# caomuqing/neptune

Hardware: AMD Instinct MI355X
Metric: backend_replans_per_sec (higher is better)
Workload: dtype f64; 1 GPU; 64 agents + 20 static obstacles, K=8, 128 seeded scenes in flight per GPU per step (seeds 0..127 over 1 GPU); the handle's default solve path: verified line presolve 4 m, polish on; agents=64, obstacles=20, scenes_per_gpu=128, scenes_in_flight=128, scene_groups=1

## Files before the change

include/neptune_backend_debug.h:

```cpp
#ifndef NEPTUNE_BACKEND_DEBUG_H
#define NEPTUNE_BACKEND_DEBUG_H

#include "neptune_backend.h"

#ifdef __cplusplus
extern "C" {
#endif

int nep_backend_debug_time_sequence(nep_backend_t* h, const nep_pwp* init, int32_t n_obst, const int32_t* hull_off,
                                    const double* hull_xy, const int32_t* h0_off, const double* h0_xy, const nep_ent_view* ent,
                                    double t_start, double dc, int32_t n_iter, double* us_out, double* us_optimize_out);

int nep_backend_debug_set_lines(nep_backend_t* h, int32_t n_lines, const int32_t* seg,
                                const double* nd);
int nep_backend_debug_get_lines(nep_backend_t* h, int32_t cap, int32_t* seg, double* nd,
                                int32_t* n_out);

int nep_debug_regroup_records(const nep_traj_rec* d_src, nep_traj_rec* d_dst, int32_t world, int32_t n_scenes,
                              int32_t n_local, void* stream);

int nep_batch_debug_redo_count(nep_batch_t* h, int32_t* by_reason);
int nep_batch_debug_redo_list(nep_batch_t* h, int32_t* slots_out, int32_t cap);

int64_t nep_batch_line_bucket_bytes(nep_batch_t* h);
int64_t nep_batch_row_scratch_bytes(nep_batch_t* h);

int nep_batch_active_rows(nep_batch_t* h, const nep_solution* d_solution, double tol, int32_t* d_out, void* stream);

int nep_batch_debug_set_separator_pack(nep_batch_t* h, int32_t pack);

int nep_batch_qp_placement(nep_batch_t* h);

int nep_batch_set_launch_order(nep_batch_t* h, int32_t enable);
int nep_batch_debug_launch_order(nep_batch_t* h, int32_t* order, int32_t cap, int32_t* n_out);

int nep_batch_debug_set_option(nep_batch_t* h, const char* name, int32_t value);
int nep_backend_debug_set_option(nep_backend_t* h, const char* name, int32_t value);
int nep_debug_set_global_option(const char* name, int32_t value);

int nep_batch_set_hull_kernel(nep_batch_t* h, int32_t mode);

int nep_batch_debug_conflicts(nep_batch_t* h, int32_t scene, uint8_t* conflict_out);
int nep_batch_debug_conflicts_prev(nep_batch_t* h, int32_t scene, uint8_t* conflict_out);

int nep_batch_kernel_time(nep_batch_t* h, int32_t which, double* avg_ms, int32_t* n_launch);
int nep_batch_enable_timing(nep_batch_t* h, int32_t on);
int nep_batch_reset_timing(nep_batch_t* h);

enum {
  NEP_PATH_BOX_KERNEL = 1,
  NEP_PATH_HULLS_GROUPED = 2,
  NEP_PATH_FUSED_BOXES = 4,
  NEP_PATH_FUSED_ORDER = 8,
  NEP_PATH_ORDERED_QP = 16,
  NEP_PATH_PRESOLVE_KERNEL = 32,
  NEP_PATH_REDO_PASS = 64
};
int nep_batch_debug_launch_path(nep_batch_t* h, int32_t* bits);
int nep_batch_debug_boxes(nep_batch_t* h, int32_t scene, double* out, int32_t cap);
int nep_batch_debug_order_keys(nep_batch_t* h, int32_t* keys, int32_t cap);

int nep_batch_debug_hulls(nep_batch_t* h, int32_t scene, double* hull_xy, int32_t* hull_nv);
int nep_batch_debug_lines(nep_batch_t* h, int32_t slot, int32_t cap, int32_t* seg, double* nd,
                          int32_t* n_out);

int nep_batch_debug_phase_cycles(nep_batch_t* h, int32_t slot, int64_t* out16);

int nep_batch_fe_search_us(nep_batch_t* h, float* us, int32_t cap);

int nep_batch_set_fe_ent_fast_caps(nep_batch_t* h, int32_t list_cap, int32_t add_cap, int32_t bend_cap);

int nep_batch_debug_polish_count(nep_batch_t* h, int32_t* listed, int32_t* certified);
int nep_batch_debug_polish_flags(nep_batch_t* h, int32_t* flags, int32_t cap);

int nep_debug_live_bytes(int64_t* device_bytes, int64_t* pinned_bytes);

#ifdef __cplusplus
}
#endif
#endif
```

neptune_amd/_lib.py:

```python
import ctypes as C
import os

from . import abi

_HERE = os.path.dirname(os.path.abspath(__file__))
LIB_PATH = os.environ.get("NEP_BACKEND_LIB") or os.path.join(_HERE, "libneptune_backend.so")
_lib = None

EXPORTS = [
    "nep_backend_create", "nep_backend_destroy", "nep_backend_set_max_values", "nep_backend_set_max_runtime",
    "nep_backend_set_tether_length", "nep_backend_set_static_obst_vert", "nep_backend_set_init_trajectory",
    "nep_backend_set_hulls", "nep_backend_set_hulls_no_inflation", "nep_backend_set_ent_state_vector",
    "nep_backend_optimize", "nep_backend_generate_pwp_out", "nep_backend_get_stats", "nep_inflate_static",
    "nep_separator_batch", "nep_separator_batch_rule", "nep_gjk_batch", "nep_hulls_batch", "nep_batch_create",
    "nep_batch_destroy", "nep_batch_set_scene_statics", "nep_batch_replan", "nep_batch_replan_lines", "nep_batch_replan_solve", "nep_batch_hull_block_bytes",
    "nep_batch_set_ent_samples", "nep_batch_hulls", "nep_batch_replan_hulls", "nep_comm_unique_id",
    "nep_comm_create", "nep_comm_destroy", "nep_comm_nranks", "nep_batch_exchange_hulls",
    "nep_batch_exchange_records", "nep_batch_exchange_slots", "nep_comm_reserve", "nep_batch_ent_bytes",
    "nep_batch_safety_commit", "nep_batch_set_line_cull", "nep_backend_set_line_cull", "nep_batch_get_line_cull", "nep_batch_reserve_row_scratch",
    "nep_batch_set_line_capacity", "nep_batch_set_separator_rule", "nep_backend_set_separator_rule",
    "nep_batch_set_tolerances", "nep_backend_set_tolerances", "nep_batch_set_polish", "nep_backend_set_polish", "nep_batch_set_max_runtime",
    "nep_batch_set_safety_check_prev", "nep_batch_set_active", "nep_batch_wait", "nep_batch_check", "nep_abi_sizeof", "nep_last_error",
    "nep_version",
]
DEBUG_EXPORTS = [
    "nep_batch_debug_polish_count", "nep_batch_debug_polish_flags",
    "nep_backend_debug_time_sequence", "nep_backend_debug_set_lines", "nep_backend_debug_get_lines",
    "nep_debug_regroup_records", "nep_batch_debug_redo_count", "nep_batch_debug_redo_list",
    "nep_batch_line_bucket_bytes", "nep_batch_row_scratch_bytes", "nep_batch_active_rows",
    "nep_batch_debug_set_separator_pack", "nep_batch_qp_placement", "nep_batch_set_launch_order",
    "nep_batch_debug_launch_order", "nep_batch_set_hull_kernel", "nep_batch_debug_conflicts", "nep_batch_debug_conflicts_prev",
    "nep_batch_kernel_time", "nep_batch_enable_timing", "nep_batch_reset_timing", "nep_batch_debug_hulls",
    "nep_batch_debug_lines", "nep_batch_debug_phase_cycles", "nep_batch_fe_search_us",
    "nep_batch_set_fe_ent_fast_caps", "nep_batch_debug_set_option", "nep_backend_debug_set_option", "nep_debug_set_global_option",
    "nep_batch_debug_launch_path", "nep_batch_debug_boxes", "nep_batch_debug_order_keys", "nep_debug_live_bytes",
]
PLAN_EXPORTS = [
    "nep_pwp_compose", "nep_pwp_compose_exact", "nep_dyntraj_wire_size", "nep_dyntraj_encode", "nep_dyntraj_decode", "nep_plan_create",
    "nep_plan_destroy", "nep_plan_reset", "nep_plan_size", "nep_plan_get", "nep_plan_next_goal",
    "nep_plan_select_a", "nep_plan_splice", "nep_plan_update_delta", "nep_plan_delta",
]
FE_EXPORTS = ["nep_batch_frontend", "nep_batch_frontend_hulls", "nep_batch_set_static_reps", "nep_batch_set_fe_ent_big_records", "nep_batch_frontend_ent", "nep_batch_frontend_ent_hulls", "nep_batch_safety_commit_ent", "nep_batch_track_ent", "nep_batch_track_ent_lists", "nep_batch_ent_lists_at_a", "nep_batch_next_starts", "nep_batch_audit", "nep_audit_records", "nep_audit_init"]
FLEET_EXPORTS = ["nep_batch_fleet_init", "nep_batch_fleet_select", "nep_batch_fleet_commit", "nep_batch_fleet_tick", "nep_batch_fleet_ring_cap",
                 "nep_batch_fleet_plans", "nep_batch_fleet_state", "nep_batch_fleet_counters", "nep_batch_fleet_init_ent", "nep_batch_fleet_predict_ent",
                 "nep_batch_fleet_track_ent", "nep_batch_fleet_ent_state", "nep_batch_fleet_init_ent_lists", "nep_batch_fleet_ent_lists", "nep_batch_fleet_mission_keepout", "nep_batch_fleet_mission_init",
                 "nep_batch_fleet_mission", "nep_batch_fleet_mission_state", "nep_batch_fleet_mission_log", "nep_mission_step"]
ENT_EXPORTS = ["nep_ent_sample_points", "nep_ent_propagate_segment", "nep_ent_propagate_guess", "nep_ent_case_ids", "nep_ent_track_step", "nep_ent_predict_a"]


class BackendError(RuntimeError):
    pass


def lib():
    global _lib
    if _lib is not None:
        return _lib
    if not os.path.exists(LIB_PATH):
        raise BackendError("%s is missing: build it with `python -c 'import __graft_entry__ as g; g.build()'` "
                           "(or make -C neptune_amd/csrc); there is no CPU fallback" % LIB_PATH)
    try:
        import torch
    except ImportError:
        pass
    L = C.CDLL(LIB_PATH)
    d, i, vp = C.c_double, C.c_int32, C.c_void_p
    pd, pi = C.POINTER(C.c_double), C.POINTER(C.c_int32)
    L.nep_last_error.restype = C.c_char_p
    L.nep_version.restype = C.c_char_p
    L.nep_abi_sizeof.argtypes = [i]; L.nep_abi_sizeof.restype = C.c_int
    L.nep_backend_create.argtypes = [C.POINTER(abi.nep_backend_cfg)]; L.nep_backend_create.restype = vp
    L.nep_backend_destroy.argtypes = [vp]; L.nep_backend_destroy.restype = None
    L.nep_backend_set_max_values.argtypes = [vp] + [d] * 9
    L.nep_backend_set_max_runtime.argtypes = [vp, d]
    L.nep_backend_set_tether_length.argtypes = [vp, d]
    L.nep_backend_set_static_obst_vert.argtypes = [vp, i, pi, pd]
    L.nep_backend_set_init_trajectory.argtypes = [vp, C.POINTER(abi.nep_pwp)]
    L.nep_backend_set_hulls.argtypes = [vp, i, pi, pd]
    L.nep_backend_set_hulls_no_inflation.argtypes = [vp, i, pi, pd]
    L.nep_backend_set_ent_state_vector.argtypes = [vp, C.POINTER(abi.nep_ent_view)]
    L.nep_backend_optimize.argtypes = [vp, pd]
    L.nep_backend_generate_pwp_out.argtypes = [vp, d, d, C.POINTER(abi.nep_pwp), pd, i, pi]
    L.nep_backend_get_stats.argtypes = [vp, C.POINTER(abi.nep_stats)]
    L.nep_backend_debug_set_lines.argtypes = [vp, i, pi, pd]
    L.nep_backend_debug_get_lines.argtypes = [vp, i, pi, pd, pi]
    L.nep_separator_batch.argtypes = [i, pi, pd, pi, pd, pd, pi]
    L.nep_inflate_static.argtypes = [i, pi, pd, d, pi, pd, i]
    L.nep_separator_batch_rule.argtypes = [i, i, pi, pd, pi, pd, pd, pi]
    L.nep_batch_set_separator_rule.argtypes = [vp, i]
    L.nep_backend_set_separator_rule.argtypes = [vp, i]
    L.nep_batch_set_tolerances.argtypes = [vp, C.c_double, C.c_double]
    L.nep_backend_set_tolerances.argtypes = [vp, C.c_double, C.c_double]
    L.nep_gjk_batch.argtypes = [i, pi, pd, pd, pi]
    L.nep_hulls_batch.argtypes = [i, vp, d, i, d, d, pd, pi, pd, pi]
    L.nep_batch_create.argtypes = [C.POINTER(abi.nep_batch_cfg)]; L.nep_batch_create.restype = vp
    L.nep_batch_destroy.argtypes = [vp]; L.nep_batch_destroy.restype = None
    L.nep_batch_replan.argtypes = [vp, vp, vp, vp, vp, vp, vp, vp]
    L.nep_batch_replan_lines.argtypes = [vp, vp, vp, vp, vp]
    L.nep_batch_replan_solve.argtypes = [vp, vp, vp, vp, vp, vp, vp, vp]
    L.nep_batch_ent_bytes.argtypes = [vp]; L.nep_batch_ent_bytes.restype = C.c_int64
    L.nep_batch_wait.argtypes = [vp, vp]
    L.nep_batch_kernel_time.argtypes = [vp, i, pd, pi]
    L.nep_batch_enable_timing.argtypes = [vp, i]
    L.nep_batch_reset_timing.argtypes = [vp]
    L.nep_batch_debug_hulls.argtypes = [vp, i, pd, pi]
    L.nep_batch_debug_lines.argtypes = [vp, i, i, pi, pd, pi]
    L.nep_batch_debug_phase_cycles.argtypes = [vp, i, C.POINTER(C.c_int64)]
    L.nep_batch_safety_commit.argtypes = [vp, vp, vp, vp, vp, vp, vp]
    L.nep_batch_debug_conflicts.argtypes = [vp, i, C.POINTER(C.c_uint8)]
    L.nep_batch_debug_conflicts_prev.argtypes = [vp, i, C.POINTER(C.c_uint8)]
    L.nep_batch_set_safety_check_prev.argtypes = [vp, i]
    L.nep_batch_set_active.argtypes = [vp, vp]
    L.nep_batch_set_line_cull.argtypes = [vp, d]; L.nep_backend_set_line_cull.argtypes = [vp, d]
    L.nep_batch_debug_set_option.argtypes = [vp, C.c_char_p, i]; L.nep_backend_debug_set_option.argtypes = [vp, C.c_char_p, i]; L.nep_debug_set_global_option.argtypes = [C.c_char_p, i]
    L.nep_batch_get_line_cull.argtypes = [vp]; L.nep_batch_get_line_cull.restype = d
    L.nep_batch_debug_redo_count.argtypes = [vp, pi]
    L.nep_batch_debug_redo_list.argtypes = [vp, pi, i]
    L.nep_batch_debug_set_separator_pack.argtypes = [vp, i]
    L.nep_batch_active_rows.argtypes = [vp, vp, d, vp, vp]
    L.nep_batch_reserve_row_scratch.argtypes = [vp]
    L.nep_batch_set_line_capacity.argtypes = [vp, i]
    L.nep_batch_set_fe_ent_big_records.argtypes = [vp, C.c_int64]
    L.nep_batch_set_fe_ent_fast_caps.argtypes = [vp, i, i, i]
    L.nep_batch_fe_search_us.argtypes = [vp, C.POINTER(C.c_float), i]
    L.nep_batch_line_bucket_bytes.argtypes = [vp]; L.nep_batch_line_bucket_bytes.restype = C.c_int64
    L.nep_batch_row_scratch_bytes.argtypes = [vp]; L.nep_batch_row_scratch_bytes.restype = C.c_int64
    L.nep_backend_debug_time_sequence.argtypes = [vp, vp, i, pi, pd, pi, pd, vp, d, d, i, pd, pd]
    L.nep_batch_set_max_runtime.argtypes = [vp, d]
    L.nep_batch_qp_placement.argtypes = [vp]
    L.nep_batch_set_launch_order.argtypes = [vp, i]
    L.nep_batch_set_hull_kernel.argtypes = [vp, i]
    L.nep_batch_debug_launch_order.argtypes = [vp, pi, i, pi]
    L.nep_batch_debug_launch_path.argtypes = [vp, pi]
    L.nep_batch_debug_boxes.argtypes = [vp, i, pd, i]
    L.nep_batch_debug_order_keys.argtypes = [vp, pi, i]
    L.nep_debug_live_bytes.argtypes = [C.POINTER(C.c_int64), C.POINTER(C.c_int64)]
    L.nep_batch_set_scene_statics.argtypes = [vp, i, i, pi, pd]
    L.nep_batch_check.argtypes = [vp, vp]
    L.nep_comm_unique_id.argtypes = [C.POINTER(C.c_uint8)]
    L.nep_comm_create.argtypes = [C.POINTER(C.c_uint8), i, i]; L.nep_comm_create.restype = vp
    L.nep_comm_destroy.argtypes = [vp]; L.nep_comm_destroy.restype = None
    L.nep_comm_nranks.argtypes = [vp]
    L.nep_comm_reserve.argtypes = [vp, C.c_int64, C.c_int64]
    L.nep_batch_exchange_hulls.argtypes = [vp, vp, vp, vp, vp]
    L.nep_batch_exchange_records.argtypes = [vp, vp, vp, vp, vp]
    L.nep_debug_regroup_records.argtypes = [vp, vp, i, i, i, vp]
    L.nep_batch_hull_block_bytes.argtypes = [vp]; L.nep_batch_hull_block_bytes.restype = C.c_int64
    L.nep_batch_hulls.argtypes = [vp, vp, vp, vp, vp]
    L.nep_batch_replan_hulls.argtypes = [vp, vp, i, vp, vp, vp, vp, vp, vp]
    ppwp, prec, phdr = C.POINTER(abi.nep_pwp), C.POINTER(abi.nep_traj_rec), C.POINTER(abi.nep_wire_header)
    pu8 = C.POINTER(C.c_uint8)
    L.nep_pwp_compose.argtypes = [d, d, ppwp, ppwp, ppwp]
    L.nep_pwp_compose_exact.argtypes = [d, ppwp, ppwp, ppwp]
    L.nep_dyntraj_wire_size.argtypes = [prec, phdr]; L.nep_dyntraj_wire_size.restype = C.c_int64
    L.nep_dyntraj_encode.argtypes = [prec, phdr, pu8, C.c_size_t]; L.nep_dyntraj_encode.restype = C.c_int64
    L.nep_dyntraj_decode.argtypes = [pu8, C.c_size_t, prec, phdr]; L.nep_dyntraj_decode.restype = C.c_int64
    L.nep_plan_create.argtypes = [C.POINTER(abi.nep_plan_cfg)]; L.nep_plan_create.restype = vp
    L.nep_plan_destroy.argtypes = [vp]; L.nep_plan_destroy.restype = None
    L.nep_plan_reset.argtypes = [vp, pd]
    L.nep_plan_size.argtypes = [vp]
    L.nep_plan_get.argtypes = [vp, i, pd]
    L.nep_plan_next_goal.argtypes = [vp, pd, pi]
    L.nep_plan_select_a.argtypes = [vp, pd, d, C.POINTER(abi.nep_point_a)]
    L.nep_plan_splice.argtypes = [vp, i, pd, i]
    L.nep_plan_update_delta.argtypes = [vp, d]
    L.nep_plan_delta.argtypes = [vp]
    pcfg, pin, pst = C.POINTER(abi.nep_ent_cfg), C.POINTER(abi.nep_ent_inputs), C.POINTER(abi.nep_ent_state)
    L.nep_ent_sample_points.argtypes = [ppwp, d, d, i, i, pd]
    L.nep_ent_propagate_segment.argtypes = [pcfg, pin, pst, pd, pd, pd, i, pd]
    L.nep_ent_propagate_guess.argtypes = [pcfg, pin, pst, vp, i, pi, pi, pi, pi, pst]
    L.nep_ent_case_ids.argtypes = [i, i, pi, pi, pi, i, pi]
    L.nep_ent_track_step.argtypes = [pcfg, C.POINTER(abi.nep_ent_track_inputs), pst, pd, pd]
    L.nep_ent_predict_a.argtypes = [pcfg, pd, pd, pi, pi, pd, pst, pd, pd, pst]
    L.nep_batch_frontend.argtypes = [vp, C.POINTER(abi.nep_fe_cfg), vp, vp, vp, vp, vp]
    L.nep_batch_frontend_hulls.argtypes = [vp, C.POINTER(abi.nep_fe_cfg), vp, i, vp, vp, vp, vp]
    L.nep_batch_set_static_reps.argtypes = [vp, i, pd, pd]
    L.nep_batch_frontend_ent.argtypes = [vp, C.POINTER(abi.nep_fe_cfg), vp, vp, vp, vp, vp, vp, vp]
    L.nep_batch_safety_commit_ent.argtypes = [vp, vp, vp, vp, vp, i, d, vp, vp, vp]
    L.nep_batch_next_starts.argtypes = [vp, vp, d, vp, vp, d, vp]
    L.nep_batch_track_ent.argtypes = [vp, vp, vp, vp, i, i, d, vp, vp, vp]
    L.nep_batch_track_ent_lists.argtypes = [vp, vp, vp, vp, i, i, d, C.POINTER(abi.nep_ent_lists), vp, vp]
    L.nep_batch_ent_lists_at_a.argtypes = [vp, C.POINTER(abi.nep_ent_lists), vp, vp, vp, vp, vp, vp]
    L.nep_batch_audit.argtypes = [vp, vp, vp, d, i, vp, vp]
    L.nep_audit_records.argtypes = [vp, i, pi, pd, i, d, d, d, i, vp]
    L.nep_audit_init.argtypes = [vp, C.c_int64]
    L.nep_batch_fleet_init.argtypes = [vp, C.POINTER(abi.nep_fleet_cfg), vp, vp, vp, vp, vp]
    L.nep_batch_fleet_select.argtypes = [vp, vp, vp, vp, vp, vp]
    L.nep_batch_fleet_commit.argtypes = [vp, vp, vp, vp, vp, vp, vp]
    L.nep_batch_fleet_tick.argtypes = [vp, vp]
    L.nep_batch_fleet_ring_cap.argtypes = [vp]
    L.nep_batch_fleet_plans.argtypes = [vp, i, i, pd, pi]
    L.nep_batch_fleet_state.argtypes = [vp, pd, vp, pi, pi, pi, pi, pi]
    L.nep_batch_fleet_counters.argtypes = [vp, pi, pd, pi]
    L.nep_batch_fleet_init_ent.argtypes = [vp, d, vp, vp]
    L.nep_batch_fleet_predict_ent.argtypes = [vp, vp, vp, vp, vp, vp]
    L.nep_batch_fleet_track_ent.argtypes = [vp, vp, vp, vp]
    L.nep_batch_fleet_ent_state.argtypes = [vp, vp, pi, pi, pi]
    L.nep_batch_fleet_init_ent_lists.argtypes = [vp, d, C.POINTER(abi.nep_ent_lists), vp]
    L.nep_batch_fleet_ent_lists.argtypes = [vp, C.POINTER(abi.nep_ent_lists), pi]
    L.nep_batch_fleet_mission_keepout.argtypes = [vp, i, i, pi, pd]
    L.nep_batch_fleet_mission_init.argtypes = [vp, C.POINTER(abi.nep_mission_cfg), vp]
    L.nep_batch_fleet_mission.argtypes = [vp, vp]
    L.nep_batch_fleet_mission_state.argtypes = [vp, pd, pd, pd, pi, pi, pd, pi, pd]
    L.nep_batch_fleet_mission_log.argtypes = [vp, vp, pi]
    L.nep_mission_step.argtypes = [C.POINTER(abi.nep_mission_cfg), C.POINTER(abi.nep_mission_scene)]
    L.nep_batch_frontend_ent_hulls.argtypes = [vp, C.POINTER(abi.nep_fe_cfg), vp, i, vp, vp, vp, vp, vp, vp]
    L.nep_batch_exchange_slots.argtypes = [vp, vp, vp, vp, C.c_int64, vp]
    L.nep_batch_set_ent_samples.argtypes = [vp, i]
    L.nep_batch_set_polish.argtypes = [vp, i]; L.nep_backend_set_polish.argtypes = [vp, i]; L.nep_batch_debug_polish_count.argtypes = [vp, pi, pi]; L.nep_batch_debug_polish_flags.argtypes = [vp, pi, i]
    L.nep_abi_sizeof.argtypes = [i]; L.nep_abi_sizeof.restype = i
    for which, struct in ((1, abi.nep_traj_rec), (5, abi.nep_guess), (6, abi.nep_solution), (11, abi.nep_fe_cfg), (12, abi.nep_fe_start),
                          (13, abi.nep_fe_result), (14, abi.nep_fe_ent_state), (17, abi.nep_audit), (18, abi.nep_fleet_cfg),
                          (20, abi.nep_mission_cfg), (21, abi.nep_mission_leg), (23, abi.nep_ent_lists)):
        if L.nep_abi_sizeof(which) != C.sizeof(struct):
            raise BackendError("%s: sizeof(%s) is %d in the library, %d in neptune_amd/abi.py — rebuild the library from this tree's headers"
                               % (LIB_PATH, struct.__name__, L.nep_abi_sizeof(which), C.sizeof(struct)))
    _lib = L
    return L
# ... 7 lines not shown
```

neptune_amd/backend.py:

```python
import ctypes as C

import numpy as np

from . import abi
from ._lib import BackendError, check, lib


def _csr(polys):
    off = np.zeros(len(polys) + 1, dtype=np.int32)
    for k, p in enumerate(polys):
        off[k + 1] = off[k] + len(p)
    xy = (np.concatenate([np.asarray(p, dtype=np.float64).reshape(-1, 2) for p in polys])
          if len(polys) and off[-1] > 0 else np.zeros((0, 2)))
    return off, np.ascontiguousarray(xy, dtype=np.float64)


def make_pwp(times, coeff):
    p = abi.nep_pwp()
    K = coeff.shape[1]
    p.n_seg = K
    for i in range(K + 1):
        p.times[i] = float(times[i])
    arr = np.ctypeslib.as_array(p.coeff)
    arr[:, :K, :] = coeff
# ... 383 lines not shown
        check(lib().nep_batch_fleet_ent_state(self._h, out["state"].ctypes.data if states else None, abi.iptr(out["flags"]), abi.iptr(out["ever"]),
                                              abi.iptr(out["walked"])))
        return out

    def fleet_mission_keepout(self, scene, polys):
        off, xy = _csr(polys)
        check(lib().nep_batch_fleet_mission_keepout(self._h, scene, len(polys), abi.iptr(off), abi.dptr(xy)))

    def fleet_mission_init(self, cfg, stream=None):
        st = stream if stream is not None else self.torch.cuda.current_stream(self.device)
        check(lib().nep_batch_fleet_mission_init(self._h, C.byref(cfg), st.cuda_stream))
        self.mission_cfg = cfg

    def fleet_mission(self, stream=None):
        st = stream if stream is not None else self.torch.cuda.current_stream(self.device)
        check(lib().nep_batch_fleet_mission(self._h, st.cuda_stream))

    def fleet_mission_state(self):
        n, S = self.slots, self.n_scenes
        out = dict(goal=np.zeros((n, 3)), t_issue=np.zeros(n), length=np.zeros(n), completed=np.zeros(n, dtype=np.int32),
                   counts=np.zeros((n, 4), dtype=np.int32), sums=np.zeros((n, 2)), scene=np.zeros((S, 4), dtype=np.int32), t_run=np.zeros(S))
        check(lib().nep_batch_fleet_mission_state(self._h, abi.dptr(out["goal"]), abi.dptr(out["t_issue"]), abi.dptr(out["length"]),
                                                  abi.iptr(out["completed"]), abi.iptr(out["counts"]), abi.dptr(out["sums"]),
                                                  abi.iptr(out["scene"]), abi.dptr(out["t_run"])))
        return out

    def fleet_mission_finished(self):
        sc = np.zeros((self.n_scenes, 4), dtype=np.int32)
        check(lib().nep_batch_fleet_mission_state(self._h, None, None, None, None, None, None, abi.iptr(sc), None))
        return sc[:, 3] != 0

    def fleet_mission_log(self, ordered=True):
        cfg = self.mission_cfg
        owners = self.slots if cfg.mode == abi.NEP_MISSION_PER_AGENT else self.n_scenes
        cap = int(cfg.log_cap)
        log = np.zeros((owners, max(cap, 1)), dtype=abi.MISSION_LEG_DTYPE); n = np.zeros(owners, dtype=np.int32)
        check(lib().nep_batch_fleet_mission_log(self._h, log.ctypes.data, abi.iptr(n)))
        log = log[:, :cap]
        if not ordered:
            return log, n
        return [log[o, [i % cap for i in range(max(0, int(n[o]) - cap), int(n[o]))]] if cap else log[o, :0] for o in range(owners)], n

    def next_starts(self, d_records, dt, d_start, d_alt_goal=None, switch_radius=0.0, stream=None):
        st = stream if stream is not None else self.torch.cuda.current_stream(self.device)
        check(lib().nep_batch_next_starts(self._h, d_records.data_ptr(), float(dt), d_start.data_ptr(),
                                          d_alt_goal.data_ptr() if d_alt_goal is not None else None, float(switch_radius), st.cuda_stream))

    def safety_commit(self, d_prev, d_new, d_guess, d_final, d_accept=None, stream=None):
        st = stream if stream is not None else self.torch.cuda.current_stream(self.device)
        check(lib().nep_batch_safety_commit(self._h, d_prev.data_ptr(), d_new.data_ptr(), d_guess.data_ptr(), d_final.data_ptr(),
                                            d_accept.data_ptr() if d_accept is not None else None, st.cuda_stream))

    def set_active(self, mask):
        torch = self.torch
        if mask is not None:
            if mask.dtype != torch.int32 or mask.device != self.device or tuple(mask.shape) != (self.n_scenes, self.N) or not mask.is_contiguous():
                raise ValueError("the active mask is a contiguous int32 tensor [n_scenes, N] on the handle's device")
        check(lib().nep_batch_set_active(self._h, mask.data_ptr() if mask is not None else None))
        self._active = mask

    def set_scene_statics(self, scene, statics):
        soff, sxy = _csr(statics)
        check(lib().nep_batch_set_scene_statics(self._h, scene, len(statics), abi.iptr(soff), abi.dptr(sxy)))

    def check(self, stream=None):
        st = stream if stream is not None else self.torch.cuda.current_stream(self.device)
        check(lib().nep_batch_check(self._h, st.cuda_stream))

    def qp_kernel_name(self):
        return "qp_reg_kernel" if lib().nep_batch_qp_placement(self._h) == 1 else "qp_kernel"

    def set_hull_kernel(self, mode=0):
        check(lib().nep_batch_set_hull_kernel(self._h, int(mode)))

    def set_launch_order(self, enable=True):
        check(lib().nep_batch_set_launch_order(self._h, 1 if enable else 0))

    def launch_order(self):
        out = np.zeros(self.n_scenes * self.n_local, dtype=np.int32); n = C.c_int32(0)
        check(lib().nep_batch_debug_launch_order(self._h, abi.iptr(out), len(out), C.byref(n)))
        return out[:n.value].copy() if n.value else None

    LAUNCH_PATH = (("box_kernel", 1), ("grouped_hulls", 2), ("fused_boxes", 4), ("fused_order", 8), ("ordered_qp", 16),
                   ("presolve_kernel", 32), ("redo_pass", 64))

    def debug_launch_path(self):
        b = C.c_int32(0)
        check(lib().nep_batch_debug_launch_path(self._h, C.byref(b)))
        return {name: bool(b.value & bit) for name, bit in self.LAUNCH_PATH}

    def debug_boxes(self, scene=0):
        out = np.zeros((self.N + self.n_static, self.par.num_pol, 4))
        check(lib().nep_batch_debug_boxes(self._h, int(scene), abi.dptr(out), out.size))
        return out

    def debug_order_keys(self):
        out = np.zeros(self.slots, dtype=np.int32)
        check(lib().nep_batch_debug_order_keys(self._h, abi.iptr(out), len(out)))
        return out

    def set_max_runtime(self, seconds):
        check(lib().nep_batch_set_max_runtime(self._h, float(seconds)))

    def set_line_cull(self, radius):
        check(lib().nep_batch_set_line_cull(self._h, float(radius)))

    def line_cull(self):
        return float(lib().nep_batch_get_line_cull(self._h))

    def redo_count(self):
        r = np.zeros(2, dtype=np.int32)
        n = int(check(lib().nep_batch_debug_redo_count(self._h, abi.iptr(r))))
        self.redo_reasons = {"parked_line_violated": int(r[0]), "moved_beyond_radius": int(r[1])}
        return n

    def reserve_row_scratch(self):
        check(lib().nep_batch_reserve_row_scratch(self._h))

    def fe_search_us(self):
        out = np.zeros(self.slots, dtype=np.float32)
        check(lib().nep_batch_fe_search_us(self._h, out.ctypes.data_as(C.POINTER(C.c_float)), int(self.slots)))
        return out

    def set_fe_ent_big_records(self, records):
        check(lib().nep_batch_set_fe_ent_big_records(self._h, int(records)))

    def set_fe_ent_fast_caps(self, list_cap=40, add_cap=32, bend_cap=8):
        check(lib().nep_batch_set_fe_ent_fast_caps(self._h, int(list_cap), int(add_cap), int(bend_cap)))

    def set_line_capacity(self, lines_per_segment):
        check(lib().nep_batch_set_line_capacity(self._h, int(lines_per_segment)))

    def line_bucket_bytes(self):
        return int(lib().nep_batch_line_bucket_bytes(self._h))

    def row_scratch_bytes(self):
        return int(lib().nep_batch_row_scratch_bytes(self._h))

    def set_separator_pack(self, pack):
        check(lib().nep_batch_debug_set_separator_pack(self._h, int(pack)))

    def redo_list(self, cap=4096):
        out = np.zeros(cap, dtype=np.int32)
        n = int(check(lib().nep_batch_debug_redo_list(self._h, abi.iptr(out), cap)))
        return out[:n].copy()

    def set_separator_rule(self, rule):
        check(lib().nep_batch_set_separator_rule(self._h, int(rule)))

    def set_tolerances(self, residual_tol=1e-10, gap_tol=1e-11):
        check(lib().nep_batch_set_tolerances(self._h, float(residual_tol), float(gap_tol)))

    def set_polish(self, on=True):
        check(lib().nep_batch_set_polish(self._h, int(on) if (on is not True and on is not False) else (1 if on else 0)))

    def debug_option(self, name, value):
        check(lib().nep_batch_debug_set_option(self._h, name.encode(), int(value)))

    def polish_count(self):
        a = C.c_int32(0); b = C.c_int32(0)
        check(lib().nep_batch_debug_polish_count(self._h, C.byref(a), C.byref(b)))
        return a.value, b.value

    def polish_flags(self):
        out = np.zeros(self.n_scenes * self.n_local, dtype=np.int32)
        check(lib().nep_batch_debug_polish_flags(self._h, abi.iptr(out), len(out)))
        return out

    def set_safety_check_prev(self, on=True):
        check(lib().nep_batch_set_safety_check_prev(self._h, 1 if on else 0))

    def debug_conflicts(self, scene=0):
        out = np.zeros((self.N, self.N), dtype=np.uint8)
        check(lib().nep_batch_debug_conflicts(self._h, scene, out.ctypes.data_as(C.POINTER(C.c_uint8))))
        return out

    def debug_conflicts_prev(self, scene=0):
        out = np.zeros((self.N, self.N), dtype=np.uint8)
        check(lib().nep_batch_debug_conflicts_prev(self._h, scene, out.ctypes.data_as(C.POINTER(C.c_uint8))))
        return out

# ... 71 lines not shown
```

neptune_amd/csrc/backend.hip:

```cpp
#include <hip/hip_runtime.h>

#include <atomic>
#include <chrono>
#include <cmath>
#include <cstdio>
#include <cstdlib>
#include <cstring>
#include <memory>
#include <string>
#include <vector>

#include "nep_device.h"
#include "qp_outputs.h"
#include "audit_common.h"
#include "mission_common.h"
#include "../../include/neptune_plan.h"
#include "../../include/neptune_entangle.h"

using namespace nep;

namespace nep { DebugGlobals g_debug; }

namespace {

// ... 14 lines not shown
  ~DevBuf() { release(); }
  int ensure(size_t count) {
    if (count <= n && p) return 0;
    release();
    if (count == 0) count = 1;
    hipError_t e = hipMalloc((void**)&p, count * sizeof(T));
    if (e != hipSuccess) { p = nullptr; g_err = std::string("hipMalloc: ") + hipGetErrorString(e); return NEP_E_HIP; }
    n = count; g_live_device += (long long)(n * sizeof(T));
    return 0;
  }
  void release() { if (p) { hipFree(p); g_live_device -= (long long)(n * sizeof(T)); } p = nullptr; n = 0; }
};

struct ListBuf {
  DevBuf<int> n_alpha, n_bend; DevBuf<int16_t> id, bend; DevBuf<int8_t> cs; DevBuf<double> beta; int cap = 0;
  int ensure(size_t slots, int cap_) {
    if (int e = n_alpha.ensure(slots)) return e;
    if (int e = n_bend.ensure(slots)) return e;
    if (int e = id.ensure(slots * cap_)) return e;
    if (int e = cs.ensure(slots * cap_)) return e;
    if (int e = beta.ensure(slots * cap_)) return e;
    if (int e = bend.ensure(slots * NEP_MAX_BEND)) return e;
    cap = cap_;
    return 0;
  }
  nep_ent_lists view() const { nep_ent_lists v{}; v.cap = cap; v.n_alpha = n_alpha.p; v.n_bend = n_bend.p; v.id = id.p; v.cs = cs.p; v.beta = beta.p; v.bend = bend.p; return v; }
};

struct PinnedArena {
  char* p = nullptr; size_t n = 0;
  PinnedArena() = default;
  PinnedArena(const PinnedArena&) = delete;
  PinnedArena& operator=(const PinnedArena&) = delete;
  PinnedArena(PinnedArena&& o) noexcept : p(o.p), n(o.n) { o.p = nullptr; o.n = 0; }
  PinnedArena& operator=(PinnedArena&& o) noexcept { if (this != &o) { release(); p = o.p; n = o.n; o.p = nullptr; o.n = 0; } return *this; }
  ~PinnedArena() { release(); }
  int ensure(size_t bytes) {
    if (bytes <= n && p) return 0;
    char* q = nullptr;
    hipError_t e = hipHostMalloc((void**)&q, bytes ? bytes : 1, hipHostMallocDefault);
    if (e != hipSuccess) { g_err = std::string("hipHostMalloc: ") + hipGetErrorString(e); return NEP_E_HIP; }
    if (p) std::memcpy(q, p, n);
    if (bytes > n) std::memset(q + n, 0, bytes - n);
    release();
    p = q; n = bytes; g_live_pinned += (long long)(bytes ? bytes : 1);
    return 0;
  }
  void release() { if (p) { hipHostFree(p); g_live_pinned -= (long long)(n ? n : 1); } p = nullptr; n = 0; }
};

constexpr size_t kLdsBudget = 150 * 1024;

bool normalize_ccw(double* xy, int n) {
  if (n < 3) return true;
  double area2 = 0, scale = 0;
  for (int v = 0; v < n; v++) {
    const double* a = xy + 2 * v; const double* b = xy + 2 * ((v + 1) % n);
    area2 += a[0] * b[1] - a[1] * b[0];
    scale = std::fmax(scale, std::fmax(std::fabs(a[0]), std::fabs(a[1])));
  }
  if (area2 < 0) for (int lo = 1, hi = n - 1; lo < hi; lo++, hi--) { std::swap(xy[2 * lo], xy[2 * hi]); std::swap(xy[2 * lo + 1], xy[2 * hi + 1]); }
  const double tol = 1e-9 * (1.0 + scale) * (1.0 + scale);
  for (int v = 0; v < n; v++) {
    const double* o = xy + 2 * v; const double* a = xy + 2 * ((v + 1) % n); const double* b = xy + 2 * ((v + 2) % n);
    if ((a[0] - o[0]) * (b[1] - o[1]) - (a[1] - o[1]) * (b[0] - o[0]) < -tol) return false;
  }
  return true;
}

double wall_clock_hz() {
  int dev = 0, khz = 0;
  if (hipGetDevice(&dev) == hipSuccess && hipDeviceGetAttribute(&khz, hipDeviceAttributeWallClockRate, dev) == hipSuccess && khz > 0) return (double)khz * 1e3;
  return 1e8;
}

struct Engine {
  SceneParams sp{};
  int n_scenes = 1;
  DevBuf<QpTable> d_tables;
  DevBuf<int> d_sched_n, d_sched_seg; DevBuf<double> d_sched_dt;
  DevBuf<double> d_pb, d_static_xy, d_static_el; DevBuf<int> d_static_nv;
  DevBuf<double> d_hull_xy, d_hull0_xy, d_bend_xy, d_line_nd, d_row_scratch;
  DevBuf<int> d_hull_nv, d_hull0_nv, d_bend_n, d_line_cnt, d_line_far, d_lp_stats;
  DevBuf<int> d_presolved; bool presolve_kernel = true;
  DevBuf<int> d_line_skip, d_redo_list, d_redo_count;
  DevBuf<double> d_polish_z; DevBuf<int> d_polish_flag, d_polish_list, d_polish_count; bool polish = true, polish_presolve = true, last_polish_armed = false;
  DevBuf<long long> d_dbg; bool profile_phases = false;
  DevBuf<int> d_flags;
  DevBuf<double> d_sampled, d_srep, d_slong; DevBuf<int> d_present, d_entangles;
  DevBuf<nep_fe_ent_state> d_fe_nodes, d_fe_work, d_fe_saved; DevBuf<double> d_fe_arc, d_fe_packed; bool have_reps = false;
  DevBuf<double> d_fe_big_beta, d_fe_stf; DevBuf<long long> d_fe_stvox; DevBuf<unsigned> d_fe_xpool;
  DevBuf<unsigned char> d_fe_big, d_fe_big_check; DevBuf<int> d_fe_big_count, d_fe_big_check_count; long fe_big_records = 0;
  int fe_fast_cap = NEP_FE_ENT_CAP, fe_fast_add = 32, fe_fast_bend = NEP_MAX_BEND;
  DevBuf<unsigned char> d_conflict, d_conflict_prev;
  bool safety_check_prev = false;
  int lds_lines = 0, lds_rows = 0, rows_cap = 0; size_t lds_bytes = 0;
  DevBuf<double> d_fe_box;
  DevBuf<int> d_fe_order, d_fe_order_key; DevBuf<float> d_fe_us; bool fe_history = false, fe_lpt = true;
  DevBuf<int> d_order, d_order_key; bool have_history = false, lpt = true, last_ordered = false;
  const int* active = nullptr;
  DevBuf<int> d_act, d_fe_act;
  ListBuf d_track_lsave;
  DevBuf<nep_fe_ent_state> d_track_save; DevBuf<int> d_track_flags; DevBuf<double> d_track_pos;
  DevBuf<AuditPart> d_audit_part;
  int static_nv_max = 0;
  DevBuf<nep_traj_rec> d_safety_recs;
  bool use_reg = false;
  double clock_hz = 1e8;
  void set_clock() { clock_hz = wall_clock_hz(); sp.us_per_tick = 1e6 / clock_hz; sp.corr_from_it = opt_corr_from; sp.corr_max_count = opt_corr_max; if (!(sp.tol_res > 0.0)) { sp.tol_res = 1e-10; sp.tol_gap = 1e-11; sp.tol_res_inv = 1e10; sp.tol_gap_inv = 1e11; sp.tol_gap_floor = 0.1 * 1e-11; } }
  double sched_dc = -1, tab_T = -1, tab_w = -1; int sched_cap = 0;
  std::vector<int> h_sched_n, h_sched_seg; std::vector<double> h_sched_dt;
  bool timing = false; std::vector<hipEvent_t> ev; size_t ev_used = 0;

  int build_tables() {
    if (tab_T == sp.T_span && tab_w == sp.weight && d_tables.p) return 0;
    std::vector<QpTable> t(2 * (kMaxK + 1));
    std::memset(t.data(), 0, t.size() * sizeof(QpTable));
    for (int mode = 0; mode < 2; mode++) for (int K = 1; K <= kMaxK; K++) build_qp_table(K, sp.T_span, sp.weight, mode, &t[mode * (kMaxK + 1) + K]);
    if (int e = d_tables.ensure(t.size())) return e;
    HIPCHK(hipMemcpy(d_tables.p, t.data(), t.size() * sizeof(QpTable), hipMemcpyHostToDevice));
    tab_T = sp.T_span; tab_w = sp.weight;
    return 0;
  }
  int build_schedule(double dc, int cap) {
    if (dc == sched_dc && cap == sched_cap && d_sched_n.p) return 0;
    h_sched_n.assign(kMaxK + 1, 0); h_sched_seg.assign((size_t)(kMaxK + 1) * cap, 0); h_sched_dt.assign((size_t)(kMaxK + 1) * cap, 0.0);
    for (int K = 1; K <= kMaxK; K++) h_sched_n[K] = build_sample_schedule(K, sp.T_span, dc, cap, &h_sched_seg[(size_t)K * cap], &h_sched_dt[(size_t)K * cap]);
    if (int e = d_sched_n.ensure(h_sched_n.size())) return e;
    if (int e = d_sched_seg.ensure(h_sched_seg.size())) return e;
    if (int e = d_sched_dt.ensure(h_sched_dt.size())) return e;
    HIPCHK(hipMemcpy(d_sched_n.p, h_sched_n.data(), h_sched_n.size() * sizeof(int), hipMemcpyHostToDevice));
    HIPCHK(hipMemcpy(d_sched_seg.p, h_sched_seg.data(), h_sched_seg.size() * sizeof(int), hipMemcpyHostToDevice));
    HIPCHK(hipMemcpy(d_sched_dt.p, h_sched_dt.data(), h_sched_dt.size() * sizeof(double), hipMemcpyHostToDevice));
    sched_dc = dc; sched_cap = cap; sp.max_states = cap; sp.dc = dc;
    return 0;
  }
  static constexpr double kAutoCullRadius = 4.0;
  bool fits_reg = true, cull_user_set = false, skip_lps = true, no_redo = false; int lds_lines_lds = 0, sep_pack = 0, force_kernel = 0, opt_qp_key_decay = 2, opt_fe_key_decay = 1, opt_corr_from = kCorrFromItDefault, opt_corr_max = kCorrMaxCountDefault, opt_fleet_ent_proof = 1;
  static constexpr int kScratchPool = 1024;
  bool scratch_full = false; int scratch_chunks = 0;
  std::vector<double> h_static_box;
  const double* box_buf = nullptr; int box_N = -1, box_S = -1, box_np = -1;
  bool static_boxes_ok = false;
  bool static_boxes_placed() const { return static_boxes_ok && box_buf == d_fe_box.p && box_N == sp.num_agents && box_S == sp.n_static && box_np == sp.num_pol; }
  static void static_boxes_of(int n, const std::vector<double>& sx, const std::vector<int>& nv, double* out) {
    for (int j = 0; j < n; j++) {
      const double* q = &sx[(size_t)j * kHullV * 2];
      double x0 = HUGE_VAL, x1 = -HUGE_VAL, y0 = HUGE_VAL, y1 = -HUGE_VAL;
      if (nv[j] > 0) { x0 = x1 = q[0]; y0 = y1 = q[1]; }
      for (int v = 1; v < nv[j]; v++) { x0 = std::fmin(x0, q[2 * v]); x1 = std::fmax(x1, q[2 * v]); y0 = std::fmin(y0, q[2 * v + 1]); y1 = std::fmax(y1, q[2 * v + 1]); }
      out[4 * j] = x0; out[4 * j + 1] = x1; out[4 * j + 2] = y0; out[4 * j + 3] = y1;
    }
  }
  int push_static_boxes(int scene = -1) {
    const bool placed = static_boxes_placed();
    static_boxes_ok = false;
    const int N = sp.num_agents, S = sp.n_static, np = sp.num_pol;
    const size_t row = (size_t)(N + S) * np * 4, blk = (size_t)S * np * 4;
    if (!d_fe_box.p || d_fe_box.n < (size_t)n_scenes * row || h_static_box.size() < (size_t)n_scenes * S * 4) return 0;
    if (S > 0) {
      const int s0 = (scene >= 0 && placed) ? scene : 0, s1 = (scene >= 0 && placed) ? scene + 1 : n_scenes;
      std::vector<double> b((size_t)(s1 - s0) * blk);
      for (int s = s0; s < s1; s++)
        for (int j = 0; j < S; j++)
          for (int i = 0; i < np; i++) std::memcpy(&b[(((size_t)(s - s0) * S + j) * np + i) * 4], &h_static_box[((size_t)s * S + j) * 4], 4 * sizeof(double));
      HIPCHK(hipMemcpy2D(d_fe_box.p + (size_t)s0 * row + (size_t)N * np * 4, row * sizeof(double), b.data(), blk * sizeof(double), blk * sizeof(double), (size_t)(s1 - s0), hipMemcpyHostToDevice));
    }
// ... 1 lines not shown
    return 0;
  }
  int last_path = 0;
  int lines_cap_user = 0;
  bool can_skip_lps() const { return sp.cull_radius > 0.0 && use_reg && sp.sep_rule == 0 && sp.skip_own == 1 && sp.n_hull == sp.num_agents && skip_lps && statics_boxy; }
  bool skip_mode() const { return can_skip_lps() && !no_redo; }
  int size_row_scratch() {
    const long slots = (long)n_scenes * sp.n_local;
    const bool pooled = skip_mode() && !scratch_full && slots > kScratchPool;
    scratch_chunks = pooled ? kScratchPool : 0;
    return d_row_scratch.ensure((size_t)(pooled ? kScratchPool : slots) * (11L * (rows_cap / 4 + 2)));
  }
  void choose_placement() {
    use_reg = fits_reg || sp.cull_radius > 0.0;
    if (force_kernel == 1) use_reg = true; else if (force_kernel == 2) use_reg = false;
    if (use_reg) { lds_lines = NEP_MAX_POL * 8 * qp_reg_slots(); lds_rows = 4 * lds_lines; lds_bytes = qp_reg_lds_bytes(); }
    else { lds_lines = lds_lines_lds; lds_rows = 4 * lds_lines; lds_bytes = qp_lds_fixed_bytes() + (size_t)(lds_lines + 2) * 11 * 8; }
  }
  int size_scratch() {
    const int N = sp.num_agents, np = sp.num_pol;
    const long slots = (long)n_scenes * sp.n_local;
    const int worst_lines = sp.n_hull + N + sp.n_static + (sp.ent_enabled ? N * kBend : 0);
    if ((long)NEP_MAX_POL * worst_lines > 65535) return fail(NEP_E_CAP, "more than 65535 separator candidates per agent");
    sp.lines_cap = lines_cap_user < 0 ? worst_lines : (lines_cap_user > 0 ? lines_cap_user : sp.n_hull + N + sp.n_static + (sp.ent_enabled ? std::min(N * kBend, std::max(2 * N, 64)) : 0));
    if (sp.lines_cap > worst_lines) sp.lines_cap = worst_lines;
    if (sp.lines_cap < 8) sp.lines_cap = 8;
    const long lines_total = (long)NEP_MAX_POL * sp.lines_cap;
    const size_t fixed = qp_lds_fixed_bytes();
    const long per_line = 11 * 8;
    const long l_half = ((long)(160 * 1024 / 2) - (long)fixed) / per_line - 2;
    const long l_full = ((long)kLdsBudget - (long)fixed) / per_line - 2;
    const long expect = (long)NEP_MAX_POL * (sp.n_hull + 4 + sp.n_static / 8 + (sp.ent_enabled ? sp.num_agents / 8 : 0));
    long ll = expect <= l_half ? l_half : l_full;
    if (ll > lines_total) ll = lines_total;
    lds_lines_lds = (int)((ll + 1) & ~1L);
    fits_reg = expect / NEP_MAX_POL <= 8L * qp_reg_slots() + 8;
    if (!cull_user_set) sp.cull_radius = kAutoCullRadius;
    sp.fe_key_decay = opt_fe_key_decay; sp.qp_key_decay = opt_qp_key_decay;
    if (lpt) { if (int e = d_order.ensure((size_t)slots)) return e; const int* was = d_order_key.p; if (int e = d_order_key.ensure((size_t)slots)) return e; if (d_order_key.p != was) hipMemset(d_order_key.p, 0, d_order_key.n * sizeof(int)); }
    if (lpt) { if (int e = d_fe_order.ensure((size_t)slots)) return e; const int* was = d_fe_order_key.p; if (int e = d_fe_order_key.ensure((size_t)slots)) return e; if (d_fe_order_key.p != was) hipMemset(d_fe_order_key.p, 0, d_fe_order_key.n * sizeof(int)); }
    if (int e = d_fe_us.ensure((size_t)slots)) return e;
    choose_placement();
    rows_cap = 4 * (int)lines_total; rows_cap = (rows_cap + 3) & ~3;
    if (int e = d_hull_xy.ensure((size_t)n_scenes * sp.n_hull * np * kHullV * 2)) return e;
    if (int e = d_fe_box.ensure((size_t)n_scenes * (N + (sp.n_static > 0 ? sp.n_static : 0)) * np * 4)) return e;
    if (!static_boxes_placed()) { if (int e = push_static_boxes()) return e; }
    if (int e = d_hull_nv.ensure((size_t)n_scenes * sp.n_hull * np)) return e;
    if (int e = d_hull0_xy.ensure((size_t)n_scenes * N * np * 2)) return e;
    if (int e = d_hull0_nv.ensure((size_t)n_scenes * N * np)) return e;
    if (int e = d_bend_xy.ensure((size_t)n_scenes * N * kBend * 2)) return e;
    if (int e = d_bend_n.ensure((size_t)n_scenes * N)) return e;
    if (int e = d_line_nd.ensure((size_t)slots * lines_total * 3)) return e;
    if (int e = d_line_cnt.ensure((size_t)slots * NEP_MAX_POL)) return e;
    if (int e = d_line_far.ensure((size_t)slots * NEP_MAX_POL)) return e;
    if (int e = d_lp_stats.ensure((size_t)slots * NEP_MAX_POL * 2)) return e;
    if (int e = d_line_skip.ensure((size_t)slots * NEP_MAX_POL)) return e;
    if (int e = d_redo_list.ensure((size_t)slots)) return e;
    if (int e = d_presolved.ensure((size_t)slots)) return e;
    if (!d_redo_count.p) { if (int e = d_redo_count.ensure(4)) return e; HIPCHK(hipMemset(d_redo_count.p, 0, 4 * sizeof(int))); }
    if (!d_flags.p) { if (int e = d_flags.ensure(1)) return e; HIPCHK(hipMemset(d_flags.p, 0, sizeof(int))); }
    if (int e = d_polish_z.ensure((size_t)slots * 2 * 24)) return e;
    if (int e = d_polish_flag.ensure((size_t)slots)) return e;
    if (int e = d_polish_list.ensure((size_t)slots)) return e;
    if (!d_polish_count.p) { if (int e = d_polish_count.ensure(8)) return e; HIPCHK(hipMemset(d_polish_count.p, 0, 8 * sizeof(int))); }
    if (!profile_phases) profile_phases = getenv("NEP_QP_PROFILE") != nullptr;
    if (profile_phases) { if (int e = d_dbg.ensure((size_t)slots * 32)) return e; }
    if (int e = size_row_scratch()) return e;
    return 0;
  }
  void fill(ProblemSet& ps) {
    ps.pb = d_pb.p; ps.static_xy = d_static_xy.p; ps.static_nv = d_static_nv.p; ps.static_el = d_static_el.p;
    ps.hull_xy = d_hull_xy.p; ps.hull_nv = d_hull_nv.p; ps.hull0_xy = d_hull0_xy.p; ps.hull0_nv = d_hull0_nv.p;
    ps.bend_xy = d_bend_xy.p; ps.bend_n = d_bend_n.p;
    ps.fe_order = nullptr; ps.fe_order_key = (lpt && fe_lpt && d_fe_order_key.n >= (size_t)n_scenes * (size_t)sp.n_local) ? d_fe_order_key.p : nullptr; ps.fe_us = d_fe_us.p;
    ps.line_nd = d_line_nd.p; ps.line_cnt = d_line_cnt.p; ps.lp_stats = d_lp_stats.p;
    ps.line_far = sp.cull_radius > 0.0 ? d_line_far.p : nullptr;
    const bool skip = can_skip_lps();
    ps.scratch_chunks = skip_mode() ? scratch_chunks : 0; ps.scratch_by_block = 0;
    ps.skip_box = skip ? d_fe_box.p : nullptr; ps.line_skip = skip ? d_line_skip.p : nullptr;
    ps.redo_list = skip ? d_redo_list.p : nullptr; ps.redo_count = skip ? d_redo_count.p : nullptr; ps.order_count = nullptr;
    ps.sep_pack = sep_pack;
    ps.row_scratch = d_row_scratch.p; ps.rows_cap = rows_cap; ps.lds_rows = lds_rows; ps.lds_lines = lds_lines;
    ps.dbg = profile_phases ? d_dbg.p : nullptr;
    ps.presolved = nullptr;
    ps.flags = d_flags.p;
    ps.fe_box = d_fe_box.p;
    ps.active = active; ps.fe_count = nullptr;
    const bool pol = polish && use_reg && (polish_presolve || !(sp.cull_radius > 0.0)) && d_polish_z.p != nullptr;
    ps.polish_z = pol ? d_polish_z.p : nullptr; ps.polish_flag = pol ? d_polish_flag.p : nullptr;
    ps.polish_list = pol ? d_polish_list.p : nullptr; ps.polish_count = pol ? d_polish_count.p : nullptr;
    last_polish_armed = pol;
  }
  bool statics_boxy = true;
  int pack_statics(int n, const int32_t* off, const double* xy, std::vector<double>& sx, std::vector<int>& nv, std::vector<double>& el) {
    sx.assign((size_t)(n > 0 ? n : 1) * kHullV * 2, 0.0); nv.assign(n > 0 ? n : 1, 0);
    for (int j = 0; j < n; j++) {
      int c = off[j + 1] - off[j];
      if (c > kHullV) return fail(NEP_E_CAP, "static obstacle with more than NEP_HULL_MAX_V vertices");
      if (c < 0) return fail(NEP_E_ARG, "static obstacle offsets must not decrease");
      nv[j] = c;
      if (c > static_nv_max) static_nv_max = c;
      for (int v = 0; v < c; v++) { sx[((size_t)j * kHullV + v) * 2] = xy[2 * (off[j] + v)]; sx[((size_t)j * kHullV + v) * 2 + 1] = xy[2 * (off[j] + v) + 1]; }
      if (!normalize_ccw(&sx[(size_t)j * kHullV * 2], c)) return fail(NEP_E_ARG, "static obstacle polygon is not convex");
      if (c > 0) {
        const double* q = &sx[(size_t)j * kHullV * 2];
        double lo[2] = {q[0], q[1]}, hi[2] = {q[0], q[1]};
        for (int v = 1; v < c; v++) for (int a = 0; a < 2; a++) { lo[a] = std::min(lo[a], q[2 * v + a]); hi[a] = std::max(hi[a], q[2 * v + a]); }
        const double tol = 1e-9 * (1.0 + (hi[0] - lo[0]) + (hi[1] - lo[1]));
        for (int a = 0; a < 2; a++) {
          int n_lo = 0, n_hi = 0;
          for (int v = 0; v < c; v++) { n_lo += q[2 * v + a] - lo[a] <= tol; n_hi += hi[a] - q[2 * v + a] <= tol; }
          if (n_lo < 2 || n_hi < 2) statics_boxy = false;
        }
      }
    }
    el.assign(sx.size() / 2, 0.0);
    for (int j = 0; j < n; j++)
      for (int v = 0; v + 1 < nv[j]; v++) {
        const double* q = &sx[((size_t)j * kHullV + v) * 2];
        volatile double ex = q[2] - q[0], ey = q[3] - q[1];
        volatile double a = ex * ex, b = ey * ey;
        volatile double c = a + b;
        el[(size_t)j * kHullV + v] = std::sqrt(c);
      }
    return 0;
  }
  int upload_statics(int n, const int32_t* off, const double* xy) {
    static_boxes_ok = false;
    std::vector<double> sx, el; std::vector<int> nv;
    statics_boxy = true;
    if (int e = pack_statics(n, off, xy, sx, nv, el)) return e;
    if (int e = d_static_xy.ensure(sx.size())) return e;
    if (int e = d_static_el.ensure(el.size())) return e;
    if (int e = d_static_nv.ensure(nv.size())) return e;
    HIPCHK(hipMemcpy(d_static_el.p, el.data(), el.size() * sizeof(double), hipMemcpyHostToDevice));
    HIPCHK(hipMemcpy(d_static_xy.p, sx.data(), sx.size() * sizeof(double), hipMemcpyHostToDevice));
    HIPCHK(hipMemcpy(d_static_nv.p, nv.data(), nv.size() * sizeof(int), hipMemcpyHostToDevice));
    sp.n_static = n; sp.static_stride = 0;
    h_static_box.resize((size_t)n_scenes * n * 4);
    for (int s = 0; s < n_scenes; s++) static_boxes_of(n, sx, nv, &h_static_box[(size_t)s * n * 4]);
    if (n_scenes > 0 && sp.num_agents > 0 && sp.num_pol > 0)
      if (int e = d_fe_box.ensure((size_t)n_scenes * (sp.num_agents + n) * sp.num_pol * 4)) return e;
    return push_static_boxes();
  }
  int upload_scene_statics(int scene, int n, const int32_t* off, const double* xy) {
    const int S = sp.n_static;
    if (n != S) return fail(NEP_E_ARG, "every scene must have the handle's n_static polygons");
    if (S == 0) return 0;
    std::vector<double> sx, el; std::vector<int> nv;
    if (int e = pack_statics(n, off, xy, sx, nv, el)) return e;
    if (sp.static_stride == 0) {
      DevBuf<double> nxy, nel; DevBuf<int> nnv;
      if (int e = nxy.ensure((size_t)n_scenes * S * kHullV * 2)) return e;
      if (int e = nel.ensure((size_t)n_scenes * S * kHullV)) return e;
      if (int e = nnv.ensure((size_t)n_scenes * S)) return e;
      for (int s = 0; s < n_scenes; s++) {
        HIPCHK(hipMemcpy(nxy.p + (size_t)s * S * kHullV * 2, d_static_xy.p, (size_t)S * kHullV * 2 * sizeof(double), hipMemcpyDeviceToDevice));
        HIPCHK(hipMemcpy(nel.p + (size_t)s * S * kHullV, d_static_el.p, (size_t)S * kHullV * sizeof(double), hipMemcpyDeviceToDevice));
        HIPCHK(hipMemcpy(nnv.p + (size_t)s * S, d_static_nv.p, (size_t)S * sizeof(int), hipMemcpyDeviceToDevice));
      }
      d_static_xy = std::move(nxy); d_static_el = std::move(nel); d_static_nv = std::move(nnv);
      sp.static_stride = S;
      if (have_reps && d_srep.p && d_srep.n >= (size_t)S * 4 && d_slong.n >= (size_t)S * 2) {
        DevBuf<double> nr, nl;
        if (int e = nr.ensure((size_t)n_scenes * S * 4)) return e;
        if (int e = nl.ensure((size_t)n_scenes * S * 2)) return e;
        for (int s = 0; s < n_scenes; s++) {
          HIPCHK(hipMemcpy(nr.p + (size_t)s * S * 4, d_srep.p, (size_t)S * 4 * sizeof(double), hipMemcpyDeviceToDevice));
          HIPCHK(hipMemcpy(nl.p + (size_t)s * S * 2, d_slong.p, (size_t)S * 2 * sizeof(double), hipMemcpyDeviceToDevice));
        }
        d_srep = std::move(nr); d_slong = std::move(nl);
      } else have_reps = false;
    }
    HIPCHK(hipMemcpy(d_static_xy.p + (size_t)scene * S * kHullV * 2, sx.data(), (size_t)S * kHullV * 2 * sizeof(double), hipMemcpyHostToDevice));
    HIPCHK(hipMemcpy(d_static_el.p + (size_t)scene * S * kHullV, el.data(), (size_t)S * kHullV * sizeof(double), hipMemcpyHostToDevice));
    HIPCHK(hipMemcpy(d_static_nv.p + (size_t)scene * S, nv.data(), (size_t)S * sizeof(int), hipMemcpyHostToDevice));
    static_boxes_of(S, sx, nv, &h_static_box[(size_t)scene * S * 4]);
    return push_static_boxes(scene);
  }
  hipEvent_t next_event() {
    if (ev_used == ev.size()) { hipEvent_t e; hipEventCreate(&e); ev.push_back(e); }
    return ev[ev_used++];
  }
  int run(const nep_traj_rec* d_recs, int n_rec, ProblemSet& ps, hipStream_t st, int phases = 3) {
    const int slots = n_scenes * sp.n_local;
    SampleSched sc{d_sched_n.p, d_sched_seg.p, d_sched_dt.p};
    const bool geo = (phases & 1) != 0, qp = (phases & 2) != 0;
    if (timing) hipEventRecord(next_event(), st);
    const bool fused_boxes = d_recs && geo && ps.skip_box != nullptr && !ps.lines_override && static_boxes_ok && ps.hull_pb <= 0
                             && n_rec == sp.num_agents && sp.n_hull == sp.num_agents && hulls_grouped(sp, n_scenes, n_rec);
    const bool want_order = qp && lpt && have_history && slots > 1024 && d_order_key.n >= (size_t)slots && d_order.n >= (size_t)slots;
    const bool fused_order = fused_boxes && want_order;
    if (fused_order) { ps.order = d_order.p; ps.order_key = d_order_key.p; }
    if (geo) last_path = 0; else last_path &= NEP_PATH_BOX_KERNEL | NEP_PATH_HULLS_GROUPED | NEP_PATH_FUSED_BOXES | NEP_PATH_FUSED_ORDER;
    if (d_recs && geo) launch_hulls(d_recs, n_scenes, n_rec, ps.guess, sp, ps, st, fused_boxes);
    if (d_recs && geo && hulls_grouped(sp, n_scenes, n_rec)) last_path |= NEP_PATH_HULLS_GROUPED;
    if (fused_boxes) last_path |= NEP_PATH_FUSED_BOXES;
    if (fused_order) last_path |= NEP_PATH_FUSED_ORDER;
    if (timing) hipEventRecord(next_event(), st);
    if (ps.lines_override) { ps.skip_box = nullptr; ps.line_skip = nullptr; ps.redo_list = nullptr; ps.redo_count = nullptr; }
    if (scratch_chunks > 0 && ps.scratch_chunks == 0) {
      scratch_full = true;
      HIPCHK(hipStreamSynchronize(st));
      if (int e = size_row_scratch()) return e;
      ps.row_scratch = d_row_scratch.p;
    }
    const bool skip = ps.skip_box != nullptr;
    if (!ps.lines_override && geo) {
      if (skip && !fused_boxes) { launch_boxes(n_scenes, sp, ps, st); last_path |= NEP_PATH_BOX_KERNEL; }
      launch_separator(slots, sp, ps, st);
    }
    if (timing) hipEventRecord(next_event(), st);
    if (!qp) { if (timing) hipEventRecord(next_event(), st); HIPCHK(hipGetLastError()); return 0; }
    ps.order = nullptr; last_ordered = false;
    ps.order_key = (lpt && d_order_key.n >= (size_t)slots) ? d_order_key.p : nullptr;
    if (ps.order_key && have_history && slots > 1024 && d_order.n >= (size_t)slots) {
      if (!fused_order) launch_qp_order(slots, d_order_key.p, d_order.p, st, ps.polish_count);
      ps.order = d_order.p; last_ordered = true; last_path |= NEP_PATH_ORDERED_QP;
    } else if (ps.polish_count && !(use_reg && slots == 1)) launch_qp_polish_zero(ps.polish_count, st);
    if (ps.active) {
      if (int e = d_act.ensure((size_t)slots + 1)) return e;
      launch_active_list(slots, sp, ps.active, ps.order, d_act.p, ps.polish_count, st);
      ps.order = d_act.p; ps.order_count = d_act.p + slots;
      launch_skipped_replan(slots, sp, ps, st);
    }
    if (use_reg && presolve_kernel && ps.line_far != nullptr && !ps.lines_override && d_presolved.n >= (size_t)slots) {
      ps.presolved = d_presolved.p;
      launch_qp_presolve(slots, sp, ps, d_tables.p, sc, d_presolved.p, st);
      last_path |= NEP_PATH_PRESOLVE_KERNEL;
    }
    if (use_reg) launch_qp_reg(slots, sp, ps, d_tables.p, sc, lds_bytes, st);
    else launch_qp(slots, sp, ps, d_tables.p, sc, lds_bytes, st);
    if (skip && !no_redo) {
      launch_separator_redo(slots, sp, ps, st);
      last_path |= NEP_PATH_REDO_PASS;
      ProblemSet pr = ps;
      pr.line_far = nullptr; pr.line_skip = nullptr; pr.order = d_redo_list.p; pr.order_count = d_redo_count.p;
      pr.presolved = nullptr;
      pr.scratch_by_block = ps.scratch_chunks > 0 ? 1 : 0;
      launch_qp_reg(slots, sp, pr, d_tables.p, sc, lds_bytes, st);
    }
    if (ps.polish_list) launch_qp_polish(slots, sp, ps, d_tables.p, sc, st);
    have_history = ps.order_key != nullptr;
    if (timing) hipEventRecord(next_event(), st);
    HIPCHK(hipGetLastError());
    return 0;
  }
  ~Engine() { for (auto e : ev) hipEventDestroy(e); }
};

bool have_device() { int n = 0; return hipGetDeviceCount(&n) == hipSuccess && n > 0; }


__global__ void sample_kernel(const nep_solution* __restrict__ sol, int K, const int* __restrict__ seg, const double* __restrict__ dt, int ns, double* __restrict__ out) {
  const int s = blockIdx.x * blockDim.x + threadIdx.x;
  if (s >= ns) return;
  sample_state(&sol->coeff[0][0][0], seg[s], dt[s], out + (long)s * NEP_STATE_DOUBLES);
}

int read_lines(Engine& E, size_t slot, int n_seg, int32_t cap, int32_t* seg, double* nd, int32_t* n_out) {
  std::vector<int> cnt(NEP_MAX_POL), far(NEP_MAX_POL, 0); std::vector<double> buf((size_t)NEP_MAX_POL * E.sp.lines_cap * 3);
  HIPCHK(hipMemcpy(cnt.data(), E.d_line_cnt.p + slot * NEP_MAX_POL, cnt.size() * sizeof(int), hipMemcpyDeviceToHost));
  if (E.sp.cull_radius > 0.0) HIPCHK(hipMemcpy(far.data(), E.d_line_far.p + slot * NEP_MAX_POL, far.size() * sizeof(int), hipMemcpyDeviceToHost));
  HIPCHK(hipMemcpy(buf.data(), E.d_line_nd.p + slot * NEP_MAX_POL * E.sp.lines_cap * 3, buf.size() * sizeof(double), hipMemcpyDeviceToHost));
  for (int& c : cnt) c = line_count(c);
  int n = 0;
  for (int s = 0; s < n_seg && s < NEP_MAX_POL; s++)
    for (int c = 0; c < cnt[s] + far[s]; c++) {
      const size_t q = c < cnt[s] ? (size_t)c : (size_t)E.sp.lines_cap - 1 - (size_t)(c - cnt[s]);
      const double* e = &buf[((size_t)s * E.sp.lines_cap + q) * 3];
      if (e[0] == 0.0 && e[1] == 0.0 && e[2] == 0.0) continue;
      if (n < cap) { seg[n] = s; for (int k = 0; k < 3; k++) nd[3 * n + k] = e[k]; }
      n++;
    }
  *n_out = n;
  return 0;
}

}

struct InLayout { size_t guess, nv, cas, h0xy, h0nv, bend, bendn, xy, cap_end; };
static InLayout in_layout(int N, int np, int cap) {
  auto up = [](size_t v) { return (v + 255) & ~(size_t)255; };
  InLayout L{};
  size_t o = 0;
  L.guess = o; o = up(o + sizeof(nep_guess));
  L.nv = o; o = up(o + (size_t)cap * np * sizeof(int));
  L.cas = o; o = up(o + (size_t)NEP_MAX_POL * N * sizeof(int));
  L.h0xy = o; o = up(o + (size_t)N * np * 2 * sizeof(double));
  L.h0nv = o; o = up(o + (size_t)N * np * sizeof(int));
  L.bend = o; o = up(o + (size_t)N * kBend * 2 * sizeof(double));
  L.bendn = o; o = up(o + (size_t)N * sizeof(int));
  L.xy = o; o = up(o + (size_t)cap * np * kHullV * 2 * sizeof(double));
  L.cap_end = o;
  return L;
}
struct nep_backend {
  Engine eng;
  nep_backend_cfg cfg{};
  std::vector<double> pb;
  double max_runtime = 0.05, tether = 0, j_max = 0;
  bool have_bounds = false, have_init = false, have_hulls = false, solved = false;
  nep_guess guess{}; std::vector<double> guess_times;
  int n_obst = 0;
  PinnedArena hin, hout; DevBuf<char> d_in, d_out;
  int in_cap = 0; InLayout L{};
  bool have_h0 = false, have_ent = false, states_fresh = false;
  int override_n = -1; std::vector<int> ov_seg; std::vector<double> ov_nd;
  nep_solution h_sol{}; nep_stats stats{};
// ... 1275 lines not shown
  launch_next_starts(d_records, h->cfg.n_scenes, h->cfg.num_agents, h->cfg.first_local, h->cfg.n_local, dt, d_start, d_alt_goal, switch_radius, (hipStream_t)stream);
  HIPCHK(hipGetLastError());
  return 0;
}

int nep_batch_set_scene_statics(nep_batch_t* h, int32_t scene, int32_t n_static, const int32_t* static_off, const double* static_xy) {
  if (!h || scene < 0 || scene >= h->cfg.n_scenes || n_static < 0 || (n_static > 0 && (!static_off || !static_xy))) return fail(NEP_E_ARG, "bad arguments");
  HIPCHK(hipDeviceSynchronize());
  return h->eng.upload_scene_statics(scene, n_static, static_off, static_xy);
}

int nep_batch_debug_redo_count(nep_batch_t* h, int32_t* by_reason) {
  if (!h) return fail(NEP_E_ARG, "null handle");
  int n[3] = {0, 0, 0};
  HIPCHK(hipDeviceSynchronize());
  if (h->eng.d_redo_count.p) HIPCHK(hipMemcpy(n, h->eng.d_redo_count.p, 3 * sizeof(int), hipMemcpyDeviceToHost));
  if (by_reason) { by_reason[0] = n[1]; by_reason[1] = n[2]; }
  return n[0];
}

int nep_batch_debug_redo_list(nep_batch_t* h, int32_t* slots_out, int32_t cap) {
  if (!h || !slots_out || cap < 0) return fail(NEP_E_ARG, "bad arguments");
  int n = 0;
  HIPCHK(hipDeviceSynchronize());
  if (!h->eng.d_redo_count.p) return 0;
  HIPCHK(hipMemcpy(&n, h->eng.d_redo_count.p, sizeof(int), hipMemcpyDeviceToHost));
  if (n > cap) n = cap;
  if (n > 0) HIPCHK(hipMemcpy(slots_out, h->eng.d_redo_list.p, (size_t)n * sizeof(int), hipMemcpyDeviceToHost));
  return n;
}

int nep_batch_debug_set_separator_pack(nep_batch_t* h, int32_t pack) {
  if (!h || pack < -1 || pack > NEP_MAX_POL) return fail(NEP_E_ARG, "pack must be -1, 0 or 1..NEP_MAX_POL");
  h->eng.sep_pack = pack;
  return 0;
}

int nep_batch_qp_placement(nep_batch_t* h) { return h ? (h->eng.use_reg ? 1 : 0) : NEP_E_ARG; }

int nep_batch_set_launch_order(nep_batch_t* h, int32_t enable) {
  if (!h) return fail(NEP_E_ARG, "null handle");
  if (enable) { if (int e = h->eng.d_order.ensure((size_t)h->slots)) return e; if (int e = h->eng.d_order_key.ensure((size_t)h->slots)) return e; }
  if (enable) { if (int e = h->eng.d_fe_order.ensure((size_t)h->slots)) return e; if (int e = h->eng.d_fe_order_key.ensure((size_t)h->slots)) return e; }
  if (!enable) { h->eng.have_history = false; h->eng.fe_history = false; }
  if (enable && !h->eng.lpt) {
    HIPCHK(hipDeviceSynchronize());
    HIPCHK(hipMemset(h->eng.d_order_key.p, 0, h->eng.d_order_key.n * sizeof(int))); HIPCHK(hipMemset(h->eng.d_fe_order_key.p, 0, h->eng.d_fe_order_key.n * sizeof(int)));
    h->eng.have_history = false; h->eng.fe_history = false;
  }
  h->eng.lpt = enable != 0;
  return 0;
}
int nep_batch_fe_search_us(nep_batch_t* h, float* us, int32_t cap) {
  if (!h || !us || cap < h->slots) return fail(NEP_E_ARG, "bad arguments");
  HIPCHK(hipDeviceSynchronize());
  HIPCHK(hipMemcpy(us, h->eng.d_fe_us.p, (size_t)h->slots * sizeof(float), hipMemcpyDeviceToHost));
  return 0;
}
int nep_batch_debug_launch_order(nep_batch_t* h, int32_t* order, int32_t cap, int32_t* n_out) {
  if (!h || !order || !n_out || cap < 0) return fail(NEP_E_ARG, "bad arguments");
  *n_out = 0;
  if (!h->eng.last_ordered) return 0;
  if (cap < h->slots) return fail(NEP_E_CAP, "order buffer smaller than the slot count");
  HIPCHK(hipDeviceSynchronize());
  HIPCHK(hipMemcpy(order, h->eng.d_order.p, (size_t)h->slots * sizeof(int), hipMemcpyDeviceToHost));
  *n_out = h->slots;
  return 0;
}
int nep_batch_debug_launch_path(nep_batch_t* h, int32_t* bits) {
  if (!h || !bits) return fail(NEP_E_ARG, "bad arguments");
  *bits = h->eng.last_path;
  return 0;
}
int nep_batch_debug_boxes(nep_batch_t* h, int32_t scene, double* out, int32_t cap) {
  if (!h || !out || scene < 0 || scene >= h->cfg.n_scenes || cap < 0) return fail(NEP_E_ARG, "bad arguments");
  const Engine& E = h->eng;
  const size_t n = (size_t)(E.sp.num_agents + E.sp.n_static) * E.sp.num_pol * 4;
  if ((size_t)cap < n) return fail(NEP_E_CAP, "box buffer smaller than (num_agents + n_static) x num_pol x 4 doubles");
  if (!E.d_fe_box.p || E.d_fe_box.n < (size_t)h->cfg.n_scenes * n) return fail(NEP_E_STATE, "the handle has no obstacle boxes");
  HIPCHK(hipDeviceSynchronize());
  HIPCHK(hipMemcpy(out, E.d_fe_box.p + (size_t)scene * n, n * sizeof(double), hipMemcpyDeviceToHost));
  return 0;
}
int nep_batch_debug_order_keys(nep_batch_t* h, int32_t* keys, int32_t cap) {
  if (!h || !keys || cap < 0) return fail(NEP_E_ARG, "bad arguments");
  if (cap < h->slots) return fail(NEP_E_CAP, "key buffer smaller than the slot count");
  if (!h->eng.d_order_key.p || h->eng.d_order_key.n < (size_t)h->slots) return fail(NEP_E_STATE, "the handle has no ordering keys (nep_batch_set_launch_order)");
  HIPCHK(hipDeviceSynchronize());
  HIPCHK(hipMemcpy(keys, h->eng.d_order_key.p, (size_t)h->slots * sizeof(int), hipMemcpyDeviceToHost));
  return 0;
}

static int engine_option(Engine& E, const char* name, int32_t v) {
  if (!name) return fail(NEP_E_ARG, "null option name");
  const std::string n(name);
  if (n == "qp_kernel") { if (v < 0 || v > 2) return fail(NEP_E_ARG, "qp_kernel: 0 automatic, 1 register placement, 2 LDS placement"); E.force_kernel = v; E.choose_placement(); }
  else if (n == "sep_skip") E.skip_lps = v != 0;
  else if (n == "sep_no_redo") E.no_redo = v != 0;
  else if (n == "qp_lpt") E.lpt = v != 0;
  else if (n == "fe_lpt") E.fe_lpt = v != 0;
  else if (n == "qp_key_decay") E.opt_qp_key_decay = v;
  else if (n == "fe_key_decay") E.opt_fe_key_decay = v;
  else if (n == "sep_pack") { if (v < -1 || v > NEP_MAX_POL) return fail(NEP_E_ARG, "sep_pack: -1 unpacked, 0 automatic, 1..NEP_MAX_POL"); E.sep_pack = v; }
  else if (n == "corr_from") { if (v < 1) return fail(NEP_E_ARG, "corr_from >= 1"); E.opt_corr_from = v; E.sp.corr_from_it = v; }
  else if (n == "corr_max") { if (v < 1) return fail(NEP_E_ARG, "corr_max >= 1"); E.opt_corr_max = v; E.sp.corr_max_count = v; }
  else if (n == "fleet_ent_proof") E.opt_fleet_ent_proof = v != 0;
  else if (n == "qp_profile") E.profile_phases = v != 0;
  else if (n == "presolve_kernel") E.presolve_kernel = v != 0;
  else return fail(NEP_E_ARG, "unknown debug option: " + n);
  return 0;
}
int nep_batch_debug_set_option(nep_batch_t* h, const char* name, int32_t value) { if (!h) return fail(NEP_E_ARG, "null handle"); return engine_option(h->eng, name, value); }
int nep_backend_debug_set_option(nep_backend_t* h, const char* name, int32_t value) { if (!h) return fail(NEP_E_ARG, "null handle"); return engine_option(h->eng, name, value); }
int nep_debug_set_global_option(const char* name, int32_t value) {
  if (!name) return fail(NEP_E_ARG, "null option name");
  const std::string n(name);
  if (n == "fe_three") g_debug.fe_three = value != 0;
  else if (n == "fe_xcd") g_debug.fe_xcd = value;
  else if (n == "polish_grid") { if (value < 1) return fail(NEP_E_ARG, "polish_grid >= 1"); g_debug.polish_grid = value; }
  else return fail(NEP_E_ARG, "unknown global debug option: " + n);
  return 0;
}

int nep_batch_set_hull_kernel(nep_batch_t* h, int32_t mode) {
  if (!h || mode < 0 || mode > 2) return fail(NEP_E_ARG, "mode: 0 automatic, 1 one hull per wave, 2 eight hulls per wave");
  h->eng.sp.hull_mode = mode;
  return 0;
}

int nep_batch_set_max_runtime(nep_batch_t* h, double seconds) {
  if (!h || !(seconds >= 0.0)) return fail(NEP_E_ARG, "bad arguments");
  h->eng.sp.time_limit_ticks = seconds > 0 ? (long long)(seconds * h->eng.clock_hz) : 0;
  return 0;
}

namespace {
int set_line_cull(Engine* E, double radius) {
  if (!E || !(radius >= 0.0)) return fail(NEP_E_ARG, "bad arguments");
  E->sp.cull_radius = radius; E->cull_user_set = true;
  return 0;
}
int set_separator_rule(Engine* E, int32_t rule) {
  if (!E || (rule != 0 && rule != 1)) return fail(NEP_E_ARG, "separator rule: 0 largest gap, 1 GLPK-class simplex");
  E->sp.sep_rule = rule;
  return 0;
}
int resize_row_scratch(Engine& E) { HIPCHK(hipDeviceSynchronize()); return E.size_row_scratch(); }
}
int nep_batch_set_line_cull(nep_batch_t* h, double radius) {
  if (int e = set_line_cull(h ? &h->eng : nullptr, radius)) return e;
  h->eng.choose_placement();
  return resize_row_scratch(h->eng);
}
double nep_batch_get_line_cull(nep_batch_t* h) { return h ? h->eng.sp.cull_radius : -1.0; }
int nep_backend_set_line_cull(nep_backend_t* h, double radius) { return set_line_cull(h ? &h->eng : nullptr, radius); }

int nep_batch_set_separator_rule(nep_batch_t* h, int32_t rule) {
  if (int e = set_separator_rule(h ? &h->eng : nullptr, rule)) return e;
  return resize_row_scratch(h->eng);
}
int nep_batch_reserve_row_scratch(nep_batch_t* h) {
  if (!h) return fail(NEP_E_ARG, "null handle");
  h->eng.scratch_full = true;
  return resize_row_scratch(h->eng);
}
int nep_batch_set_line_capacity(nep_batch_t* h, int32_t lines_per_segment) {
  if (!h || lines_per_segment < -1) return fail(NEP_E_ARG, "bad arguments");
  HIPCHK(hipDeviceSynchronize());
  h->eng.lines_cap_user = lines_per_segment;
  return h->eng.size_scratch();
}
int64_t nep_batch_line_bucket_bytes(nep_batch_t* h) { return h ? (int64_t)h->slots * NEP_MAX_POL * h->eng.sp.lines_cap * 3 * (int64_t)sizeof(double) : 0; }
int64_t nep_batch_row_scratch_bytes(nep_batch_t* h) { return h ? (int64_t)(h->eng.d_row_scratch.n * sizeof(double)) : 0; }
int nep_backend_set_separator_rule(nep_backend_t* h, int32_t rule) { return set_separator_rule(h ? &h->eng : nullptr, rule); }

namespace { int set_tol(Engine& E, double res, double gap) {
  if (!(res >= 1e-12 && res <= 1e-6) || !(gap >= 1e-13 && gap <= 1e-7)) return fail(NEP_E_ARG, "tolerances: residuals in [1e-12, 1e-6], relative gap in [1e-13, 1e-7]");
  E.sp.tol_res = res; E.sp.tol_gap = gap;
  E.sp.tol_res_inv = res == 1e-10 ? 1e10 : (res == 1e-9 ? 1e9 : 1.0 / res); E.sp.tol_gap_inv = gap == 1e-11 ? 1e11 : (gap == 1e-10 ? 1e10 : 1.0 / gap); E.sp.tol_gap_floor = 0.1 * gap;
  return 0;
} }
int nep_batch_set_tolerances(nep_batch_t* h, double residual_tol, double gap_tol) { if (!h) return fail(NEP_E_ARG, "null handle"); return set_tol(h->eng, residual_tol, gap_tol); }
int nep_backend_set_tolerances(nep_backend_t* h, double residual_tol, double gap_tol) { if (!h) return fail(NEP_E_ARG, "null handle"); return set_tol(h->eng, residual_tol, gap_tol); }

namespace { int set_polish(Engine& E, int32_t on) { E.polish = on != 0; E.polish_presolve = on == 1 || on == 2; return 0; } }
int nep_batch_set_polish(nep_batch_t* h, int32_t on) { if (!h) return fail(NEP_E_ARG, "null handle"); return set_polish(h->eng, on); }
int nep_backend_set_polish(nep_backend_t* h, int32_t on) { if (!h) return fail(NEP_E_ARG, "null handle"); return set_polish(h->eng, on); }
int nep_batch_debug_polish_count(nep_batch_t* h, int32_t* listed, int32_t* certified) {
  if (!h) return fail(NEP_E_ARG, "null handle");
  int c[8] = {0, 0, 0, 0, 0, 0, 0, 0};
// ... 157 lines not shown
```

neptune_amd/csrc/geom_kernels.hip:

```cpp
#include <hip/hip_runtime.h>

#include <cstdlib>
#include <cstring>

#include "nep_device.h"
#include "../../include/neptune_frontend.h"
#include "ent_device.h"

namespace nep {

__constant__ double cAPosInv[4][4] = {
    {-0.03203276669713047, -0.09273093424558249, 0.3420572455666699, 1.1023313949144335},
    {-0.05111494245568798, -0.046272612998418894, 0.5458234872124772, 1.0979806946005568},
    {-0.07454781852812224, 0.203951949894552, 0.796048050105448, 1.0745478185281223},
    {1.0, 1.0, 0.9999999999999996, 0.9999999999999993}};

#define SEP_MIN_GAP 1e-7
#define NEP_INF (__builtin_huge_val())

__device__ __forceinline__ double cross3(double ox, double oy, double ax, double ay, double bx, double by) {
  return (ax - ox) * (by - oy) - (ay - oy) * (bx - ox);
}
__device__ __forceinline__ bool lex_less(double ax, double ay, double bx, double by) {
  return ax < bx || (ax == bx && ay < by);
}

__device__ int wave_hull(int n, double px, double py, double* sxy, double* hxy) {
  const int lane = threadIdx.x & 63;
  sxy[2 * lane] = px; sxy[2 * lane + 1] = py;
  __syncthreads();
  int rank = 0;
  if (lane < n) {
    for (int j = 0; j < n; j++) {
      const double qx = sxy[2 * j], qy = sxy[2 * j + 1];
      if (lex_less(qx, qy, px, py) || (qx == px && qy == py && j < lane)) rank++;
    }
  }
  __syncthreads();
  if (lane < n) { sxy[2 * rank] = px; sxy[2 * rank + 1] = py; }
  __syncthreads();
  double ux = 0, uy = 0; bool keep = false;
  if (lane < n) { ux = sxy[2 * lane]; uy = sxy[2 * lane + 1]; keep = lane == 0 || ux != sxy[2 * lane - 2] || uy != sxy[2 * lane - 1]; }
  const unsigned long long km = __ballot(keep);
  const int m = __popcll(km);
  __syncthreads();
  if (keep) { const int pos = __popcll(km & ((1ull << lane) - 1ull)); sxy[2 * pos] = ux; sxy[2 * pos + 1] = uy; }
  __syncthreads();
  if (m == 0) return 0;
  if (m == 1) { if (lane == 0) { hxy[0] = sxy[0]; hxy[1] = sxy[1]; } __syncthreads(); return 1; }
  double* hu = hxy + 132;
  int kc = 0;
  if (lane < 2) {
    double* st = lane == 0 ? hxy : hu;
    double ax = 0, ay = 0, bx = 0, by = 0;
    for (int i = 0; i < m; i++) {
      const int idx = lane == 0 ? i : m - 1 - i;
      const double x = sxy[2 * idx], y = sxy[2 * idx + 1];
      while (kc >= 2 && cross3(ax, ay, bx, by, x, y) <= 0.0) { kc--; bx = ax; by = ay; if (kc >= 2) { ax = st[2 * (kc - 2)]; ay = st[2 * (kc - 2) + 1]; } }
      st[2 * kc] = x; st[2 * kc + 1] = y; kc++;
      ax = bx; ay = by; bx = x; by = y;
    }
  }
  const int kl = __shfl(kc, 0), ku = __shfl(kc, 1);
  __syncthreads();
  if (lane >= 1 && lane < ku - 1) { hxy[2 * (kl + lane - 1)] = hu[2 * lane]; hxy[2 * (kl + lane - 1) + 1] = hu[2 * lane + 1]; }
  __syncthreads();
  return kl + ku - 2;
}

__device__ void hull_body(const nep_traj_rec* __restrict__ r, double ts, int i, double T_span, double drone_radius,
                          long out, bool full0, double* __restrict__ hull_xy, int* __restrict__ hull_nv,
                          double* __restrict__ hull0_xy, int* __restrict__ hull0_nv, int* __restrict__ flags) {
  __shared__ __attribute__((aligned(16))) double sxy[128], hxy[264];
  __shared__ double cpx[kHullCP], cpy[kHullCP], stimes[NEP_TRAJ_MAX_SEG + 2];
  const int lane = threadIdx.x;
  if (!(r->valid && r->is_agent) || r->pwp.n_seg <= 0) {
    if (lane == 0) { hull_nv[out] = 0; if (hull0_nv) hull0_nv[out] = 0; }
    return;
  }
  const double t0 = ts + i * T_span, t1 = ts + (i + 1) * T_span;
  const int n = r->pwp.n_seg;
  const bool inr = lane <= n;
  const double tk = inr ? r->pwp.times[lane] : 0.0;
  if (inr) stimes[lane] = tk;
  int first = __popcll(__ballot(inr && tk < t0)) - 1;
  int last = __popcll(__ballot(inr && tk <= t1)) - 1;
  if (first < 0) first = 0; if (first > n - 1) first = n - 1;
  if (last < 0) last = 0; if (last > n - 1) last = n - 1;
  int nseg = last - first + 1; if (nseg < 0) nseg = 0;
  if (nseg > kHullCP / 4) { nseg = kHullCP / 4; if (lane == 0 && flags) atomicOr(flags, NEP_FLAG_HULL_OVERFLOW); }
  const int np0 = 4 * nseg;
  __syncthreads();
  if (lane < 2 * np0) {
    const int sl = lane >> 3, k = (lane >> 1) & 3, ax = lane & 1;
    const int s = first + sl;
    double _t;
    if (s != last) _t = stimes[s + 1] - stimes[s];
    else if (t1 > stimes[s + 1]) _t = stimes[s + 1] - stimes[s];
// ... 777 lines not shown
      if (!ok) { n_fail++; nd[0] = nd[1] = nd[2] = 0.0; }
      if (cull) {
        double worst = -NEP_INF;
#pragma unroll
        for (int k = 0; k < 4; k++) { const double v = (nd[0] * B4.x[k] + nd[1] * B4.y[k]) + (nd[2] - 1.0); if (v > worst) worst = v; }
        const double len = sqrt(nd[0] * nd[0] + nd[1] * nd[1]);
        far = !ok || -worst > sp.cull_radius * len;
      }
    }
    if (!cull) {
      if (active && a < sp.lines_cap) { bucket[3 * a] = nd[0]; bucket[3 * a + 1] = nd[1]; bucket[3 * a + 2] = nd[2]; }
    } else {
      const unsigned long long mn = __ballot(active && !far), mf = __ballot(active && far);
      const unsigned long long below = (1ull << lane) - 1ull;
      if (active) {
        const long pos = far ? (long)sp.lines_cap - 1 - (n_far + __popcll(mf & below)) : (long)n_near + __popcll(mn & below);
        if (pos >= 0 && pos < sp.lines_cap) { bucket[3 * pos] = nd[0]; bucket[3 * pos + 1] = nd[1]; bucket[3 * pos + 2] = nd[2]; }
      }
      n_near += __popcll(mn); n_far += __popcll(mf);
    }
  }
  for (int o = 32; o > 0; o >>= 1) n_fail += __shfl_xor(n_fail, o);
  if (lane == 0) {
    const bool spill = cull ? n_near + n_far > sp.lines_cap : n_att > sp.lines_cap;
    if (spill) { if (ps.flags) atomicOr(ps.flags, NEP_FLAG_LINES); if (n_near > sp.lines_cap) n_near = sp.lines_cap; if (n_far > sp.lines_cap - n_near) n_far = sp.lines_cap - n_near; }
    const int n_out = cull ? n_near : (n_att < sp.lines_cap ? n_att : sp.lines_cap);
    *cnt_out = spill ? -1 - n_out : n_out;
    if (ps.line_far) ps.line_far[(long)slot * NEP_MAX_POL + seg] = cull ? n_far : 0;
    if (ps.line_skip) ps.line_skip[(long)slot * NEP_MAX_POL + seg] = n_skip;
    lp_out[0] = n_att + n_skip; lp_out[1] = n_fail;
  }
}
template <int RULE>
__global__ __launch_bounds__(64, NEP_SEP_WAVES) void separator_kernel(SceneParams sp, ProblemSet ps, int pool_pairs) {
  if (!slot_active(sp, ps.active, blockIdx.x / NEP_MAX_POL)) return;
  separator_body<RULE>(sp, ps, pool_pairs, blockIdx.x / NEP_MAX_POL, blockIdx.x % NEP_MAX_POL, true);
}
__device__ __forceinline__ int wave_incl_scan(int v) {
  v += __builtin_amdgcn_update_dpp(0, v, 0x111, 0xf, 0xf, false);
  v += __builtin_amdgcn_update_dpp(0, v, 0x112, 0xf, 0xf, false);
  v += __builtin_amdgcn_update_dpp(0, v, 0x114, 0xf, 0xf, false);
  v += __builtin_amdgcn_update_dpp(0, v, 0x118, 0xf, 0xf, false);
  v += __builtin_amdgcn_update_dpp(0, v, 0x142, 0xa, 0xf, false);
  v += __builtin_amdgcn_update_dpp(0, v, 0x143, 0xc, 0xf, false);
  return v;
}
__host__ __device__ inline int sep_packed_cap(int n_plain) { return n_plain + 72 < 320 ? 320 : n_plain + 72; }
#ifdef NEP_SEP_PROF
__device__ unsigned long long g_sep_prof[16384 * 16];
#define SEP_PT(k) do { const long long t_ = clock64(); pa_[k] += t_ - pt_; pt_ = t_; } while (0)
#else
#define SEP_PT(k) do { } while (0)
#endif
__global__ __launch_bounds__(64, NEP_SEP_WAVES) void separator_packed_kernel(SceneParams sp, ProblemSet ps, int pool_pairs, int kSepPack) {
#ifdef NEP_SEP_PROF
  long long pt_ = clock64(); long long pa_[12] = {0, 0, 0, 0, 0, 0, 0, 0, 0, 0, 0, 0};
#endif
  const int kSepGroups = (NEP_MAX_POL + kSepPack - 1) / kSepPack;
  extern __shared__ __attribute__((aligned(16))) double sdyn[];
  const int rh = (sp.n_hull + 63) >> 6, rb = (sp.num_agents + 63) >> 6, rs = (sp.n_static + 63) >> 6, rounds = rh + rb + rs;
  double2* sA = (double2*)sdyn;
  double* sBx = sdyn + 2 * pool_pairs; double* sBy = sBx + 4 * NEP_MAX_POL;
  double* sEl = sBy + 4 * NEP_MAX_POL;
  double* sBb = sEl + 3 * NEP_MAX_POL;
  unsigned long long* sMask = (unsigned long long*)(sBb + 4 * NEP_MAX_POL);
  const bool ent_any = sp.ent_enabled && ps.case_id;
  unsigned long long* sEMask = sMask + 2 * NEP_MAX_POL * rounds;
  int* sCnt = (int*)(sEMask + (ent_any ? NEP_MAX_POL * rb : 0));
  unsigned short* sAtt = (unsigned short*)(sCnt + 6 * NEP_MAX_POL);
  const int lane = threadIdx.x;
  const int slot = blockIdx.x / kSepGroups, grp = blockIdx.x % kSepGroups;
  if (!slot_active(sp, ps.active, slot)) return;
  const int seg_lo = grp * kSepPack, seg_hi = seg_lo + kSepPack < NEP_MAX_POL ? seg_lo + kSepPack : NEP_MAX_POL;
  const nep_guess* g = ps.guess + slot;
  const int K = g->K;
  const double T = sp.T_span;
  SepCtx cx; cx.sp = &sp; cx.ps = &ps; cx.slot = slot; cx.scene = slot / sp.n_local; cx.own = sp.first_local + (slot % sp.n_local);
  cx.N = sp.num_agents; cx.S = sp.n_static; cx.nH = sp.n_hull;
  cx.total = cx.nH + cx.N + cx.S + ((sp.ent_enabled && ps.case_id) ? cx.N * kBend : 0);
  const bool cull = sp.cull_radius > 0.0 && ps.line_far != nullptr;
  cx.skip_box = cull ? ps.skip_box : nullptr; cx.skip_r = sp.cull_radius;
  const int total = cx.total, cap = sep_packed_cap(cx.nH + cx.N + cx.S);
  int seg_end = seg_hi < K ? seg_hi : K; if (seg_end > sp.num_pol) seg_end = sp.num_pol;
  if (lane < 6 * NEP_MAX_POL) sCnt[lane] = 0;
  if (lane < 4 * (seg_hi - seg_lo)) {
    const int seg = seg_lo + (lane >> 2), k = lane & 3;
    const double4 Px = *(const double4*)g->coeff[0][seg], Py = *(const double4*)g->coeff[1][seg];
    const double tp0 = T * T * T, tp1 = T * T, tp2 = T;
    const double m0 = tp0 * cAPosInv[0][k], m1 = tp1 * cAPosInv[1][k], m2 = tp2 * cAPosInv[2][k], m3 = 1.0 * cAPosInv[3][k];
    const double vx_ = ((Px.x * m0 + Px.y * m1) + Px.z * m2) + Px.w * m3, vy_ = ((Py.x * m0 + Py.y * m1) + Py.z * m2) + Py.w * m3;
    if (seg < seg_end) { sBx[seg * 4 + k] = vx_; sBy[seg * 4 + k] = vy_; }
  }
  __syncthreads();
  if (lane < 4 * (seg_hi - seg_lo) && seg_lo + (lane >> 2) < seg_end) {
    const int seg = seg_lo + (lane >> 2), k = lane & 3;
    const double* bx_ = sBx + seg * 4; const double* by_ = sBy + seg * 4;
    if (k < 3) { const double ex = bx_[k + 1] - bx_[k], ey = by_[k + 1] - by_[k]; sEl[seg * 3 + k] = sqrt(ex * ex + ey * ey); }
    const double* q_ = k < 2 ? bx_ : by_;
    sBb[seg * 4 + k] = (k & 1) ? fmax(fmax(q_[0], q_[1]), fmax(q_[2], q_[3])) : fmin(fmin(q_[0], q_[1]), fmin(q_[2], q_[3]));
  }
  __syncthreads();
  SEP_PT(0);
  const int nsv = seg_end - seg_lo;
  const int n_items = nsv > 0 ? nsv * rounds : 0;
  const bool reg_items = cx.total == cx.nH + cx.N + cx.S && n_items <= 64;
  unsigned long long my_a = 0ull, my_k = 0ull;
  auto put_mask = [&](int sg, int round, unsigned long long ma, unsigned long long mk) {
    if (reg_items) { if (lane == (sg - seg_lo) * rounds + round) { my_a = ma; my_k = mk; } }
    else if (lane == 0) { sMask[(sg * rounds + round) * 2] = ma; sMask[(sg * rounds + round) * 2 + 1] = mk; }
  };
  if (nsv > 0) {
    const double rr = cx.skip_r;
    for (int c0 = 0; c0 < cx.nH; c0 += 64) {
      const int j = c0 + lane; const bool in = j < cx.nH;
      const bool valid0 = in && !(sp.skip_own && j == cx.own);
      if (cx.skip_box) {
        const double2* q = (const double2*)(cx.skip_box + ((long)cx.scene * (cx.N + cx.S) + (in ? j : 0)) * sp.num_pol * 4);
        for (int s0 = seg_lo; s0 < seg_end; s0 += 8) {
          double2 qa[8], qb[8];
#pragma unroll
          for (int u = 0; u < 8; u++) { const int sg = s0 + u < seg_end ? s0 + u : seg_end - 1; qa[u] = q[sg * 2]; qb[u] = q[sg * 2 + 1]; }
#pragma unroll
          for (int u = 0; u < 8; u++) {
            const int sg = s0 + u;
            if (sg < seg_end) {
              const double* bb = sBb + sg * 4;
              const bool valid = valid0 && qa[u].x < NEP_INF;
              const bool far = (qa[u].x - bb[1] > rr) | (bb[0] - qa[u].y > rr) | (qb[u].x - bb[3] > rr) | (bb[2] - qb[u].y > rr);
              const unsigned long long ma = __ballot(valid && !far), mk = __ballot(valid && far);
              put_mask(sg, c0 >> 6, ma, mk);
            }
          }
        }
      } else {
        for (int sg = seg_lo; sg < seg_end; sg++) {
          int nA; int ord; const double2* unused = nullptr;
          const bool att = in && cand_eval(cx, sg, j, sBx + sg * 4, sBy + sg * 4, 0.0, 0, nullptr, nA, ord, unused);
          const unsigned long long ma = __ballot(att);
          put_mask(sg, c0 >> 6, ma, 0ull);
        }
      }
    }
    SEP_PT(1);
    for (int j0 = 0; j0 < cx.N; j0 += 64) {
      const int j = j0 + lane; const bool in = j < cx.N;
      constexpr double base_radius = 0.7;
      const double pbx = ps.pb[2 * (in ? j : 0)], pby = ps.pb[2 * (in ? j : 0) + 1];
      for (int sg = seg_lo; sg < seg_end; sg++) {
        const double* bx_ = sBx + sg * 4; const double* by_ = sBy + sg * 4;
        constexpr double kBaseNear2 = 0x1.1a3d70a3d70a2p+2;
        static_assert(base_radius * 3 == 0x1.0ccccccccccccp+1, "kBaseNear2 belongs to 0.7 * 3");
        bool close_to_base = false;
#pragma unroll
        for (int k = 0; k < 4; k++) { const double ddx = bx_[k] - pbx, ddy = by_[k] - pby; close_to_base |= ddx * ddx + ddy * ddy < kBaseNear2; }
        close_to_base &= in;
        const unsigned long long ma = __ballot(close_to_base);
        put_mask(sg, rh + (j0 >> 6), ma, 0ull);
      }
    }
    SEP_PT(2);
    const int spr = (cx.S > 0 && cx.S <= 32) ? 64 / cx.S : 1;
    for (int c0 = 0; c0 < cx.S; c0 += 64) {
      const int qs = spr > 1 ? lane / cx.S : 0;
      const int js = spr > 1 ? lane - qs * cx.S : c0 + lane; const bool in = js < cx.S && qs < spr;
      const long j = (long)cx.scene * sp.static_stride + (in ? js : 0);
      const int nv = in ? ps.static_nv[j] : 0;
      const double* src = ps.static_xy + j * kHullV * 2;
      const double sx0 = src[0], sy0 = src[1];
      const double* elp = ps.static_el + j * kHullV;
      const double e0 = elp[0], e1 = elp[1], e2 = elp[2];
      double perim = 0;
      if (nv > 1) perim += e0; if (nv > 2) perim += e1; if (nv > 3) perim += e2;
      for (int k = 3; k < nv - 1; k++) perim += elp[k];
      double2 qa = make_double2(0, 0), qb = qa;
      if (cx.skip_box) { const double2* q = (const double2*)(cx.skip_box + (((long)cx.scene * (cx.N + cx.S) + cx.N + (in ? js : 0)) * sp.num_pol + seg_lo) * 4); qa = q[0]; qb = q[1]; }
      for (int sg0 = seg_lo; sg0 < seg_end; sg0 += spr) {
        const int sg = sg0 + qs;
        const bool on = nv > 0 && sg < seg_end;
        const int sgc = sg < seg_end ? sg : seg_end - 1;
        const double* bb = sBb + sgc * 4;
        const double el0 = sEl[sgc * 3], el1 = sEl[sgc * 3 + 1], el2 = sEl[sgc * 3 + 2];
        bool close_s = false;
        const double ddx = sBx[sgc * 4] - sx0, ddy = sBy[sgc * 4] - sy0;
        const double d2s = ddx * ddx + ddy * ddy;
        const double thr = ((el0 + el1) + el2 + perim) * 1.000001 + 1e-6;
        if (__ballot(on && d2s <= thr * thr) != 0ull)
        if (on) {
          double dist = sqrt(d2s);
          dist -= el0; close_s |= dist < 0; dist -= el1; close_s |= dist < 0; dist -= el2; close_s |= dist < 0;
          if (nv > 1) { dist -= e0; close_s |= dist < 0; }
          if (nv > 2) { dist -= e1; close_s |= dist < 0; }
          if (nv > 3) { dist -= e2; close_s |= dist < 0; }
          for (int k = 3; k < nv - 1; k++) { dist -= elp[k]; close_s |= dist < 0; }
        }
        const bool far = cx.skip_box != nullptr && ((qa.x - bb[1] > rr) | (bb[0] - qa.y > rr) | (qb.x - bb[3] > rr) | (bb[2] - qb.y > rr));
        const unsigned long long ma = __ballot(close_s && !far), mk = __ballot(close_s && far);
        if (spr > 1) {
          const unsigned long long sm = (1ull << cx.S) - 1ull;
          for (int u = 0; u < spr && sg0 + u < seg_end; u++) put_mask(sg0 + u, rh + rb, (ma >> (u * cx.S)) & sm, (mk >> (u * cx.S)) & sm);
        } else put_mask(sg0, rh + rb + (c0 >> 6), ma, mk);
      }
      if (spr > 1) break;
    }
    if (ent_any) {
      for (int j0 = 0; j0 < cx.N; j0 += 256) {
        for (int s0 = seg_lo; s0 < seg_end; s0 += 8) {
          int cv[4][8];
#pragma unroll
          for (int w = 0; w < 4; w++) {
            const int j = j0 + 64 * w + lane;
            const int* cp = ps.case_id + ((long)cx.slot * NEP_MAX_POL + seg_lo) * cx.N + (j < cx.N ? j : 0);
#pragma unroll
            for (int u = 0; u < 8; u++) { const int sg = s0 + u < seg_end ? s0 + u : seg_end - 1; cv[w][u] = cp[(long)(sg - seg_lo) * cx.N]; }
          }
#pragma unroll
          for (int w = 0; w < 4; w++) {
            const int j = j0 + 64 * w + lane; const bool in = j < cx.N && j != cx.own;
            if (j0 + 64 * w < cx.N) {
#pragma unroll
              for (int u = 0; u < 8; u++) {
                if (s0 + u < seg_end) { const unsigned long long m = __ballot(in && cv[w][u] != 0); if (lane == 0) sEMask[(s0 + u) * rb + ((j0 >> 6) + w)] = m; }
              }
            }
          }
        }
      }
    }
    SEP_PT(3);
  }
  __syncthreads();
  int n_list = 0;
  auto flush = [&]() {
    __syncthreads();
    SEP_PT(4);
    for (int a0 = 0; a0 < n_list; a0 += 64) {
      const int a = a0 + lane;
      const bool active = a < n_list;
      const int e = active ? (int)sAtt[a] : 0;
      const int sl = e >> 13, c = e & 8191;
      Pts4 B4;
#pragma unroll
      for (int k = 0; k < 4; k++) { B4.x[k] = sBx[sl * 4 + k]; B4.y[k] = sBy[sl * 4 + k]; }
      double nd[3] = {0.0, 0.0, 0.0};
      bool far = false, ok = true;
      int nA = 0; int ord = 0;
      if (active) { const double2* u_ = nullptr; cand_eval(cx, sl, c, sBx, sBy, 0.0, 2, nullptr, nA, ord, u_); }
      const int incl = wave_incl_scan(nA);
      if (active) {
        double2 priv[4];
        double2* myA = (incl <= pool_pairs) ? sA + (incl - nA) : nullptr;
        const bool made_here = (c >= cx.nH && c < cx.nH + cx.N) || c >= cx.nH + cx.N + cx.S;
        if (!myA && made_here) myA = priv;
        const double2* Ause = myA;
        cand_eval(cx, sl, c, sBx, sBy, 0.0, 1, myA, nA, ord, Ause);
#ifdef NEP_SEP_PROF
        SEP_PT(5);
#endif
        ok = separator_impl(nA, Ause, ord, B4, nd);
#ifdef NEP_SEP_PROF
        SEP_PT(6);
#endif
        if (!ok) { nd[0] = nd[1] = nd[2] = 0.0; }
        if (cull) {
          double worst = -NEP_INF;
#pragma unroll
          for (int k = 0; k < 4; k++) { const double v = (nd[0] * B4.x[k] + nd[1] * B4.y[k]) + (nd[2] - 1.0); if (v > worst) worst = v; }
          const double len = sqrt(nd[0] * nd[0] + nd[1] * nd[1]);
          far = !ok || -worst > sp.cull_radius * len;
        }
      }
      {
        const unsigned long long below = (1ull << lane) - 1ull;
        const unsigned long long mact = __ballot(active), mn = __ballot(active && !far), mf = __ballot(active && far), mx = __ballot(active && !ok);
        const int sl_prev = __builtin_amdgcn_update_dpp(-1, sl, 0x138, 0xf, 0xf, false);
        const unsigned long long ms = __ballot(active && (lane == 0 || sl != sl_prev));
        const unsigned long long upto = ms & (below | (1ull << lane));
        const int s0_ = upto ? 63 - __clzll((long long)upto) : 0;
        const unsigned long long run_below = below & ~((1ull << s0_) - 1ull), run_incl = run_below | (1ull << lane);
        const bool last = active && (lane == 63 || (((~mact | ms) >> (lane + 1)) & 1ull));
        const int base_n = active ? sCnt[sl * 6] : 0, base_f = active ? sCnt[sl * 6 + 1] : 0;
        if (active) {
          double* bucket = ps.line_nd + ((long)slot * NEP_MAX_POL + sl) * sp.lines_cap * 3;
          const long pos = far ? (long)sp.lines_cap - 1 - (base_f + __popcll(mf & run_below)) : (long)base_n + __popcll(mn & run_below);
          if (pos >= 0 && pos < sp.lines_cap) { bucket[3 * pos] = nd[0]; bucket[3 * pos + 1] = nd[1]; bucket[3 * pos + 2] = nd[2]; }
        }
        __syncthreads();
        if (last) { sCnt[sl * 6] = base_n + __popcll(mn & run_incl); sCnt[sl * 6 + 1] = base_f + __popcll(mf & run_incl); sCnt[sl * 6 + 2] += __popcll(mx & run_incl); }
        __syncthreads();
      }
      SEP_PT(7);
    }
    n_list = 0;
  };
  int seg = seg_lo - 1, ph = 4, c0 = 0, n_att = 0, n_skip = 0, n_act = 0;
  const int n_plain = cx.nH + cx.N + cx.S;
  const double* bx = sBx; const double* by = sBy;
  double hulldist = 0;
  int tag = 0;
  unsigned short* sAct = sAtt + cap;
  bool more = true;
  const bool ent_c = n_plain < total;
  int it_sg = seg_lo, it_r = 0;
  if (!ent_c && !reg_items && lane < nsv) {
    int na_ = 0, nk_ = 0;
    for (int r = 0; r < rounds; r++) { na_ += __popcll(sMask[((seg_lo + lane) * rounds + r) * 2]); nk_ += __popcll(sMask[((seg_lo + lane) * rounds + r) * 2 + 1]); }
    sCnt[(seg_lo + lane) * 6 + 3] = na_; sCnt[(seg_lo + lane) * 6 + 4] = nk_;
  }
  bool placed = false;
  if (reg_items) {
    const int cnt_ = __popcll(my_a), cntk_ = __popcll(my_k);
    const int incl_ = wave_incl_scan(cnt_), inclk_ = wave_incl_scan(cntk_);
    const int tot_ = __builtin_amdgcn_readlane(incl_, 63);
    {
      const int hi_ = lane < nsv ? (lane + 1) * rounds - 1 : 0, lo_ = (lane < nsv && lane > 0) ? lane * rounds - 1 : 0;
      const int a_hi = __shfl(incl_, hi_), k_hi = __shfl(inclk_, hi_), a_lo = __shfl(incl_, lo_), k_lo = __shfl(inclk_, lo_);
      if (lane < nsv) { sCnt[(seg_lo + lane) * 6 + 3] = a_hi - (lane > 0 ? a_lo : 0); sCnt[(seg_lo + lane) * 6 + 4] = k_hi - (lane > 0 ? k_lo : 0); }
    }
    if (tot_ <= cap) {
      const int sgi_ = lane / rounds, r_ = lane - sgi_ * rounds;
      const int cb_ = r_ < rh ? (r_ << 6) : (r_ < rh + rb ? cx.nH + ((r_ - rh) << 6) : cx.nH + cx.N + ((r_ - rh - rb) << 6));
      const int ebase_ = ((seg_lo + sgi_) << 13) | cb_, off_ = incl_ - cnt_;
      { unsigned long long m_ = my_a; int o_ = off_; while (m_) { const int b_ = __builtin_ctzll(m_); m_ &= m_ - 1ull; sAtt[o_++] = (unsigned short)(ebase_ + b_); } }
      n_list = tot_; placed = true;
    } else {
      if (lane < n_items) { sMask[(seg_lo * rounds + lane) * 2] = my_a; sMask[(seg_lo * rounds + lane) * 2 + 1] = my_k; }
      __syncthreads();
    }
  }
  while (more) {
    if (!ent_c) {
      if (placed) it_sg = seg_end;
      for (; it_sg < seg_end; ) {
        if (n_list > 0 && n_list + 64 > cap) break;
        const unsigned long long mv = sMask[(it_sg * rounds + it_r) * 2];
        const unsigned mlo = __builtin_amdgcn_readfirstlane((unsigned)mv), mhi = __builtin_amdgcn_readfirstlane((unsigned)(mv >> 32));
        const int cb_ = it_r < rh ? (it_r << 6) : (it_r < rh + rb ? cx.nH + ((it_r - rh) << 6) : cx.nH + cx.N + ((it_r - rh - rb) << 6));
        const unsigned rank = __builtin_amdgcn_mbcnt_hi(mhi, __builtin_amdgcn_mbcnt_lo(mlo, 0u));
        if ((((lane & 32) ? mhi : mlo) >> (lane & 31)) & 1u) sAtt[n_list + rank] = (unsigned short)((it_sg << 13) | (cb_ + lane));
        n_list += __popc(mlo) + __popc(mhi);
        if (++it_r == rounds) { it_r = 0; it_sg++; }
      }
      if (it_sg >= seg_end) more = false;
    } else
    for (;;) {
      if (ph == 4) {
        if (seg >= seg_lo && seg < seg_end && lane == 0) { sCnt[seg * 6 + 3] = n_att; sCnt[seg * 6 + 4] = n_skip; }
        seg++;
        if (seg >= seg_end) { more = false; break; }
        bx = sBx + seg * 4; by = sBy + seg * 4; tag = seg << 13;
        hulldist = 0;
        for (int k = 0; k < 3; k++) { cx.el[k] = sEl[seg * 3 + k]; hulldist += cx.el[k]; }
// ... 11 lines not shown
        }
        if (n_list > 0 && n_list + tot_seg > cap) break;
        for (int r0 = 0; r0 < rounds; r0 += 64) {
          const int r = r0 + lane;
          unsigned long long m_ = r < rounds ? sMask[(seg * rounds + r) * 2] : 0ull;
          const int cnt_ = __popcll(m_), incl_ = wave_incl_scan(cnt_);
          const int cb_ = r < rh ? (r << 6) : (r < rh + rb ? cx.nH + ((r - rh) << 6) : cx.nH + cx.N + ((r - rh - rb) << 6));
          int o_ = n_list + incl_ - cnt_;
          while (m_) { const int b_ = __builtin_ctzll(m_); m_ &= m_ - 1ull; sAtt[o_++] = (unsigned short)(tag | (cb_ + b_)); }
          n_list += __builtin_amdgcn_readlane(incl_, 63);
        }
        n_att += tot_seg; n_skip += skip_seg;
        ph = n_plain < total ? 2 : 4;
      } else if (ph == 2) {
        SEP_PT(4);
        n_act = 0;
        __syncthreads();
        for (int ch = 0; ch < rb; ch++) {
          const unsigned long long mask = sEMask[seg * rb + ch];
          if ((mask >> lane) & 1ull) sAct[n_act + __popcll(mask & ((1ull << lane) - 1ull))] = (unsigned short)((ch << 6) + lane);
          n_act += __popcll(mask);
        }
        __syncthreads();
        ph = 3; c0 = 0;
        SEP_PT(9);
      } else {
        SEP_PT(4);
        const int n_pairs = n_act * kBend;
        int nr = (n_pairs - c0 + 63) >> 6; if (nr > 4) nr = 4;
        while (nr > 1 && n_list + 64 * nr > cap) nr--;
        int cid[4], nbv[4], h0n[4], jj[4]; double2 X[4], Y[4], Z[4];
#pragma unroll
        for (int u = 0; u < 4; u++) {
          const int pp = c0 + 64 * u + lane; const bool in = u < nr && pp < n_pairs;
          const int j = in ? (int)sAct[pp / kBend] : 0, k = pp % kBend + 1;
          jj[u] = j;
          const HullRef hr = hull_ref(ps, cx.N, cx.scene, j);
          cid[u] = ps.case_id[((long)cx.slot * NEP_MAX_POL + seg) * cx.N + j];
          nbv[u] = blk(ps.bend_n, hr.boff)[hr.e];
          const double2* bp = (const double2*)(blk(ps.bend_xy, hr.boff) + hr.e * kBend * 2);
          const long h0 = hr.e * sp.num_pol + seg;
          h0n[u] = blk(ps.hull0_nv, hr.boff)[h0];
          X[u] = k == 1 ? ((const double2*)blk(ps.hull0_xy, hr.boff))[h0] : bp[k - 2];
          Y[u] = bp[k - 1];
        }
#pragma unroll
        for (int u = 0; u < 4; u++) {
          const int pp = c0 + 64 * u + lane; const int k = pp % kBend + 1;
          const HullRef hr = hull_ref(ps, cx.N, cx.scene, jj[u]);
          const double2* bp = (const double2*)(blk(ps.bend_xy, hr.boff) + hr.e * kBend * 2);
          int nbc = nbv[u]; if (nbc < 1) nbc = 1; if (nbc > kBend) nbc = kBend;
          Z[u] = bp[k == 1 ? nbc - 1 : 0];
        }
#pragma unroll
        for (int u = 0; u < 4; u++) {
          if (u < nr) {
            const int pp = c0 + 64 * u + lane; const int k = pp % kBend + 1;
            bool att = pp < n_pairs && cid[u] != 0 && k != cid[u] && k <= nbv[u];
            double pAx, pAy, pBx, pBy;
            if (k == 1) {
              att = att && h0n[u] > 0;
              pAx = (1 - sp.long_length) * Z[u].x + sp.long_length * X[u].x; pAy = (1 - sp.long_length) * Z[u].y + sp.long_length * X[u].y;
              pBx = X[u].x; pBy = X[u].y;
            } else { pAx = X[u].x; pAy = X[u].y; pBx = Y[u].x; pBy = Y[u].y; }
            const double ax_ = pAx - bx[0], ay_ = pAy - by[0], bx_ = pBx - bx[0], by_ = pBy - by[0];
            const double d2a = ax_ * ax_ + ay_ * ay_, d2b = bx_ * bx_ + by_ * by_;
            const double h2 = hulldist * hulldist, h2hi = h2 * (1.0 + 1e-12), h2lo = h2 * (1.0 - 1e-12);
            bool ga = d2a > h2hi, gb = d2b > h2hi;
            if (__ballot(att && ((!ga && !(d2a < h2lo)) || (!gb && !(d2b < h2lo)))) != 0ull) { ga = sqrt(d2a) - hulldist > 0; gb = sqrt(d2b) - hulldist > 0; }
            if (att && ga && gb) att = false;
            const int c = n_plain + jj[u] * kBend + (k - 1);
            const unsigned long long mask = __ballot(att);
            if (att) sAtt[n_list + __popcll(mask & ((1ull << lane) - 1ull))] = (unsigned short)(tag | c);
            n_list += __popcll(mask); n_att += __popcll(mask);
          }
        }
        c0 += 64 * nr;
        SEP_PT(10);
      }
    }
    flush();
  }
  __syncthreads();
  if (lane < seg_hi - seg_lo) {
    const int seg = seg_lo + lane;
    const long o = (long)slot * NEP_MAX_POL + seg;
    int cn_ = sCnt[seg * 6], cf_ = sCnt[seg * 6 + 1];
    bool spill_ = false;
    if (cn_ + cf_ > sp.lines_cap) { spill_ = true; if (ps.flags) atomicOr(ps.flags, NEP_FLAG_LINES); if (cn_ > sp.lines_cap) cn_ = sp.lines_cap; if (cf_ > sp.lines_cap - cn_) cf_ = sp.lines_cap - cn_; }
    ps.line_cnt[o] = spill_ ? -1 - cn_ : cn_;
    if (ps.line_far) ps.line_far[o] = cf_;
    if (ps.line_skip) ps.line_skip[o] = sCnt[seg * 6 + 4];
    ps.lp_stats[o * 2] = sCnt[seg * 6 + 3] + sCnt[seg * 6 + 4]; ps.lp_stats[o * 2 + 1] = sCnt[seg * 6 + 2];
  }
  SEP_PT(8);
#ifdef NEP_SEP_PROF
  if (lane == 0 && blockIdx.x < 16384) { for (int k = 0; k < 12; k++) g_sep_prof[blockIdx.x * 16 + k] += (unsigned long long)pa_[k]; g_sep_prof[blockIdx.x * 16 + 15] += 1ull; }
#endif
}
#ifdef NEP_SEP_PROF
extern "C" int nep_debug_sep_prof(unsigned long long* out16, int reset) {
  std::vector<unsigned long long> h((size_t)16384 * 16);
  (void)hipMemcpyFromSymbol(h.data(), HIP_SYMBOL(g_sep_prof), h.size() * 8);
  if (out16) { for (int k = 0; k < 16; k++) out16[k] = 0; for (size_t b = 0; b < 16384; b++) for (int k = 0; k < 16; k++) out16[k] += h[b * 16 + k]; }
  if (reset) { std::fill(h.begin(), h.end(), 0ull); (void)hipMemcpyToSymbol(HIP_SYMBOL(g_sep_prof), h.data(), h.size() * 8); }
  return 0;
}
#endif

template <int RULE>
__global__ __launch_bounds__(64, NEP_SEP_WAVES) void separator_redo_kernel(SceneParams sp, ProblemSet ps, int pool_pairs) {
  const int n = *ps.redo_count * NEP_MAX_POL;
  for (int i = blockIdx.x; i < n; i += gridDim.x) {
    separator_body<RULE>(sp, ps, pool_pairs, ps.redo_list[i / NEP_MAX_POL], i % NEP_MAX_POL, false);
    __syncthreads();
  }
}

size_t separator_lds_bytes(const SceneParams& sp) {
  const int total = sp.n_hull + sp.num_agents + sp.n_static + (sp.ent_enabled ? sp.num_agents * kBend : 0);
  const size_t tail = 8 * sizeof(double) + (((size_t)(total + 8 + (sp.ent_enabled ? sp.num_agents : 0)) * sizeof(unsigned short) + 15) & ~(size_t)15);
  size_t pool = tail + 64 * 8 * 16 <= (size_t)kSepLdsTarget ? (size_t)kSepLdsTarget - tail : (size_t)64 * 8 * 16;
  pool &= ~(size_t)15;
  return pool + tail;
}
static int separator_pool_pairs(const SceneParams& sp) {
  const int total = sp.n_hull + sp.num_agents + sp.n_static + (sp.ent_enabled ? sp.num_agents * kBend : 0);
  const size_t tail = 8 * sizeof(double) + (((size_t)(total + 8 + (sp.ent_enabled ? sp.num_agents : 0)) * sizeof(unsigned short) + 15) & ~(size_t)15);
  return (int)((separator_lds_bytes(sp) - tail) / 16);
}

void launch_separator(int n_slots, const SceneParams& sp, const ProblemSet& ps, hipStream_t st) {
  if (n_slots <= 0) return;
  const int total = sp.n_hull + sp.num_agents + sp.n_static + (sp.ent_enabled ? sp.num_agents * kBend : 0);
  if (((ps.skip_box && ps.line_far && sp.cull_radius > 0.0 && ps.sep_pack >= 0) || (sp.cull_radius == 0.0 && ps.sep_pack >= 1)) && sp.sep_rule == 0 && total <= 8191) {
    const size_t rounds_ = (size_t)((sp.n_hull + 63) / 64 + (sp.num_agents + 63) / 64 + (sp.n_static + 63) / 64);
    const size_t extras = 15 * NEP_MAX_POL * sizeof(double) + 2 * NEP_MAX_POL * rounds_ * sizeof(unsigned long long) + 6 * NEP_MAX_POL * sizeof(int)
                          + ((sp.ent_enabled && ps.case_id) ? (size_t)NEP_MAX_POL * ((sp.num_agents + 63) / 64) * sizeof(unsigned long long) : 0)
                          + (size_t)(sep_packed_cap(sp.n_hull + sp.num_agents + sp.n_static) + (sp.ent_enabled ? sp.num_agents : 0)) * sizeof(unsigned short);
    size_t pool_b = extras + 64 * 6 * 16 <= (size_t)kSepLdsTarget ? (size_t)kSepLdsTarget - extras : (size_t)64 * 6 * 16;
    pool_b &= ~(size_t)15;
    const int pairs = (int)(pool_b / 16);
    const size_t lds_p = (pool_b + extras + 15) & ~(size_t)15;
    static DynLdsAttr attr_p;
    (void)attr_p.ensure((const void*)separator_packed_kernel, lds_p);
    int pack = 1; while (pack < NEP_MAX_POL && (long)n_slots * (NEP_MAX_POL / (pack * 2)) >= 4096) pack *= 2;
    if (ps.sep_pack >= 1 && ps.sep_pack <= NEP_MAX_POL) pack = ps.sep_pack;
    const int groups = (NEP_MAX_POL + pack - 1) / pack;
    hipLaunchKernelGGL(separator_packed_kernel, dim3(n_slots * groups), dim3(64), lds_p, st, sp, ps, pairs, pack);
    return;
  }
  const size_t lds = separator_lds_bytes(sp);
  static DynLdsAttr attr[2];
  if (sp.sep_rule == 1) {
    (void)attr[1].ensure((const void*)separator_kernel<1>, lds);
    hipLaunchKernelGGL(separator_kernel<1>, dim3(n_slots * NEP_MAX_POL), dim3(64), lds, st, sp, ps, separator_pool_pairs(sp));
  } else {
    (void)attr[0].ensure((const void*)separator_kernel<0>, lds);
    hipLaunchKernelGGL(separator_kernel<0>, dim3(n_slots * NEP_MAX_POL), dim3(64), lds, st, sp, ps, separator_pool_pairs(sp));
  }
}
void launch_separator_redo(int n_slots, const SceneParams& sp, const ProblemSet& ps, hipStream_t st) {
  if (n_slots <= 0 || !ps.redo_count || !ps.redo_list) return;
  const size_t lds = separator_lds_bytes(sp);
  static DynLdsAttr attr[2];
  const int grid = n_slots * NEP_MAX_POL < 1024 ? n_slots * NEP_MAX_POL : 1024;
  if (sp.sep_rule == 1) {
    (void)attr[1].ensure((const void*)separator_redo_kernel<1>, lds);
    hipLaunchKernelGGL(separator_redo_kernel<1>, dim3(grid), dim3(64), lds, st, sp, ps, separator_pool_pairs(sp));
  } else {
    (void)attr[0].ensure((const void*)separator_redo_kernel<0>, lds);
    hipLaunchKernelGGL(separator_redo_kernel<0>, dim3(grid), dim3(64), lds, st, sp, ps, separator_pool_pairs(sp));
  }
}

__global__ void separator_explicit_kernel(int n_prob, const int* __restrict__ a_off, const double* __restrict__ a_xy,
                                          const int* __restrict__ b_off, const double* __restrict__ b_xy,
                                          double* __restrict__ nd_out, int* __restrict__ solved, int rule) {
  const int p = blockIdx.x * blockDim.x + threadIdx.x;
  if (p >= n_prob) return;
  double2 A[kHullV];
  Pts4 B;
  int nA = a_off[p + 1] - a_off[p];
  if (nA > kHullV) nA = kHullV;
  for (int i = 0; i < nA; i++) A[i] = make_double2(a_xy[2 * (a_off[p] + i)], a_xy[2 * (a_off[p] + i) + 1]);
  for (int i = 0; i < 4; i++) { B.x[i] = b_xy[2 * (b_off[p] + i)]; B.y[i] = b_xy[2 * (b_off[p] + i) + 1]; }
  double nd[3];
  const bool ok = rule == 1 ? separator_glpk_class(nA, A, B, nd) : separator_impl(nA, A, 0, B, nd);
  nd_out[3 * p] = nd[0]; nd_out[3 * p + 1] = nd[1]; nd_out[3 * p + 2] = nd[2];
  solved[p] = ok ? 1 : 0;
}

void launch_separator_explicit(int n_prob, const int* a_off, const double* a_xy, const int* b_off,
                               const double* b_xy, double* nd, int* solved, int rule, hipStream_t st) {
  if (n_prob <= 0) return;
  hipLaunchKernelGGL(separator_explicit_kernel, dim3((n_prob + 63) / 64), dim3(64), 0, st, n_prob, a_off, a_xy, b_off, b_xy, nd, solved, rule);
}

__global__ __launch_bounds__(64) void hull_explicit_kernel(const nep_traj_rec* __restrict__ recs, double t_start, int num_pol,
                                                           double T_span, double drone_radius,
                                                           double* __restrict__ hull_xy, int* __restrict__ hull_nv,
                                                           double* __restrict__ hull0_xy, int* __restrict__ hull0_nv, int* __restrict__ flags) {
  const int i = blockIdx.x % num_pol;
  const int jt = blockIdx.x / num_pol;
  hull_body(recs + jt, t_start, i, T_span, drone_radius, (long)jt * num_pol + i, true, hull_xy, hull_nv, hull0_xy, hull0_nv, flags);
}

void launch_hulls_explicit(const nep_traj_rec* recs, int n_traj, double t_start, int num_pol,
                           double T_span, double drone_radius, double* hull_xy, int* hull_nv,
                           double* hull0_xy, int* hull0_nv, int* flags, hipStream_t st) {
  if (n_traj * num_pol <= 0) return;
  hipLaunchKernelGGL(hull_explicit_kernel, dim3(n_traj * num_pol), dim3(64), 0, st, recs, t_start, num_pol, T_span,
                     drone_radius, hull_xy, hull_nv, hull0_xy, hull0_nv, flags);
}

template <class VP> __device__ __forceinline__ int gjk_furthest(int n, VP V, double dx, double dy) {
  double mx = dx * V[0] + dy * V[1]; int idx = 0;
  for (int i = 1; i < n; i++) { const double p = dx * V[2 * i] + dy * V[2 * i + 1]; if (p > mx) { mx = p; idx = i; } }
  return idx;
}
__device__ __forceinline__ void gjk_furthest4(const Pts4& B, double dx, double dy, double& px, double& py) {
  double mx = dx * B.x[0] + dy * B.y[0]; px = B.x[0]; py = B.y[0];
#pragma unroll
  for (int i = 1; i < 4; i++) { const double p = dx * B.x[i] + dy * B.y[i]; if (p > mx) { mx = p; px = B.x[i]; py = B.y[i]; } }
}
template <class VP> __device__ bool gjk_collision(int n1, VP V1, const Pts4& B) {
  if (n1 <= 0) return false;
  double p1x = 0, p1y = 0, p2x = 0, p2y = 0;
  for (int i = 0; i < n1; i++) { p1x += V1[2 * i]; p1y += V1[2 * i + 1]; }
#pragma unroll
  for (int i = 0; i < 4; i++) { p2x += B.x[i]; p2y += B.y[i]; }
  p1x /= n1; p1y /= n1; p2x /= 4; p2y /= 4;
  double dx = p1x - p2x, dy = p1y - p2y;
  if (dx == 0 && dy == 0) dx = 1.0;
// ... 1299 lines not shown
```

neptune_amd/csrc/nep_device.h:

```cpp
#pragma once
#include <hip/hip_runtime.h>

#include <mutex>

#include "nep_tables.h"
#include "../../include/neptune_frontend.h"
#include "../../include/neptune_fleet.h"
#include "../../include/neptune_backend_debug.h"

namespace nep {

constexpr int kHullV = NEP_HULL_MAX_V;
constexpr int kHullCP = NEP_HULL_MAX_CP;
constexpr int kBend = NEP_MAX_BEND;

struct DebugGlobals { bool fe_three = false; int fe_xcd = 1; int polish_grid = 256; };
extern DebugGlobals g_debug;

constexpr int kCorrFromItDefault = 10, kCorrMaxCountDefault = 8;
struct SceneParams {
  int num_agents;
  int num_pol;
  int n_static;
  int n_hull;
  int ent_enabled;
  int hull_mode;
  int max_states;
  int lines_cap;
  int n_local;
  int first_local;
  int skip_own;
  int static_stride;
  double T_span, weight, dc, drone_radius;
  double mins[3], maxs[3], v_max, a_max;
  double long_length;
  double cull_radius;
  long long time_limit_ticks;
  int corr_from_it, corr_max_count;
  double tol_res, tol_gap, tol_res_inv, tol_gap_inv, tol_gap_floor;
  int sep_rule;
  int qp_key_decay;
  int fe_key_decay;
  double us_per_tick;
};

struct ProblemSet {
  const nep_guess* guess;
  const double* pb;
  const double* static_xy;
  const int* static_nv;
  const double* static_el;
  const int* case_id;
  double* hull_xy;
  int* hull_nv;
  double* hull0_xy;
  int* hull0_nv;
  double* bend_xy;
  int* bend_n;
  int hull_pb;
  unsigned long long hull_pb_magic;
  long hull_bstride;
  double* line_nd;
  int* line_cnt;
  int* line_far;
  int* lp_stats;
  const double* skip_box;
  int* line_skip;
  int* redo_list;
  int* redo_count;
  const int* order_count;
  int lines_override;
  int sep_pack;
  const int* order;
  int* order_key;
  const int* fe_order;
  int* fe_order_key;
  float* fe_us;
  double* row_scratch;
  int scratch_chunks;
  int scratch_by_block;
  int rows_cap;
  int lds_rows;
  int lds_lines;
  nep_solution* solution;
  double* states;
  nep_traj_rec* commit;
  const nep_traj_rec* prev_commit;
  double* polish_z;
  int* polish_flag;
  int* polish_list; int* polish_count;
  int* presolved;
  long long* dbg;
  int* flags;
  double* fe_box;
  const int* active;
  const int* fe_count;
};
__device__ __forceinline__ bool slot_active(const SceneParams& sp, const int* active, int slot) {
  return active == nullptr || active[(long)(slot / sp.n_local) * sp.num_agents + sp.first_local + slot % sp.n_local] != 0;
}
constexpr int NEP_FLAG_MISSION = 128;
constexpr int NEP_FLAG_FLEET = 64;
constexpr int NEP_FLAG_ENT_TRACK = 32;
constexpr int NEP_FLAG_ENT_POOL = 16;
constexpr int NEP_FLAG_LINES = 8;
constexpr int NEP_FLAG_SCRATCH = 4;
constexpr int NEP_FLAG_ENT_BETA = 2;
constexpr int NEP_FLAG_HULL_OVERFLOW = 1;

__host__ __device__ inline int line_count(int stored) { return stored < 0 ? -1 - stored : stored; }
struct HullRef { long e; long boff; };
__host__ __device__ inline HullRef hull_ref(const ProblemSet& ps, int per_scene, int scene, int j) {
  if (ps.hull_pb <= 0) return HullRef{(long)scene * per_scene + j, 0L};
  const int b = ps.hull_pb_magic ? (int)(((unsigned long long)(unsigned)j * ps.hull_pb_magic) >> 32) : j / ps.hull_pb;
  return HullRef{(long)scene * ps.hull_pb + (j - b * ps.hull_pb), (long)b * ps.hull_bstride};
}
template <typename T> __host__ __device__ inline T* blk(T* base, long boff) { return (T*)((char*)base + boff); }

struct DynLdsAttr {
  std::mutex mu; size_t configured[64] = {};
  hipError_t ensure(const void* fn, size_t bytes) {
    int dev = 0;
    if (hipGetDevice(&dev) != hipSuccess || dev < 0 || dev >= 64) return hipFuncSetAttribute(fn, hipFuncAttributeMaxDynamicSharedMemorySize, (int)bytes);
    std::lock_guard<std::mutex> lk(mu);
    if (bytes <= configured[dev]) return hipSuccess;
    const hipError_t e = hipFuncSetAttribute(fn, hipFuncAttributeMaxDynamicSharedMemorySize, (int)bytes);
    if (e == hipSuccess) configured[dev] = bytes;
    return e;
  }
};

struct SampleSched {
  const int* n;
  const int* seg;
  const double* dt;
};

bool hulls_grouped(const SceneParams& sp, int n_scenes, int n_rec);
void launch_hulls(const nep_traj_rec* recs, int n_scenes, int n_rec, const nep_guess* guess,
                  const SceneParams& sp, const ProblemSet& ps, hipStream_t st, bool boxes = false);
void launch_hulls_ts(const nep_traj_rec* recs, int n_scenes, int n_rec, const double* ts0, long ts_slot_stride,
                     const SceneParams& sp, const ProblemSet& ps, hipStream_t st, bool boxes = false);
void launch_hulls_explicit(const nep_traj_rec* recs, int n_traj, double t_start, int num_pol,
                           double T_span, double drone_radius, double* hull_xy, int* hull_nv,
                           double* hull0_xy, int* hull0_nv, int* flags, hipStream_t st);
void launch_separator(int n_slots, const SceneParams& sp, const ProblemSet& ps, hipStream_t st);
void launch_separator_redo(int n_slots, const SceneParams& sp, const ProblemSet& ps, hipStream_t st);
void launch_boxes(int n_scenes, const SceneParams& sp, const ProblemSet& ps, hipStream_t st);
void launch_active_rows(int n_slots, const SceneParams& sp, const ProblemSet& ps, double tol, int* out, hipStream_t st);
void launch_separator_explicit(int n_prob, const int* a_off, const double* a_xy, const int* b_off,
                               const double* b_xy, double* nd, int* solved, int rule, hipStream_t st);
void launch_qp(int n_slots, const SceneParams& sp, const ProblemSet& ps, const QpTable* tables,
               const SampleSched& sched, size_t lds_bytes, hipStream_t st);
size_t qp_lds_fixed_bytes();
void launch_qp_order(int n_slots, const int* key, int* order, hipStream_t st, int* zero_these = nullptr);
void launch_qp_polish_zero(int* counters, hipStream_t st);
void launch_order_xcd(int n_slots, const int* key, int* order, hipStream_t st);
void launch_qp_reg(int n_slots, const SceneParams& sp, const ProblemSet& ps, const QpTable* tables,
                   const SampleSched& sched, size_t lds_bytes, hipStream_t st);
void launch_qp_polish(int n_slots, const SceneParams& sp, const ProblemSet& ps, const QpTable* tables, const SampleSched& sched, hipStream_t st);
void launch_qp_presolve(int n_slots, const SceneParams& sp, const ProblemSet& ps, const QpTable* tables, const SampleSched& sched, int* presolved, hipStream_t st);
int qp_reg_slots();
size_t qp_reg_lds_bytes();
struct EntBigPool { unsigned char* base; int* count; int n_rec; int rec_bytes; int cap; int add_lim; };
__host__ __device__ inline int ent_big_cap(int N, int S, int mult = 1) { int c = (N + S) * mult; if (c < NEP_FE_ENT_CAP) c = NEP_FE_ENT_CAP; return (c + 3) & ~3; }
__host__ __device__ inline int ent_big_add_lim(int N, int S, int mult = 1) { return ((N + S) * mult + 2 + 31) & ~31; }
__host__ __device__ inline int ent_big_rec_bytes(int N, int S, int mult = 1) { const int c = ent_big_cap(N, S, mult), a = ent_big_add_lim(N, S, mult); return (((8 + 13 * c + 3) & ~3) + 4 * a + a / 8 + 7) & ~7; }
struct FeEntArgs {
  const double* sampled;
  const int* present;
  const double* srep;
  const double* slong;
  const nep_fe_ent_state* init;
  nep_fe_ent_state* nodes;
  nep_fe_ent_state* work;
  nep_fe_ent_state* saved;
  double* saved_arc;
  double* st_f; long long* st_vox;
  int* case_out;
  int ns;
  double* packed;
  int pk_stride;
  EntBigPool big;
  EntBigPool big_check;
  int big_lds_off;
  double* big_beta;
  int* redo_list; int* redo_count; int redo_cap;
  unsigned* xpool; int xpool_stride;
  int fast_cap, fast_add, fast_bend;
};
size_t frontend_children_cap(const nep_fe_cfg& fc, int num_pol);
size_t frontend_ent_xpool_words(const SceneParams& sp, const nep_fe_cfg& fc, int ent_ns);
void launch_frontend(int n_slots, const SceneParams& sp, const ProblemSet& ps, const nep_fe_cfg& fc, const nep_fe_start* starts,
                     nep_guess* guess_out, nep_fe_result* res_out, const FeEntArgs* ea, hipStream_t st, int* order_buf = nullptr, bool have_history = false,
                     int* active_buf = nullptr);
void launch_ent_sample(const nep_traj_rec* recs, int n_scenes, int N, const double* ts0, long ts_scene_stride, int num_pol, int ns, double T_span,
                       double* sampled, int* present, hipStream_t st, int* zero_this = nullptr);
struct AuditPart { double c_d2, box, stat; int c_k, c_p, b_k, b_p, s_k, s_i, n_pair, n_stat; };
struct AuditArgs {
  int N, S, n_scenes, static_stride, vstride, n_ticks, chunk_len, n_chunks;
  double tick, drone_radius;
  const nep_traj_rec* recs;
  const nep_fe_start* starts;
  const double* static_xy;
  const int* static_nv;
  AuditPart* part;
  nep_audit* out;
};
size_t audit_lds_bytes(int N, int S, int vstride);
void launch_audit(const AuditArgs& aa, hipStream_t st);
struct FleetArgs {
  int N, n_scenes, cap, max_states;
  nep_fleet_cfg cfg;
  double drone_radius;
  const double* pb;
  double* ring;
  int* head; int* size; int* k_end;
  double* state;
  double* goal;
  nep_pwp* pwp;
  int* flown; int* done; int* outcome; int* sflags;
  const int* period; const int* phase;
  double* t_now; int* round;
  int* counters;
  int* gflags;
  nep_fe_start* start; nep_traj_rec* recs; int* active_out; nep_fe_start* clock;
  const nep_solution* sol; const double* states_in; const nep_fe_result* fres; const int* accept; int* outcome_out;
  const int* active;
};
// ... 68 lines not shown
```

neptune_amd/csrc/nep_tables.h:

```cpp
#pragma once
#include <algorithm>
#include <cmath>
#include <cstring>
#include <vector>

#include "../../include/neptune_backend.h"

namespace nep {

static const double kAPosInv[4][4] = {
    {-0.03203276669713047, -0.09273093424558249, 0.3420572455666699, 1.1023313949144335},
    {-0.05111494245568798, -0.046272612998418894, 0.5458234872124772, 1.0979806946005568},
    {-0.07454781852812224, 0.203951949894552, 0.796048050105448, 1.0745478185281223},
    {1.0, 1.0, 0.9999999999999996, 0.9999999999999993}};
static const double kAVelInv[3][3] = {
    {-0.07735026918962577, 0.16666666666666635, 1.077350269189625},
    {-0.07735026918962577, 0.49999999999999967, 1.077350269189625},
    {1.0000000000000002, 1.0000000000000009, 1.0000000000000016}};

constexpr int kMaxK = NEP_MAX_POL;
constexpr int kMaxR = 8 * kMaxK;
constexpr int kNZ = 8;

struct QpTable {
  int K, nz, R, mode;
  double B[kMaxR][kNZ];
  double U[kMaxR][3];
  double Th[4 * kMaxK][kNZ];
  double ThU[4 * kMaxK][3];
  double Hax[kNZ][kNZ];
  double RowMap[kMaxR][4];
  double ThMap[4 * kMaxK][4];
  double ObjQ[4][4];
  double Gi[kNZ][3];
  double ep[kNZ], ev[kNZ], ea[kNZ];
  double up[3], uv[3], ua[3];
  double Nt[kNZ][kMaxK];
  double Pp[kMaxK][3];
  double res_u[2][3];
  double Zp[kNZ][4 * kMaxK];
  double HaxInv[kNZ][kNZ];
};

struct SampleTable {
  int n;
  int seg[1];
};

inline void build_qp_table(int K, double T, double weight, int mode, QpTable* t) {
  std::memset(t, 0, sizeof(*t));
  double M4[4][4], V3[3][3];
  const double tp[4] = {T * T * T, T * T, T, 1.0};
  const double tv[3] = {T * T, T, 1.0}, m321[3] = {3.0, 2.0, 1.0};
  for (int j = 0; j < 4; j++) for (int k = 0; k < 4; k++) M4[j][k] = tp[j] * kAPosInv[j][k];
  for (int j = 0; j < 3; j++) for (int k = 0; k < 3; k++) V3[j][k] = m321[j] * (tv[j] * kAVelInv[j][k]);
  std::vector<double> Phi(4 * K * K, 0.0), PhiU(4 * K * 3, 0.0);
  double ba[3][kMaxK] = {{0}}, bu[3][3] = {{1, 0, 0}, {0, 1, 0}, {0, 0, 1}};
  for (int i = 0; i < K; i++) {
    Phi[(4 * i + 0) * K + i] = 1.0;
    for (int r = 0; r < 3; r++) {
      for (int c = 0; c < K; c++) Phi[(4 * i + 1 + r) * K + c] = ba[r][c];
      for (int c = 0; c < 3; c++) PhiU[(4 * i + 1 + r) * 3 + c] = bu[r][c];
    }
    double na[3][kMaxK], nu[3][3];
    for (int c = 0; c < K; c++) {
      double e = (c == i) ? 1.0 : 0.0;
      na[0][c] = ba[0][c] + 3 * T * e;
      na[1][c] = ba[1][c] + 2 * T * ba[0][c] + 3 * T * T * e;
      na[2][c] = ba[2][c] + T * ba[1][c] + T * T * ba[0][c] + T * T * T * e;
    }
    for (int c = 0; c < 3; c++) {
      nu[0][c] = bu[0][c];
      nu[1][c] = bu[1][c] + 2 * T * bu[0][c];
      nu[2][c] = bu[2][c] + T * bu[1][c] + T * T * bu[0][c];
    }
    std::memcpy(ba, na, sizeof(ba)); std::memcpy(bu, nu, sizeof(bu));
  }
  int nz;
  std::vector<double> N(K * kNZ, 0.0), Pp(K * 3, 0.0);
  if (mode == 1) {
    nz = K;
    for (int i = 0; i < K; i++) N[i * kNZ + i] = 1.0;
  } else {
    nz = K > 2 ? K - 2 : 0;
    const double* e0 = ba[0]; const double* e1 = ba[1];
    double g00 = 0, g01 = 0, g11 = 0;
    for (int c = 0; c < K; c++) { g00 += e0[c] * e0[c]; g01 += e0[c] * e1[c]; g11 += e1[c] * e1[c]; }
    if (K >= 2) {
      double det = g00 * g11 - g01 * g01;
      double i00 = g11 / det, i01 = -g01 / det, i11 = g00 / det;
      for (int c = 0; c < K; c++) {
        double p0 = e0[c] * i00 + e1[c] * i01, p1 = e0[c] * i01 + e1[c] * i11;
        for (int u = 0; u < 3; u++) Pp[c * 3 + u] = -(p0 * bu[0][u] + p1 * bu[1][u]);
      }
    } else {
      double den = e0[0] * e0[0] + e1[0] * e1[0];
      for (int u = 0; u < 3; u++) Pp[u] = -(e0[0] * bu[0][u] + e1[0] * bu[1][u]) / den;
// ... 122 lines not shown
```

neptune_amd/csrc/qp_outputs.h:

```cpp
#pragma once
#include "nep_device.h"

namespace nep {

__device__ __forceinline__ int sched_states(const SceneParams& sp, const SampleSched& sched, int K) {
  const int ns_all = sched.n[K];
  return ns_all < sp.max_states ? ns_all : sp.max_states;
}

__device__ __forceinline__ void sample_state(const double* theta, int i, double dt, double* st) {
  for (int ax = 0; ax < 3; ax++) {
    const double* c = theta + (ax * NEP_MAX_POL + i) * 4;
    st[ax] = ((c[0] * (dt * dt * dt) + c[1] * (dt * dt)) + c[2] * dt) + c[3];
    st[3 + ax] = (c[0] * (3 * dt * dt) + c[1] * (2 * dt)) + c[2];
    st[6 + ax] = c[0] * (6 * dt) + c[1] * 2;
    st[9 + ax] = c[0] * 6;
  }
}

template <int NT>
__device__ __forceinline__ void write_states(const SceneParams& sp, const ProblemSet& ps, const SampleSched& sched, int slot, const double* theta, int K, int ns, int tid) {
  if (!ps.states) return;
  for (int s = tid; s < ns; s += NT)
    sample_state(theta, sched.seg[K * sp.max_states + s], sched.dt[K * sp.max_states + s], ps.states + ((long)slot * sp.max_states + s) * NEP_STATE_DOUBLES);
}

template <int NT>
__device__ __forceinline__ void write_trajectory(nep_solution* sol, const double* theta, int K, const double* t_start, double T, int tid) {
  for (int t = tid; t < 3 * NEP_MAX_POL * 4; t += NT) (&sol->coeff[0][0][0])[t] = ((t % (NEP_MAX_POL * 4)) / 4 < K) ? theta[t] : 0.0;
  if (tid <= NEP_MAX_POL) sol->times[tid] = (tid <= K) ? *t_start + tid * T : 0.0;
}

template <int NT>
__device__ __forceinline__ void write_commit(const SceneParams& sp, const ProblemSet& ps, int slot, const double* theta, int K, const double* t_start, double T, int tid) {
  nep_traj_rec* cr = ps.commit + slot;
  const int own = sp.first_local + (slot % sp.n_local);
  if (tid == 0) {
    cr->id = own + 1; cr->is_agent = 1; cr->n_bend = 1; cr->valid = 1;
    for (int a = 0; a < 3; a++) { cr->bbox[a] = 2 * sp.drone_radius; cr->pos[a] = theta[(a * NEP_MAX_POL) * 4 + 3]; }
    cr->bend[0][0] = ps.pb[2 * own]; cr->bend[0][1] = ps.pb[2 * own + 1];
    cr->pwp.n_seg = K;
  }
  if (tid <= NEP_TRAJ_MAX_SEG) cr->pwp.times[tid] = (tid <= K) ? *t_start + tid * T : 0.0;
  for (int e = tid; e < 3 * NEP_TRAJ_MAX_SEG * 4; e += NT) {
    const int ax = e / (NEP_TRAJ_MAX_SEG * 4), r = e % (NEP_TRAJ_MAX_SEG * 4), seg = r / 4, j = r % 4;
    (&cr->pwp.coeff[0][0][0])[e] = (seg < K) ? theta[(ax * NEP_MAX_POL + seg) * 4 + j] : 0.0;
  }
}

template <int NT>
__device__ __forceinline__ void carry_commit(const SceneParams& sp, const ProblemSet& ps, int slot, int tid) {
  if (!ps.prev_commit) return;
  const int own = sp.first_local + (slot % sp.n_local);
  const double* src = (const double*)(ps.prev_commit + (long)(slot / sp.n_local) * sp.num_agents + own);
  double* dst = (double*)(ps.commit + slot);
  for (int e = tid; e < (int)(sizeof(nep_traj_rec) / sizeof(double)); e += NT) dst[e] = src[e];
}

__device__ __forceinline__ void lp_totals(const ProblemSet& ps, int slot, int& n_lp, int& n_lpf) {
  n_lp = 0; n_lpf = 0;
  if (ps.lp_stats && !ps.lines_override) {
    int v[2 * NEP_MAX_POL];
#pragma unroll
    for (int i = 0; i < 2 * NEP_MAX_POL; i++) v[i] = ps.lp_stats[(long)slot * NEP_MAX_POL * 2 + i];
#pragma unroll
    for (int i = 0; i < NEP_MAX_POL; i++) { n_lp += v[2 * i]; n_lpf += v[2 * i + 1]; }
  }
}

__device__ __forceinline__ void write_solve_time(const SceneParams& sp, const ProblemSet& ps, nep_solution* sol, int slot, long long t_wg0) {
  const long long dt_ = (long long)wall_clock64() - t_wg0;
  const double us_ = (double)dt_ * sp.us_per_tick;
  sol->stats.solve_us = us_;
  if (ps.order_key) {
    const double k_ = us_ * 0.125;
    const int kn = k_ > 63.0 ? 63 : (int)k_, ko = ps.order_key[slot] - sp.qp_key_decay;
    ps.order_key[slot] = (sp.qp_key_decay > 0 && ko > kn) ? ko : kn;
  }
}

}
```

neptune_amd/csrc/qp_presolve_kernel.hip:

```cpp
#include <hip/hip_runtime.h>

#include "nep_device.h"
#include "nep_tables.h"
#include "qp_outputs.h"

namespace nep {

namespace {
__constant__ double cPreAPosInv[4][4] = {
    {-0.03203276669713047, -0.09273093424558249, 0.3420572455666699, 1.1023313949144335},
    {-0.05111494245568798, -0.046272612998418894, 0.5458234872124772, 1.0979806946005568},
    {-0.07454781852812224, 0.203951949894552, 0.796048050105448, 1.0745478185281223},
    {1.0, 1.0, 0.9999999999999996, 0.9999999999999993}};

__device__ __forceinline__ double pre_wave_max(double v) {
#pragma unroll
  for (int o = 32; o > 0; o >>= 1) v = fmax(v, __shfl_xor(v, o));
  return v;
}
__device__ __forceinline__ double pre_wave_sum(double v) {
#pragma unroll
  for (int o = 32; o > 0; o >>= 1) v += __shfl_xor(v, o);
  return v;
}
}

#ifndef NEP_PRE_WAVES
#define NEP_PRE_WAVES 6
#endif
__global__ __launch_bounds__(64, NEP_PRE_WAVES) void qp_presolve_kernel(SceneParams sp, ProblemSet ps, const QpTable* __restrict__ tables, SampleSched sched, int* __restrict__ presolved) {
  __builtin_amdgcn_s_setprio(3);
  const int lane = threadIdx.x;
  if (ps.order_count && (int)blockIdx.x >= *ps.order_count) return;
  const int slot = ps.order_count ? ps.order[blockIdx.x] : (int)blockIdx.x;
  const long long t0 = (long long)wall_clock64();
  __shared__ double sCoef[96], sTheta[96], sA[2 * 32];
  __shared__ int sCnt[3 * NEP_MAX_POL + 4];
  const nep_guess* __restrict__ g = ps.guess + slot;
  nep_solution* __restrict__ sol = ps.solution + slot;
  const int K = g->K;
  const double T = sp.T_span;
  if (lane == 0) presolved[slot] = 0;
  if (K < 3 || K > NEP_MAX_POL || K > sp.num_pol) return;
  const int R = 8 * K;
  const QpTable* __restrict__ tb = tables + K;

  int cn = 0, cf = 0, cs = 0; bool ovf = false;
  if (lane < NEP_MAX_POL && lane < K) {
    const int raw = ps.line_cnt[(long)slot * NEP_MAX_POL + lane];
    ovf = raw < 0; cn = line_count(raw);
    cf = ps.line_far[(long)slot * NEP_MAX_POL + lane];
    cs = ps.line_skip ? ps.line_skip[(long)slot * NEP_MAX_POL + lane] : 0;
  }
  const double c_lo = (&g->coeff[0][0][0])[lane], c_hi = lane + 64 < 96 ? (&g->coeff[0][0][0])[lane + 64] : 0.0;
  double rm0 = 0, rm1 = 0, rm2 = 0, rm3 = 0, tm0 = 0, tm1 = 0, tm2 = 0, tm3 = 0;
  if (lane < R) { const double* q = tb->RowMap[lane]; rm0 = q[0]; rm1 = q[1]; rm2 = q[2]; rm3 = q[3]; }
  if (lane < 4 * K) { const double* q = tb->ThMap[lane]; tm0 = q[0]; tm1 = q[1]; tm2 = q[2]; tm3 = q[3]; }
  int lpv = 0;
  if (ps.lp_stats && lane < 2 * NEP_MAX_POL) lpv = ps.lp_stats[(long)slot * NEP_MAX_POL * 2 + lane];
  double vv[3][4];
#pragma unroll
  for (int ax = 0; ax < 3; ax++) {
    const double* c0 = g->coeff[ax][0]; const double* cK = g->coeff[ax][K - 1];
    vv[ax][0] = c0[1]; vv[ax][1] = c0[2]; vv[ax][2] = c0[3];
    vv[ax][3] = ((T * T * T) * cK[0] + (T * T) * cK[1] + T * cK[2]) + cK[3];
  }
  if (__ballot(ovf) != 0ull) return;
  sCoef[lane] = c_lo; if (lane + 64 < 96) sCoef[lane + 64] = c_hi;
  if (lane < NEP_MAX_POL) { sCnt[lane] = cn; sCnt[NEP_MAX_POL + lane] = cf; sCnt[2 * NEP_MAX_POL + lane] = cs; }
  const double dix = vv[0][2] - vv[0][3], diy = vv[1][2] - vv[1][3], diz = vv[2][2] - vv[2][3];
  const bool has_qc = sqrt(dix * dix + diy * diy + diz * diz) < 1.0;
  const bool z_override = sqrt(dix * dix + diy * diy) < 1.0;

  double viol = -1.0;
  if (lane < R) {
#pragma unroll
    for (int ax = 0; ax < 3; ax++) {
      const double a = ((rm0 * vv[ax][0] + rm1 * vv[ax][1]) + rm2 * vv[ax][2]) + rm3 * vv[ax][3];
      const double hi = lane < 4 * K ? sp.maxs[ax] : (lane < 7 * K ? sp.v_max : sp.a_max);
      const double lo = lane < 4 * K ? sp.mins[ax] : (lane < 7 * K ? -sp.v_max : -sp.a_max);
      viol = fmax(viol, fmax(a - hi, lo - a));
      if (ax < 2 && lane < 4 * K) sA[ax * 32 + lane] = a;
    }
  }
  sTheta[lane] = 0.0; if (lane + 64 < 96) sTheta[lane + 64] = 0.0;
  __syncthreads();
  if (lane < 4 * K) {
#pragma unroll
    for (int ax = 0; ax < 3; ax++) sTheta[(ax * 8 + lane / 4) * 4 + (lane % 4)] = ((tm0 * vv[ax][0] + tm1 * vv[ax][1]) + tm2 * vv[ax][2]) + tm3 * vv[ax][3];
  }
  __syncthreads();
  int L_near = 0, n_far = 0, n_skip = 0;
#pragma unroll
  for (int i = 0; i < NEP_MAX_POL; i++) { L_near += sCnt[i]; n_far += sCnt[NEP_MAX_POL + i]; n_skip += sCnt[2 * NEP_MAX_POL + i]; }
#pragma unroll 2
  for (int e = lane; e < L_near; e += 64) {
    int i = 0, off = 0, acc = 0;
#pragma unroll
    for (int j = 0; j < NEP_MAX_POL - 1; j++) { acc += sCnt[j]; if (e >= acc) { i = j + 1; off = acc; } }
    const double* nd = ps.line_nd + (((long)slot * NEP_MAX_POL + i) * sp.lines_cap + (e - off)) * 3;
    const double n1 = nd[0], n2 = nd[1], h = 1.0 - nd[2];
#pragma unroll
    for (int k = 0; k < 4; k++) viol = fmax(viol, (n1 * sA[4 * i + k] + n2 * sA[32 + 4 * i + k]) - h);
  }
  if (has_qc) {
    double c = -0.10 * 0.10;
#pragma unroll
    for (int ax = 0; ax < 3; ax++) { const double* q = sTheta + (ax * 8 + (K - 1)) * 4; const double pe = (((T * T * T) * q[0] + (T * T) * q[1] + T * q[2]) + q[3]) - vv[ax][3]; c += pe * pe; }
    viol = fmax(viol, c);
  }
  bool bad = false;
  if (lane < 8 * K) {
    const int rho = lane >> 1, ax = lane & 1, sg = rho >> 2, k = rho & 3;
    const double c0 = (T * T * T) * cPreAPosInv[0][k], c1 = (T * T) * cPreAPosInv[1][k], c2 = T * cPreAPosInv[2][k], c3 = cPreAPosInv[3][k];
    const double* Q = sTheta + (ax * 8 + sg) * 4;
    const double v = ((Q[0] * c0 + Q[1] * c1) + Q[2] * c2) + Q[3] * c3;
    const double* P = sCoef + (ax * 8 + sg) * 4;
    const double gq = ((P[0] * c0 + P[1] * c1) + P[2] * c2) + P[3] * c3;
    double d2 = (v - gq) * (v - gq);
    d2 += __shfl_xor(d2, 1);
    bad = (n_far > 0 || n_skip > 0) && !(d2 <= sp.cull_radius * sp.cull_radius * (1.0 - 1e-9));
  }
  if (!(pre_wave_max(viol) <= 0.0)) return;
  if (__ballot(bad) != 0ull) return;

  int n_lp = (lane & 1) == 0 ? lpv : 0, n_lpf = (lane & 1) == 1 ? lpv : 0;
#pragma unroll
  for (int o_ = 8; o_ > 0; o_ >>= 1) { n_lp += __shfl_xor(n_lp, o_); n_lpf += __shfl_xor(n_lpf, o_); }
  if (z_override) { if (lane < 32) sTheta[64 + lane] = sCoef[64 + lane]; }
  __syncthreads();
  write_trajectory<64>(sol, sTheta, K, &g->t_start, T, lane);
  const int ns = sched_states(sp, sched, K);
  if (lane == 0) {
    double o = 0;
    for (int ax = 0; ax < 3; ax++) for (int a = 0; a < 4; a++) { double r_ = 0; for (int b = 0; b < 4; b++) r_ += tb->ObjQ[a][b] * vv[ax][b]; o += vv[ax][a] * r_; }
    const int L_all = L_near + n_far + n_skip;
    sol->stats.status = NEP_OK; sol->stats.iters = 0; sol->stats.iters_first = 0;
    sol->stats.n_lines = L_all - n_lpf; sol->stats.n_lp = n_lp; sol->stats.n_lp_failed = n_lpf;
    sol->stats.n_rows = 48 * K + 4 * (L_near < L_all ? L_near : L_near - n_lpf); sol->stats.qc_active = has_qc ? 1 : 0;
    sol->stats.objective = o;
    sol->K = K; sol->n_states = ns;
  }
  if (lane == 0) {
    const double us_ = (double)((long long)wall_clock64() - t0) * sp.us_per_tick;
    sol->stats.solve_us = us_;
    if (ps.order_key) { const int ko = ps.order_key[slot] - sp.qp_key_decay; ps.order_key[slot] = (sp.qp_key_decay > 0 && ko > 0) ? ko : 0; }
    presolved[slot] = 1;
  }
}

void launch_qp_presolve(int n_slots, const SceneParams& sp, const ProblemSet& ps, const QpTable* tables, const SampleSched& sched, int* presolved, hipStream_t st) {
  if (n_slots <= 0 || !presolved) return;
  hipLaunchKernelGGL(qp_presolve_kernel, dim3(n_slots), dim3(64), 0, st, sp, ps, tables, sched, presolved);
}

}
```

Before: 20.87 million replans/s.

## Fuse QP presolve certification into the packed separator kernel

Moves the line-presolve certificate check into the packed separator kernel. It evaluates the start state and the near-line violations while the lines are generated, then writes the presolved trajectory directly, so the separate presolve kernel launch is skipped. That launch also reread the line normals from global memory. The presolve code is factored into a shared header, and the standalone kernel's occupancy hint changes from 6 to 4 waves. The cost is extra LDS and registers in the separator kernel, which could lower its occupancy.

Measured after the change: 21.11 million replans/s (median of 6 runs). 1.1% higher.

```diff
diff --git a/include/neptune_backend_debug.h b/include/neptune_backend_debug.h
--- a/include/neptune_backend_debug.h
+++ b/include/neptune_backend_debug.h
@@ -54,11 +54,13 @@
   NEP_PATH_FUSED_ORDER = 8,
   NEP_PATH_ORDERED_QP = 16,
   NEP_PATH_PRESOLVE_KERNEL = 32,
-  NEP_PATH_REDO_PASS = 64
+  NEP_PATH_REDO_PASS = 64,
+  NEP_PATH_FUSED_PRESOLVE = 128
 };
 int nep_batch_debug_launch_path(nep_batch_t* h, int32_t* bits);
 int nep_batch_debug_boxes(nep_batch_t* h, int32_t scene, double* out, int32_t cap);
 int nep_batch_debug_order_keys(nep_batch_t* h, int32_t* keys, int32_t cap);
+int nep_batch_debug_presolved(nep_batch_t* h, int32_t* marks, int32_t cap);
 
 int nep_batch_debug_hulls(nep_batch_t* h, int32_t scene, double* hull_xy, int32_t* hull_nv);
 int nep_batch_debug_lines(nep_batch_t* h, int32_t slot, int32_t cap, int32_t* seg, double* nd,
diff --git a/neptune_amd/_lib.py b/neptune_amd/_lib.py
--- a/neptune_amd/_lib.py
+++ b/neptune_amd/_lib.py
@@ -33,7 +33,7 @@
     "nep_batch_kernel_time", "nep_batch_enable_timing", "nep_batch_reset_timing", "nep_batch_debug_hulls",
     "nep_batch_debug_lines", "nep_batch_debug_phase_cycles", "nep_batch_fe_search_us",
     "nep_batch_set_fe_ent_fast_caps", "nep_batch_debug_set_option", "nep_backend_debug_set_option", "nep_debug_set_global_option",
-    "nep_batch_debug_launch_path", "nep_batch_debug_boxes", "nep_batch_debug_order_keys", "nep_debug_live_bytes",
+    "nep_batch_debug_launch_path", "nep_batch_debug_boxes", "nep_batch_debug_order_keys", "nep_batch_debug_presolved", "nep_debug_live_bytes",
 ]
 PLAN_EXPORTS = [
     "nep_pwp_compose", "nep_pwp_compose_exact", "nep_dyntraj_wire_size", "nep_dyntraj_encode", "nep_dyntraj_decode", "nep_plan_create",
@@ -134,6 +134,7 @@
     L.nep_batch_debug_launch_path.argtypes = [vp, pi]
     L.nep_batch_debug_boxes.argtypes = [vp, i, pd, i]
     L.nep_batch_debug_order_keys.argtypes = [vp, pi, i]
+    L.nep_batch_debug_presolved.argtypes = [vp, pi, i]
     L.nep_debug_live_bytes.argtypes = [C.POINTER(C.c_int64), C.POINTER(C.c_int64)]
     L.nep_batch_set_scene_statics.argtypes = [vp, i, i, pi, pd]
     L.nep_batch_check.argtypes = [vp, vp]
diff --git a/neptune_amd/backend.py b/neptune_amd/backend.py
--- a/neptune_amd/backend.py
+++ b/neptune_amd/backend.py
@@ -489,7 +489,7 @@
         return out[:n.value].copy() if n.value else None
 
     LAUNCH_PATH = (("box_kernel", 1), ("grouped_hulls", 2), ("fused_boxes", 4), ("fused_order", 8), ("ordered_qp", 16),
-                   ("presolve_kernel", 32), ("redo_pass", 64))
+                   ("presolve_kernel", 32), ("redo_pass", 64), ("fused_presolve", 128))
 
     def debug_launch_path(self):
         b = C.c_int32(0)
@@ -504,6 +504,11 @@
     def debug_order_keys(self):
         out = np.zeros(self.slots, dtype=np.int32)
         check(lib().nep_batch_debug_order_keys(self._h, abi.iptr(out), len(out)))
+        return out
+
+    def debug_presolved(self):
+        out = np.zeros(self.slots, dtype=np.int32)
+        check(lib().nep_batch_debug_presolved(self._h, abi.iptr(out), len(out)))
         return out
 
     def set_max_runtime(self, seconds):
diff --git a/neptune_amd/csrc/backend.hip b/neptune_amd/csrc/backend.hip
--- a/neptune_amd/csrc/backend.hip
+++ b/neptune_amd/csrc/backend.hip
@@ -120,7 +120,7 @@
   DevBuf<double> d_pb, d_static_xy, d_static_el; DevBuf<int> d_static_nv;
   DevBuf<double> d_hull_xy, d_hull0_xy, d_bend_xy, d_line_nd, d_row_scratch;
   DevBuf<int> d_hull_nv, d_hull0_nv, d_bend_n, d_line_cnt, d_line_far, d_lp_stats;
-  DevBuf<int> d_presolved; bool presolve_kernel = true;
+  DevBuf<int> d_presolved; bool presolve_kernel = true, presolve_fused = true;
   DevBuf<int> d_line_skip, d_redo_list, d_redo_count;
   DevBuf<double> d_polish_z; DevBuf<int> d_polish_flag, d_polish_list, d_polish_count; bool polish = true, polish_presolve = true, last_polish_armed = false;
   DevBuf<long long> d_dbg; bool profile_phases = false;
@@ -288,7 +288,7 @@
     ps.sep_pack = sep_pack;
     ps.row_scratch = d_row_scratch.p; ps.rows_cap = rows_cap; ps.lds_rows = lds_rows; ps.lds_lines = lds_lines;
     ps.dbg = profile_phases ? d_dbg.p : nullptr;
-    ps.presolved = nullptr;
+    ps.presolved = nullptr; ps.pre_tables = nullptr; ps.pre_sched_n = nullptr;
     ps.flags = d_flags.p;
     ps.fe_box = d_fe_box.p;
     ps.active = active; ps.fe_count = nullptr;
@@ -412,9 +412,18 @@
       ps.row_scratch = d_row_scratch.p;
     }
     const bool skip = ps.skip_box != nullptr;
+    const bool pre = qp && use_reg && presolve_kernel && ps.line_far != nullptr && !ps.lines_override && d_presolved.n >= (size_t)slots;
+    const bool fused_pre = pre && presolve_fused && phases == 3 && !ps.active && skip && sp.cull_radius > 0.0 && (!want_order || fused_order)
+                           && separator_pack(slots, sp, ps) == NEP_MAX_POL;
     if (!ps.lines_override && geo) {
       if (skip && !fused_boxes) { launch_boxes(n_scenes, sp, ps, st); last_path |= NEP_PATH_BOX_KERNEL; }
+      if (fused_pre) {
+        ps.presolved = d_presolved.p; ps.pre_tables = d_tables.p; ps.pre_sched_n = d_sched_n.p;
+        ps.order_key = (lpt && d_order_key.n >= (size_t)slots) ? d_order_key.p : nullptr;
+        last_path |= NEP_PATH_PRESOLVE_KERNEL | NEP_PATH_FUSED_PRESOLVE;
+      }
       launch_separator(slots, sp, ps, st);
+      ps.pre_tables = nullptr; ps.pre_sched_n = nullptr;
     }
     if (timing) hipEventRecord(next_event(), st);
     if (!qp) { if (timing) hipEventRecord(next_event(), st); HIPCHK(hipGetLastError()); return 0; }
@@ -430,7 +439,7 @@
       ps.order = d_act.p; ps.order_count = d_act.p + slots;
       launch_skipped_replan(slots, sp, ps, st);
     }
-    if (use_reg && presolve_kernel && ps.line_far != nullptr && !ps.lines_override && d_presolved.n >= (size_t)slots) {
+    if (pre && !fused_pre) {
       ps.presolved = d_presolved.p;
       launch_qp_presolve(slots, sp, ps, d_tables.p, sc, d_presolved.p, st);
       last_path |= NEP_PATH_PRESOLVE_KERNEL;
@@ -1872,6 +1881,15 @@
   HIPCHK(hipMemcpy(out, E.d_fe_box.p + (size_t)scene * n, n * sizeof(double), hipMemcpyDeviceToHost));
   return 0;
 }
+int nep_batch_debug_presolved(nep_batch_t* h, int32_t* marks, int32_t cap) {
+  if (!h || !marks || cap < 0) return fail(NEP_E_ARG, "bad arguments");
+  if (cap < h->slots) return fail(NEP_E_CAP, "mark buffer smaller than the slot count");
+  if (!h->eng.d_presolved.p || h->eng.d_presolved.n < (size_t)h->slots) return fail(NEP_E_STATE, "the handle has no certificate marks");
+  HIPCHK(hipDeviceSynchronize());
+  HIPCHK(hipMemcpy(marks, h->eng.d_presolved.p, (size_t)h->slots * sizeof(int), hipMemcpyDeviceToHost));
+  return 0;
+}
+
 int nep_batch_debug_order_keys(nep_batch_t* h, int32_t* keys, int32_t cap) {
   if (!h || !keys || cap < 0) return fail(NEP_E_ARG, "bad arguments");
   if (cap < h->slots) return fail(NEP_E_CAP, "key buffer smaller than the slot count");
@@ -1896,6 +1914,7 @@
   else if (n == "corr_max") { if (v < 1) return fail(NEP_E_ARG, "corr_max >= 1"); E.opt_corr_max = v; E.sp.corr_max_count = v; }
   else if (n == "fleet_ent_proof") E.opt_fleet_ent_proof = v != 0;
   else if (n == "qp_profile") E.profile_phases = v != 0;
+  else if (n == "presolve_fused") E.presolve_fused = v != 0;
   else if (n == "presolve_kernel") E.presolve_kernel = v != 0;
   else return fail(NEP_E_ARG, "unknown debug option: " + n);
   return 0;
diff --git a/neptune_amd/csrc/geom_kernels.hip b/neptune_amd/csrc/geom_kernels.hip
--- a/neptune_amd/csrc/geom_kernels.hip
+++ b/neptune_amd/csrc/geom_kernels.hip
@@ -6,14 +6,11 @@
 #include "nep_device.h"
 #include "../../include/neptune_frontend.h"
 #include "ent_device.h"
+#include "qp_presolve.h"
 
 namespace nep {
 
-__constant__ double cAPosInv[4][4] = {
-    {-0.03203276669713047, -0.09273093424558249, 0.3420572455666699, 1.1023313949144335},
-    {-0.05111494245568798, -0.046272612998418894, 0.5458234872124772, 1.0979806946005568},
-    {-0.07454781852812224, 0.203951949894552, 0.796048050105448, 1.0745478185281223},
-    {1.0, 1.0, 0.9999999999999996, 0.9999999999999993}};
+__constant__ double cAPosInv[4][4] = NEP_APOS_INV_LITERALS;
 
 #define SEP_MIN_GAP 1e-7
 #define NEP_INF (__builtin_huge_val())
@@ -957,6 +954,9 @@
   cx.skip_box = cull ? ps.skip_box : nullptr; cx.skip_r = sp.cull_radius;
   const int total = cx.total, cap = sep_packed_cap(cx.nH + cx.N + cx.S);
   int seg_end = seg_hi < K ? seg_hi : K; if (seg_end > sp.num_pol) seg_end = sp.num_pol;
+  const bool cert = ps.pre_tables != nullptr && K >= 3 && K <= NEP_MAX_POL && K <= sp.num_pol;
+  double* sPre = sdyn + (((const char*)(sAtt + cap + (sp.ent_enabled ? sp.num_agents : 0)) - (const char*)sdyn + 7) >> 3);
+  PreStart pre; pre.viol = -1.0; pre.th[0] = pre.th[1] = pre.th[2] = 0.0; pre.obj = 0.0; pre.moved = false; pre.has_qc = false; pre.z_override = false;
   if (lane < 6 * NEP_MAX_POL) sCnt[lane] = 0;
   if (lane < 4 * (seg_hi - seg_lo)) {
     const int seg = seg_lo + (lane >> 2), k = lane & 3;
@@ -1103,6 +1103,7 @@
     }
     SEP_PT(3);
   }
+  if (cert) pre = pre_start(sp, ps.pre_tables + K, g, K, lane, sPre, sdyn, cAPosInv);
   __syncthreads();
   int n_list = 0;
   auto flush = [&]() {
@@ -1142,6 +1143,7 @@
           for (int k = 0; k < 4; k++) { const double v = (nd[0] * B4.x[k] + nd[1] * B4.y[k]) + (nd[2] - 1.0); if (v > worst) worst = v; }
           const double len = sqrt(nd[0] * nd[0] + nd[1] * nd[1]);
           far = !ok || -worst > sp.cull_radius * len;
+          if (cert && !far) pre.viol = fmax(pre.viol, pre_line_viol(nd[0], nd[1], nd[2], sPre + sl * 4, sPre + 32 + sl * 4));
         }
       }
       {
@@ -1319,16 +1321,32 @@
     flush();
   }
   __syncthreads();
+  int cn_ = 0, cf_ = 0;
+  bool spill_ = false;
   if (lane < seg_hi - seg_lo) {
     const int seg = seg_lo + lane;
     const long o = (long)slot * NEP_MAX_POL + seg;
-    int cn_ = sCnt[seg * 6], cf_ = sCnt[seg * 6 + 1];
-    bool spill_ = false;
+    cn_ = sCnt[seg * 6]; cf_ = sCnt[seg * 6 + 1];
     if (cn_ + cf_ > sp.lines_cap) { spill_ = true; if (ps.flags) atomicOr(ps.flags, NEP_FLAG_LINES); if (cn_ > sp.lines_cap) cn_ = sp.lines_cap; if (cf_ > sp.lines_cap - cn_) cf_ = sp.lines_cap - cn_; }
     ps.line_cnt[o] = spill_ ? -1 - cn_ : cn_;
     if (ps.line_far) ps.line_far[o] = cf_;
     if (ps.line_skip) ps.line_skip[o] = sCnt[seg * 6 + 4];
     ps.lp_stats[o * 2] = sCnt[seg * 6 + 3] + sCnt[seg * 6 + 4]; ps.lp_stats[o * 2 + 1] = sCnt[seg * 6 + 2];
+  }
+  if (ps.pre_tables) {
+    bool done = false;
+    if (cert && __ballot(spill_) == 0ull) {
+      const long long t0 = (long long)wall_clock64();
+      int L_near = cn_, n_far = cf_, n_sk = (lane < NEP_MAX_POL && ps.line_skip) ? sCnt[lane * 6 + 4] : 0;
+#pragma unroll
+      for (int o_ = 4; o_ > 0; o_ >>= 1) { L_near += __shfl_xor(L_near, o_); n_far += __shfl_xor(n_far, o_); n_sk += __shfl_xor(n_sk, o_); }
+      L_near = __builtin_amdgcn_readfirstlane(L_near); n_far = __builtin_amdgcn_readfirstlane(n_far); n_sk = __builtin_amdgcn_readfirstlane(n_sk);
+      int lpv = 0;
+      if (lane < 2 * NEP_MAX_POL) lpv = (lane & 1) ? sCnt[(lane >> 1) * 6 + 2] : sCnt[(lane >> 1) * 6 + 3] + sCnt[(lane >> 1) * 6 + 4];
+      SampleSched sched_; sched_.n = ps.pre_sched_n; sched_.seg = nullptr; sched_.dt = nullptr;
+      done = pre_close(sp, ps, sched_, slot, K, lane, pre, L_near, n_far, n_sk, lpv, sdyn, g, t0, ps.presolved);
+    }
+    if (!done && lane == 0) ps.presolved[slot] = 0;
   }
   SEP_PT(8);
 #ifdef NEP_SEP_PROF
@@ -1367,26 +1385,35 @@
   return (int)((separator_lds_bytes(sp) - tail) / 16);
 }
 
-void launch_separator(int n_slots, const SceneParams& sp, const ProblemSet& ps, hipStream_t st) {
+int separator_pack(int n_slots, const SceneParams& sp, const ProblemSet& ps) {
+  const int total = sp.n_hull + sp.num_agents + sp.n_static + (sp.ent_enabled ? sp.num_agents * kBend : 0);
+  if (!(((ps.skip_box && ps.line_far && sp.cull_radius > 0.0 && ps.sep_pack >= 0) || (sp.cull_radius == 0.0 && ps.sep_pack >= 1)) && sp.sep_rule == 0 && total <= 8191)) return 0;
+  int pack = 1; while (pack < NEP_MAX_POL && (long)n_slots * (NEP_MAX_POL / (pack * 2)) >= 4096) pack *= 2;
+  if (ps.sep_pack >= 1 && ps.sep_pack <= NEP_MAX_POL) pack = ps.sep_pack;
+  return pack;
+}
+void launch_separator(int n_slots, const SceneParams& sp, const ProblemSet& ps_in, hipStream_t st) {
   if (n_slots <= 0) return;
-  const int total = sp.n_hull + sp.num_agents + sp.n_static + (sp.ent_enabled ? sp.num_agents * kBend : 0);
-  if (((ps.skip_box && ps.line_far && sp.cull_radius > 0.0 && ps.sep_pack >= 0) || (sp.cull_radius == 0.0 && ps.sep_pack >= 1)) && sp.sep_rule == 0 && total <= 8191) {
+  const int pack = separator_pack(n_slots, sp, ps_in);
+  if (pack > 0) {
+    ProblemSet ps = ps_in;
+    if (pack != NEP_MAX_POL || !(sp.cull_radius > 0.0) || !ps.line_far || !ps.presolved || !ps.pre_sched_n || ps.active) ps.pre_tables = nullptr;
     const size_t rounds_ = (size_t)((sp.n_hull + 63) / 64 + (sp.num_agents + 63) / 64 + (sp.n_static + 63) / 64);
     const size_t extras = 15 * NEP_MAX_POL * sizeof(double) + 2 * NEP_MAX_POL * rounds_ * sizeof(unsigned long long) + 6 * NEP_MAX_POL * sizeof(int)
                           + ((sp.ent_enabled && ps.case_id) ? (size_t)NEP_MAX_POL * ((sp.num_agents + 63) / 64) * sizeof(unsigned long long) : 0)
-                          + (size_t)(sep_packed_cap(sp.n_hull + sp.num_agents + sp.n_static) + (sp.ent_enabled ? sp.num_agents : 0)) * sizeof(unsigned short);
+                          + (size_t)(sep_packed_cap(sp.n_hull + sp.num_agents + sp.n_static) + (sp.ent_enabled ? sp.num_agents : 0)) * sizeof(unsigned short)
+                          + (ps.pre_tables ? (size_t)8 * NEP_MAX_POL * sizeof(double) + 8 : 0);
     size_t pool_b = extras + 64 * 6 * 16 <= (size_t)kSepLdsTarget ? (size_t)kSepLdsTarget - extras : (size_t)64 * 6 * 16;
     pool_b &= ~(size_t)15;
     const int pairs = (int)(pool_b / 16);
     const size_t lds_p = (pool_b + extras + 15) & ~(size_t)15;
     static DynLdsAttr attr_p;
     (void)attr_p.ensure((const void*)separator_packed_kernel, lds_p);
-    int pack = 1; while (pack < NEP_MAX_POL && (long)n_slots * (NEP_MAX_POL / (pack * 2)) >= 4096) pack *= 2;
-    if (ps.sep_pack >= 1 && ps.sep_pack <= NEP_MAX_POL) pack = ps.sep_pack;
     const int groups = (NEP_MAX_POL + pack - 1) / pack;
     hipLaunchKernelGGL(separator_packed_kernel, dim3(n_slots * groups), dim3(64), lds_p, st, sp, ps, pairs, pack);
     return;
   }
+  const ProblemSet& ps = ps_in;
   const size_t lds = separator_lds_bytes(sp);
   static DynLdsAttr attr[2];
   if (sp.sep_rule == 1) {
diff --git a/neptune_amd/csrc/nep_device.h b/neptune_amd/csrc/nep_device.h
--- a/neptune_amd/csrc/nep_device.h
+++ b/neptune_amd/csrc/nep_device.h
@@ -90,6 +90,8 @@
   int* polish_flag;
   int* polish_list; int* polish_count;
   int* presolved;
+  const QpTable* pre_tables;
+  const int* pre_sched_n;
   long long* dbg;
   int* flags;
   double* fe_box;
@@ -145,6 +147,7 @@
                            double T_span, double drone_radius, double* hull_xy, int* hull_nv,
                            double* hull0_xy, int* hull0_nv, int* flags, hipStream_t st);
 void launch_separator(int n_slots, const SceneParams& sp, const ProblemSet& ps, hipStream_t st);
+int separator_pack(int n_slots, const SceneParams& sp, const ProblemSet& ps);
 void launch_separator_redo(int n_slots, const SceneParams& sp, const ProblemSet& ps, hipStream_t st);
 void launch_boxes(int n_scenes, const SceneParams& sp, const ProblemSet& ps, hipStream_t st);
 void launch_active_rows(int n_slots, const SceneParams& sp, const ProblemSet& ps, double tol, int* out, hipStream_t st);
diff --git a/neptune_amd/csrc/nep_tables.h b/neptune_amd/csrc/nep_tables.h
--- a/neptune_amd/csrc/nep_tables.h
+++ b/neptune_amd/csrc/nep_tables.h
@@ -8,11 +8,12 @@
 
 namespace nep {
 
-static const double kAPosInv[4][4] = {
-    {-0.03203276669713047, -0.09273093424558249, 0.3420572455666699, 1.1023313949144335},
-    {-0.05111494245568798, -0.046272612998418894, 0.5458234872124772, 1.0979806946005568},
-    {-0.07454781852812224, 0.203951949894552, 0.796048050105448, 1.0745478185281223},
-    {1.0, 1.0, 0.9999999999999996, 0.9999999999999993}};
+#define NEP_APOS_INV_LITERALS { \
+    {-0.03203276669713047, -0.09273093424558249, 0.3420572455666699, 1.1023313949144335}, \
+    {-0.05111494245568798, -0.046272612998418894, 0.5458234872124772, 1.0979806946005568}, \
+    {-0.07454781852812224, 0.203951949894552, 0.796048050105448, 1.0745478185281223}, \
+    {1.0, 1.0, 0.9999999999999996, 0.9999999999999993}}
+static const double kAPosInv[4][4] = NEP_APOS_INV_LITERALS;
 static const double kAVelInv[3][3] = {
     {-0.07735026918962577, 0.16666666666666635, 1.077350269189625},
     {-0.07735026918962577, 0.49999999999999967, 1.077350269189625},
diff --git a/neptune_amd/csrc/qp_outputs.h b/neptune_amd/csrc/qp_outputs.h
--- a/neptune_amd/csrc/qp_outputs.h
+++ b/neptune_amd/csrc/qp_outputs.h
@@ -28,7 +28,7 @@
 template <int NT>
 __device__ __forceinline__ void write_trajectory(nep_solution* sol, const double* theta, int K, const double* t_start, double T, int tid) {
   for (int t = tid; t < 3 * NEP_MAX_POL * 4; t += NT) (&sol->coeff[0][0][0])[t] = ((t % (NEP_MAX_POL * 4)) / 4 < K) ? theta[t] : 0.0;
-  if (tid <= NEP_MAX_POL) sol->times[tid] = (tid <= K) ? *t_start + tid * T : 0.0;
+  if (tid <= NEP_MAX_POL) sol->times[tid] = (tid <= K) ? __builtin_fma((double)tid, T, *t_start) : 0.0;
 }
 
 template <int NT>
diff --git a/neptune_amd/csrc/qp_presolve.h b/neptune_amd/csrc/qp_presolve.h
--- /dev/null
+++ b/neptune_amd/csrc/qp_presolve.h
@@ -0,0 +1,138 @@
+#pragma once
+#include <hip/hip_runtime.h>
+
+#include "nep_device.h"
+#include "nep_tables.h"
+#include "qp_outputs.h"
+
+namespace nep {
+
+__device__ __forceinline__ double pre_dot4(double m0, double m1, double m2, double m3, double v0, double v1, double v2, double v3) {
+#pragma clang fp contract(off)
+  return __builtin_fma(m3, v3, __builtin_fma(m2, v2, __builtin_fma(m0, v0, m1 * v1)));
+}
+__device__ __forceinline__ double pre_cubic(double T, const double* q) {
+#pragma clang fp contract(off)
+  return __builtin_fma(T, q[2], __builtin_fma(T * T * T, q[0], (T * T) * q[1])) + q[3];
+}
+
+struct PreStart {
+  double viol;
+  double th[3];
+  double obj;
+  bool moved;
+  bool has_qc, z_override;
+};
+
+__device__ __forceinline__ PreStart pre_start(const SceneParams& sp, const QpTable* __restrict__ tb, const nep_guess* __restrict__ g, int K, int lane, double* xy, double* theta, const double (*apos)[4]) {
+#pragma clang fp contract(off)
+  PreStart S;
+  const double T = sp.T_span;
+  const double* gcoef = &g->coeff[0][0][0];
+  double rm0 = 0, rm1 = 0, rm2 = 0, rm3 = 0, tm0 = 0, tm1 = 0, tm2 = 0, tm3 = 0, P0 = 0, P1 = 0, P2 = 0, P3 = 0;
+  const int rho = lane >> 1, axm = lane & 1, sg = rho >> 2, k = rho & 3;
+  if (lane < 8 * K) { const double* q = tb->RowMap[lane]; rm0 = q[0]; rm1 = q[1]; rm2 = q[2]; rm3 = q[3]; }
+  if (lane < 4 * K) { const double* q = tb->ThMap[lane]; tm0 = q[0]; tm1 = q[1]; tm2 = q[2]; tm3 = q[3]; }
+  if (lane < 8 * K) { const double* q = gcoef + (axm * 8 + sg) * 4; P0 = q[0]; P1 = q[1]; P2 = q[2]; P3 = q[3]; }
+  const double* oq = tb->ObjQ[lane & 3];
+  const double oq0 = oq[0], oq1 = oq[1], oq2 = oq[2], oq3 = oq[3];
+  const double a0 = apos[0][k], a1 = apos[1][k], a2 = apos[2][k], a3 = apos[3][k];
+  double vv[3][4];
+#pragma unroll
+  for (int ax = 0; ax < 3; ax++) {
+    const double* c0 = g->coeff[ax][0]; const double* cK = g->coeff[ax][K - 1];
+    vv[ax][0] = c0[1]; vv[ax][1] = c0[2]; vv[ax][2] = c0[3];
+    vv[ax][3] = pre_cubic(T, cK);
+  }
+  theta[lane] = 0.0; if (lane + 64 < 96) theta[lane + 64] = 0.0;
+  S.viol = -1.0;
+  if (lane < 8 * K) {
+#pragma unroll
+    for (int ax = 0; ax < 3; ax++) {
+      const double a = pre_dot4(rm0, rm1, rm2, rm3, vv[ax][0], vv[ax][1], vv[ax][2], vv[ax][3]);
+      const double hi = lane < 4 * K ? sp.maxs[ax] : (lane < 7 * K ? sp.v_max : sp.a_max);
+      const double lo = lane < 4 * K ? sp.mins[ax] : (lane < 7 * K ? -sp.v_max : -sp.a_max);
+      S.viol = fmax(S.viol, fmax(a - hi, lo - a));
+      if (ax < 2 && lane < 4 * K) xy[ax * 32 + lane] = a;
+    }
+  }
+  __syncthreads();
+#pragma unroll
+  for (int ax = 0; ax < 3; ax++) S.th[ax] = pre_dot4(tm0, tm1, tm2, tm3, vv[ax][0], vv[ax][1], vv[ax][2], vv[ax][3]);
+  if (lane < 4 * K) { theta[lane] = S.th[0]; theta[32 + lane] = S.th[1]; theta[64 + lane] = S.th[2]; }
+  __syncthreads();
+  const double dix = vv[0][2] - vv[0][3], diy = vv[1][2] - vv[1][3], diz = vv[2][2] - vv[2][3];
+  const double dxy2 = __builtin_fma(dix, dix, diy * diy);
+  S.has_qc = sqrt(__builtin_fma(diz, diz, dxy2)) < 1.0;
+  S.z_override = sqrt(dxy2) < 1.0;
+  if (S.has_qc) {
+    double c = -0.10 * 0.10;
+#pragma unroll
+    for (int ax = 0; ax < 3; ax++) { const double pe = pre_cubic(T, theta + (ax * 8 + (K - 1)) * 4) - vv[ax][3]; c = __builtin_fma(pe, pe, c); }
+    S.viol = fmax(S.viol, c);
+  }
+  S.moved = false;
+  {
+    const double c0 = (T * T * T) * a0, c1 = (T * T) * a1, c2 = T * a2, c3 = a3;
+    const double* Q = theta + (axm * 8 + (lane < 8 * K ? sg : 0)) * 4;
+    const double v = pre_dot4(Q[0], Q[1], Q[2], Q[3], c0, c1, c2, c3);
+    const double gq = pre_dot4(P0, P1, P2, P3, c0, c1, c2, c3);
+    double d2 = (v - gq) * (v - gq);
+    d2 += __shfl_xor(d2, 1);
+    if (lane < 8 * K) S.moved = !(d2 <= sp.cull_radius * sp.cull_radius * (1.0 - 1e-9));
+  }
+  double o = 0;
+#pragma unroll
+  for (int ax = 0; ax < 3; ax++) {
+    const double r_ = __builtin_fma(oq3, vv[ax][3], __builtin_fma(oq2, vv[ax][2], __builtin_fma(oq1, vv[ax][1], __builtin_fma(oq0, vv[ax][0], 0.0))));
+#pragma unroll
+    for (int a = 0; a < 4; a++) o = __builtin_fma(vv[ax][a], __shfl(r_, a), o);
+  }
+  S.obj = o;
+  return S;
+}
+
+__device__ __forceinline__ double pre_line_viol(double n1, double n2, double n3, const double* px, const double* py) {
+#pragma clang fp contract(off)
+  const double h = 1.0 - n3;
+  double viol = -1.0;
+#pragma unroll
+  for (int k = 0; k < 4; k++) viol = fmax(viol, __builtin_fma(n1, px[k], n2 * py[k]) - h);
+  return viol;
+}
+
+__device__ __forceinline__ bool pre_close(const SceneParams& sp, const ProblemSet& ps, const SampleSched& sched, int slot, int K, int lane, const PreStart& S,
+                                          int L_near, int n_far, int n_skip, int lpv, double* theta, const nep_guess* __restrict__ g, long long t0, int* __restrict__ presolved) {
+  const double T = sp.T_span;
+  nep_solution* __restrict__ sol = ps.solution + slot;
+  if (__ballot(S.viol > 0.0) != 0ull) return false;
+  if ((n_far > 0 || n_skip > 0) && __ballot(S.moved) != 0ull) return false;
+
+  int n_lp = (lane & 1) == 0 ? lpv : 0, n_lpf = (lane & 1) == 1 ? lpv : 0;
+#pragma unroll
+  for (int o_ = 8; o_ > 0; o_ >>= 1) { n_lp += __shfl_xor(n_lp, o_); n_lpf += __shfl_xor(n_lpf, o_); }
+  theta[lane] = 0.0; if (lane + 64 < 96) theta[lane + 64] = 0.0;
+  __syncthreads();
+  if (lane < 4 * K) { theta[lane] = S.th[0]; theta[32 + lane] = S.th[1]; if (!S.z_override) theta[64 + lane] = S.th[2]; }
+  if (S.z_override && lane < 32) theta[64 + lane] = (&g->coeff[2][0][0])[lane];
+  __syncthreads();
+  write_trajectory<64>(sol, theta, K, &g->t_start, T, lane);
+  const int ns = sched_states(sp, sched, K);
+  if (lane == 0) {
+    const int L_all = L_near + n_far + n_skip;
+    sol->stats.status = NEP_OK; sol->stats.iters = 0; sol->stats.iters_first = 0;
+    sol->stats.n_lines = L_all - n_lpf; sol->stats.n_lp = n_lp; sol->stats.n_lp_failed = n_lpf;
+    sol->stats.n_rows = 48 * K + 4 * (L_near < L_all ? L_near : L_near - n_lpf); sol->stats.qc_active = S.has_qc ? 1 : 0;
+    sol->stats.objective = S.obj;
+    sol->K = K; sol->n_states = ns;
+  }
+  if (lane == 0) {
+    const double us_ = (double)((long long)wall_clock64() - t0) * sp.us_per_tick;
+    sol->stats.solve_us = us_;
+    if (ps.order_key) { const int ko = ps.order_key[slot] - sp.qp_key_decay; ps.order_key[slot] = (sp.qp_key_decay > 0 && ko > 0) ? ko : 0; }
+    presolved[slot] = 1;
+  }
+  return true;
+}
+
+}
diff --git a/neptune_amd/csrc/qp_presolve_kernel.hip b/neptune_amd/csrc/qp_presolve_kernel.hip
--- a/neptune_amd/csrc/qp_presolve_kernel.hip
+++ b/neptune_amd/csrc/qp_presolve_kernel.hip
@@ -1,32 +1,13 @@
 #include <hip/hip_runtime.h>
 
-#include "nep_device.h"
-#include "nep_tables.h"
-#include "qp_outputs.h"
+#include "qp_presolve.h"
 
 namespace nep {
 
-namespace {
-__constant__ double cPreAPosInv[4][4] = {
-    {-0.03203276669713047, -0.09273093424558249, 0.3420572455666699, 1.1023313949144335},
-    {-0.05111494245568798, -0.046272612998418894, 0.5458234872124772, 1.0979806946005568},
-    {-0.07454781852812224, 0.203951949894552, 0.796048050105448, 1.0745478185281223},
-    {1.0, 1.0, 0.9999999999999996, 0.9999999999999993}};
-
-__device__ __forceinline__ double pre_wave_max(double v) {
-#pragma unroll
-  for (int o = 32; o > 0; o >>= 1) v = fmax(v, __shfl_xor(v, o));
-  return v;
-}
-__device__ __forceinline__ double pre_wave_sum(double v) {
-#pragma unroll
-  for (int o = 32; o > 0; o >>= 1) v += __shfl_xor(v, o);
-  return v;
-}
-}
+namespace { __constant__ double cPreAPosInv[4][4] = NEP_APOS_INV_LITERALS; }
 
 #ifndef NEP_PRE_WAVES
-#define NEP_PRE_WAVES 6
+#define NEP_PRE_WAVES 4
 #endif
 __global__ __launch_bounds__(64, NEP_PRE_WAVES) void qp_presolve_kernel(SceneParams sp, ProblemSet ps, const QpTable* __restrict__ tables, SampleSched sched, int* __restrict__ presolved) {
   __builtin_amdgcn_s_setprio(3);
@@ -34,15 +15,12 @@
   if (ps.order_count && (int)blockIdx.x >= *ps.order_count) return;
   const int slot = ps.order_count ? ps.order[blockIdx.x] : (int)blockIdx.x;
   const long long t0 = (long long)wall_clock64();
-  __shared__ double sCoef[96], sTheta[96], sA[2 * 32];
+  __shared__ double sTheta[96], sA[2 * 32];
   __shared__ int sCnt[3 * NEP_MAX_POL + 4];
   const nep_guess* __restrict__ g = ps.guess + slot;
-  nep_solution* __restrict__ sol = ps.solution + slot;
   const int K = g->K;
-  const double T = sp.T_span;
   if (lane == 0) presolved[slot] = 0;
   if (K < 3 || K > NEP_MAX_POL || K > sp.num_pol) return;
-  const int R = 8 * K;
   const QpTable* __restrict__ tb = tables + K;
 
   int cn = 0, cf = 0, cs = 0; bool ovf = false;
@@ -52,43 +30,11 @@
     cf = ps.line_far[(long)slot * NEP_MAX_POL + lane];
     cs = ps.line_skip ? ps.line_skip[(long)slot * NEP_MAX_POL + lane] : 0;
   }
-  const double c_lo = (&g->coeff[0][0][0])[lane], c_hi = lane + 64 < 96 ? (&g->coeff[0][0][0])[lane + 64] : 0.0;
-  double rm0 = 0, rm1 = 0, rm2 = 0, rm3 = 0, tm0 = 0, tm1 = 0, tm2 = 0, tm3 = 0;
-  if (lane < R) { const double* q = tb->RowMap[lane]; rm0 = q[0]; rm1 = q[1]; rm2 = q[2]; rm3 = q[3]; }
-  if (lane < 4 * K) { const double* q = tb->ThMap[lane]; tm0 = q[0]; tm1 = q[1]; tm2 = q[2]; tm3 = q[3]; }
   int lpv = 0;
   if (ps.lp_stats && lane < 2 * NEP_MAX_POL) lpv = ps.lp_stats[(long)slot * NEP_MAX_POL * 2 + lane];
-  double vv[3][4];
-#pragma unroll
-  for (int ax = 0; ax < 3; ax++) {
-    const double* c0 = g->coeff[ax][0]; const double* cK = g->coeff[ax][K - 1];
-    vv[ax][0] = c0[1]; vv[ax][1] = c0[2]; vv[ax][2] = c0[3];
-    vv[ax][3] = ((T * T * T) * cK[0] + (T * T) * cK[1] + T * cK[2]) + cK[3];
-  }
+  PreStart S = pre_start(sp, tb, g, K, lane, sA, sTheta, cPreAPosInv);
   if (__ballot(ovf) != 0ull) return;
-  sCoef[lane] = c_lo; if (lane + 64 < 96) sCoef[lane + 64] = c_hi;
   if (lane < NEP_MAX_POL) { sCnt[lane] = cn; sCnt[NEP_MAX_POL + lane] = cf; sCnt[2 * NEP_MAX_POL + lane] = cs; }
-  const double dix = vv[0][2] - vv[0][3], diy = vv[1][2] - vv[1][3], diz = vv[2][2] - vv[2][3];
-  const bool has_qc = sqrt(dix * dix + diy * diy + diz * diz) < 1.0;
-  const bool z_override = sqrt(dix * dix + diy * diy) < 1.0;
-
-  double viol = -1.0;
-  if (lane < R) {
-#pragma unroll
-    for (int ax = 0; ax < 3; ax++) {
-      const double a = ((rm0 * vv[ax][0] + rm1 * vv[ax][1]) + rm2 * vv[ax][2]) + rm3 * vv[ax][3];
-      const double hi = lane < 4 * K ? sp.maxs[ax] : (lane < 7 * K ? sp.v_max : sp.a_max);
-      const double lo = lane < 4 * K ? sp.mins[ax] : (lane < 7 * K ? -sp.v_max : -sp.a_max);
-      viol = fmax(viol, fmax(a - hi, lo - a));
-      if (ax < 2 && lane < 4 * K) sA[ax * 32 + lane] = a;
-    }
-  }
-  sTheta[lane] = 0.0; if (lane + 64 < 96) sTheta[lane + 64] = 0.0;
-  __syncthreads();
-  if (lane < 4 * K) {
-#pragma unroll
-    for (int ax = 0; ax < 3; ax++) sTheta[(ax * 8 + lane / 4) * 4 + (lane % 4)] = ((tm0 * vv[ax][0] + tm1 * vv[ax][1]) + tm2 * vv[ax][2]) + tm3 * vv[ax][3];
-  }
   __syncthreads();
   int L_near = 0, n_far = 0, n_skip = 0;
 #pragma unroll
@@ -99,54 +45,9 @@
 #pragma unroll
     for (int j = 0; j < NEP_MAX_POL - 1; j++) { acc += sCnt[j]; if (e >= acc) { i = j + 1; off = acc; } }
     const double* nd = ps.line_nd + (((long)slot * NEP_MAX_POL + i) * sp.lines_cap + (e - off)) * 3;
-    const double n1 = nd[0], n2 = nd[1], h = 1.0 - nd[2];
-#pragma unroll
-    for (int k = 0; k < 4; k++) viol = fmax(viol, (n1 * sA[4 * i + k] + n2 * sA[32 + 4 * i + k]) - h);
+    S.viol = fmax(S.viol, pre_line_viol(nd[0], nd[1], nd[2], sA + 4 * i, sA + 32 + 4 * i));
   }
-  if (has_qc) {
-    double c = -0.10 * 0.10;
-#pragma unroll
-    for (int ax = 0; ax < 3; ax++) { const double* q = sTheta + (ax * 8 + (K - 1)) * 4; const double pe = (((T * T * T) * q[0] + (T * T) * q[1] + T * q[2]) + q[3]) - vv[ax][3]; c += pe * pe; }
-    viol = fmax(viol, c);
-  }
-  bool bad = false;
-  if (lane < 8 * K) {
-    const int rho = lane >> 1, ax = lane & 1, sg = rho >> 2, k = rho & 3;
-    const double c0 = (T * T * T) * cPreAPosInv[0][k], c1 = (T * T) * cPreAPosInv[1][k], c2 = T * cPreAPosInv[2][k], c3 = cPreAPosInv[3][k];
-    const double* Q = sTheta + (ax * 8 + sg) * 4;
-    const double v = ((Q[0] * c0 + Q[1] * c1) + Q[2] * c2) + Q[3] * c3;
-    const double* P = sCoef + (ax * 8 + sg) * 4;
-    const double gq = ((P[0] * c0 + P[1] * c1) + P[2] * c2) + P[3] * c3;
-    double d2 = (v - gq) * (v - gq);
-    d2 += __shfl_xor(d2, 1);
-    bad = (n_far > 0 || n_skip > 0) && !(d2 <= sp.cull_radius * sp.cull_radius * (1.0 - 1e-9));
-  }
-  if (!(pre_wave_max(viol) <= 0.0)) return;
-  if (__ballot(bad) != 0ull) return;
-
-  int n_lp = (lane & 1) == 0 ? lpv : 0, n_lpf = (lane & 1) == 1 ? lpv : 0;
-#pragma unroll
-  for (int o_ = 8; o_ > 0; o_ >>= 1) { n_lp += __shfl_xor(n_lp, o_); n_lpf += __shfl_xor(n_lpf, o_); }
-  if (z_override) { if (lane < 32) sTheta[64 + lane] = sCoef[64 + lane]; }
-  __syncthreads();
-  write_trajectory<64>(sol, sTheta, K, &g->t_start, T, lane);
-  const int ns = sched_states(sp, sched, K);
-  if (lane == 0) {
-    double o = 0;
-    for (int ax = 0; ax < 3; ax++) for (int a = 0; a < 4; a++) { double r_ = 0; for (int b = 0; b < 4; b++) r_ += tb->ObjQ[a][b] * vv[ax][b]; o += vv[ax][a] * r_; }
-    const int L_all = L_near + n_far + n_skip;
-    sol->stats.status = NEP_OK; sol->stats.iters = 0; sol->stats.iters_first = 0;
-    sol->stats.n_lines = L_all - n_lpf; sol->stats.n_lp = n_lp; sol->stats.n_lp_failed = n_lpf;
-    sol->stats.n_rows = 48 * K + 4 * (L_near < L_all ? L_near : L_near - n_lpf); sol->stats.qc_active = has_qc ? 1 : 0;
-    sol->stats.objective = o;
-    sol->K = K; sol->n_states = ns;
-  }
-  if (lane == 0) {
-    const double us_ = (double)((long long)wall_clock64() - t0) * sp.us_per_tick;
-    sol->stats.solve_us = us_;
-    if (ps.order_key) { const int ko = ps.order_key[slot] - sp.qp_key_decay; ps.order_key[slot] = (sp.qp_key_decay > 0 && ko > 0) ? ko : 0; }
-    presolved[slot] = 1;
-  }
+  pre_close(sp, ps, sched, slot, K, lane, S, L_near, n_far, n_skip, lpv, sTheta, g, t0, presolved);
 }
 
 void launch_qp_presolve(int n_slots, const SceneParams& sp, const ProblemSet& ps, const QpTable* tables, const SampleSched& sched, int* presolved, hipStream_t st) {
```
